# Quantum-Chemistry-Group-BNU/PyNQS

Measured on AMD Instinct MI355X. Metric: local energies/sec (whole node), higher is better.
Workload: dtype f64

## Files before the change

### include/pynqs_amd.h

```cpp
#ifndef PYNQS_AMD_H
#define PYNQS_AMD_H

#include <stdint.h>

#ifdef __cplusplus
extern "C" {
#endif

#define PYNQS_ABI_VERSION 1

#define PYNQS_OK 0
#define PYNQS_EINVAL (-1)
#define PYNQS_ELAUNCH (-2)
#define PYNQS_ELENGTH (-3)
#define PYNQS_EOVERFLOW (-4)

#define PYNQS_F32 0
#define PYNQS_F64 1

#define PYNQS_MAX_SORB_LEN 3
#define PYNQS_MAX_SORB 192
#define PYNQS_MAX_NELE 120
#define PYNQS_MAX_NVIR 120

int pynqs_abi_version(void);
const char *pynqs_last_error(void);

int64_t pynqs_num_sd(int sorb, int noA, int noB);

int pynqs_check_sorb(int sorb, int nele);

int pynqs_comb_hij_fused(const uint64_t *bra, int64_t nbatch, int sorb, int nele, int noA, int noB,
                         const void *h1e, const void *h2e, int dtype, uint64_t *comb, void *hmat,
                         void *stream);

int pynqs_comb(const uint64_t *bra, int64_t nbatch, int sorb, int noA, int noB, uint64_t *comb,
               double *comb_pm1, void *stream);

int pynqs_hij(const uint64_t *bra, int64_t n, const uint64_t *ket, int64_t m, int ket_is_3d,
              const void *h1e, const void *h2e, int dtype, int sorb, int nele, void *hmat, void *stream);

int pynqs_onv_to_pm1(const uint64_t *bra, int64_t n, int sorb, int dtype, void *out, void *stream);

int pynqs_pm01_to_onv(const uint8_t *occ, int64_t n, int sorb, uint64_t *out, void *stream);

int pynqs_wavefunction_lut(const uint64_t *keys, int64_t nkeys, const uint64_t *onv, int64_t n, int sorb,
                           int64_t *idx, uint8_t *mask, void *stream);

int pynqs_spin_flip_rand(const uint64_t *bra, int64_t n, int sorb, int noA, int noB, uint64_t seed,
                         uint64_t offset, uint64_t *out, void *stream);

int64_t pynqs_plan_bytes(int sorb, int dtype);
int pynqs_plan_build(const void *h1e, const void *h2e, int sorb, int dtype, void *plan, void *stream);

int pynqs_comb_hij_fused_plan(const uint64_t *bra, int64_t nbatch, int sorb, int nele, int noA, int noB,
                              const void *plan, int dtype, uint64_t *comb, void *hmat, void *stream);

int pynqs_eloc_sample_space(const uint64_t *bra, int64_t nbatch, int sorb, int nele, int noA, int noB,
                            const void *plan, const uint64_t *keys, int64_t nkeys, const double *wf,
                            int wf_is_complex, double *eloc, double *psi0, void *stream);

int64_t pynqs_hash_bytes(int64_t nkeys, int sorb);
int pynqs_hash_build(const uint64_t *keys, int64_t nkeys, int sorb, void *table, void *stream);
int pynqs_hash_lookup(const void *table, int64_t nkeys, const uint64_t *onv, int64_t n, int sorb, int64_t *idx,
                      uint8_t *mask, void *stream);
int pynqs_eloc_sample_space_hash(const uint64_t *bra, int64_t nbatch, int sorb, int nele, int noA, int noB,
                                 const void *plan, const void *table, int64_t nkeys, const double *wf,
                                 int wf_is_complex, double *eloc, double *psi0, void *stream);

int pynqs_eloc_sample_space_flip(const uint64_t *bra, int64_t nbatch, int sorb, int nele, int noA, int noB,
                                 const void *plan, const uint64_t *keys, int64_t nkeys, const double *wf,
                                 int wf_is_complex, const double *psi0, double *out, void *stream);
int pynqs_eloc_sample_space_hash_flip(const uint64_t *bra, int64_t nbatch, int sorb, int nele, int noA, int noB,
                                      const void *plan, const void *table, int64_t nkeys, const double *wf,
                                      int wf_is_complex, const double *psi0, double *out, void *stream);

int pynqs_eloc_sample_space_keys(const uint64_t *bra, int64_t nbatch, int sorb, int nele, int noA, int noB, const void *plan,
                                 const uint64_t *keys, int64_t nkeys, const double *wf, int wf_is_complex, int flip, double *eloc,
                                 double *psi0, void *stream);

int64_t pynqs_keys_index_bytes(int64_t nkeys, int sorb);
int64_t pynqs_keys_index_workspace(int64_t nkeys, int sorb);
int pynqs_keys_index_build(const uint64_t *keys, int64_t nkeys, int sorb, void *index, void *workspace, void *stream);
int pynqs_keys_index_density(const void *index, int64_t nkeys, int sorb, uint64_t *sum_sq, void *stream);
int pynqs_eloc_sample_space_indexed(const uint64_t *bra, int64_t nbatch, int sorb, int nele, int noA, int noB, const void *plan,
                                    const uint64_t *keys, int64_t nkeys, const void *index, const double *wf, int wf_is_complex,
                                    int flip, double *eloc, double *psi0, void *stream);

int pynqs_eloc_sample_space_form(int64_t nbatch, int sorb, int nele, int noA, int noB, int64_t nkeys, int hash, int64_t out[8]);
int pynqs_eloc_sample_space_keys_form(int64_t nbatch, int sorb, int64_t nkeys, int indexed, int64_t out[3]);

int64_t pynqs_unique_workspace(int64_t n);
int pynqs_unique_first(const uint64_t *onv, int64_t n, int sorb, void *workspace, int32_t *first, void *stream);

int pynqs_eloc_rbm_supported(int sorb, int nele, int noA, int noB, int nhidden);
int pynqs_eloc_rbm_form(int64_t nbatch, int sorb, int nele, int noA, int noB, int nhidden, int green);
int64_t pynqs_rbm_table_bytes(int sorb, int nhidden);
int pynqs_rbm_table_build(const double *weights, const double *hidden_bias, const double *visible_bias, int sorb,
                          int nhidden, void *table, void *stream);
int pynqs_eloc_rbm(const uint64_t *bra, int64_t nbatch, int sorb, int nele, int noA, int noB, const void *plan,
                   const void *rbm_table, int nhidden, double *eloc, double *psi, void *stream);
#define PYNQS_RBM_REAL 0
#define PYNQS_RBM_TANH 1
#define PYNQS_RBM_PHASE 2
int pynqs_eloc_rbm_flavour(const uint64_t *bra, int64_t nbatch, int sorb, int nele, int noA, int noB, const void *plan,
                           const void *rbm_table, int nhidden, int flavour, double *eloc, double *psi, void *stream);

int pynqs_eloc_crbm_supported(int sorb, int nele, int noA, int noB, int nhidden);
int pynqs_eloc_crbm_form(int64_t nbatch, int sorb, int nele, int noA, int noB, int nhidden);
int64_t pynqs_crbm_table_bytes(int sorb, int nhidden);
int pynqs_crbm_table_build(const double *weights, const double *hidden_bias, const double *visible_bias, int sorb, int nhidden,
                           void *table, void *stream);
int pynqs_eloc_crbm(const uint64_t *bra, int64_t nbatch, int sorb, int nele, int noA, int noB, const void *plan,
                    const void *crbm_table, int nhidden, double log_scale, double *eloc, double *psi, void *stream);

int64_t pynqs_jastrow_table_bytes(int sorb);
int pynqs_jastrow_table_build(const double *jastrow, int sorb, void *table, void *stream);
int pynqs_eloc_jrbm_supported(int sorb, int nele, int noA, int noB, int nhidden);
int pynqs_eloc_jrbm_form(int64_t nbatch, int sorb, int nele, int noA, int noB, int nhidden);
int pynqs_eloc_jrbm(const uint64_t *bra, int64_t nbatch, int sorb, int nele, int noA, int noB, const void *plan,
                    const void *rbm_table, const void *jastrow_table, int nhidden, double *eloc, double *psi, void *stream);
int pynqs_jrbm_forward(const uint64_t *onv, int64_t n, int sorb, const double *weights, const double *hidden_bias,
                       const double *visible_bias, const double *jastrow, int nhidden, double *psi, void *stream);
int64_t pynqs_jastrow_grad_workspace(int64_t n, int sorb);
int pynqs_jastrow_grad(const uint64_t *onv, int64_t n, int sorb, const double *jastrow, const double *prob, const double *eloc,
                       const double *e_total, const double *pow, double *grad_jastrow, double *loss, void *workspace, void *stream);

int pynqs_gfmc_sample(const double *green, int64_t n, int64_t ncomb, const double *rand_num, const uint64_t *comb,
                      int sorb, int64_t *index, double *beta, uint64_t *x_new, void *stream);

int pynqs_green_rbm(const uint64_t *bra, int64_t nbatch, int sorb, int nele, int noA, int noB, const void *plan,
                    const void *rbm_table, int nhidden, int flavour, double lambda, double *eloc, double *psi, double *green,
                    uint8_t *clamped, void *stream);
int pynqs_gfmc_sample_rank(const double *green, int64_t n, const double *rand_num, const uint64_t *bra, int sorb, int nele,
                           int noA, int noB, int64_t *index, double *beta, uint64_t *x_new, void *stream);

int64_t pynqs_moments_workspace(void);
int pynqs_stats_finish(const double *moments, double inv_world, double counts, double *out5, void *stream);
int pynqs_weighted_moments(const double *x, int is_complex, const double *prob, int64_t n, void *workspace, void *stream);

int64_t pynqs_reduce_tiles(int64_t nbatch, int sorb, int nele, int noA, int noB);
int pynqs_reduce_count(const uint64_t *bra, int64_t nbatch, int sorb, int nele, int noA, int noB,
                       const void *plan, int dtype, double eps, uint32_t *tile_counts, void *stream);
int pynqs_reduce_emit(const uint64_t *bra, int64_t nbatch, int sorb, int nele, int noA, int noB,
                      const void *plan, int dtype, double eps, const int64_t *tile_offsets, int32_t *kept_col,
                      uint64_t *kept_onv, void *kept_h, void *stream);

int pynqs_reduce_count_sums(const uint64_t *bra, int64_t nbatch, int sorb, int nele, int noA, int noB,
                            const void *plan, int dtype, double eps, uint32_t *tile_counts, double *tile_sums,
                            void *stream);
int pynqs_reduce_sample(const uint64_t *bra, int64_t nbatch, int sorb, int nele, int noA, int noB, const void *plan,
                        int dtype, double eps, const int32_t *tile_draws, const int64_t *sample_offsets,
                        const double *walker_scale, uint64_t seed, int32_t *s_col, uint64_t *s_onv, void *s_h,
                        void *stream);

typedef struct pynqs_reduce_io {
  int64_t cap_doubles;
  int64_t cap_unique;
  int64_t dedup_slots;
  int32_t *rec_col;
  void *rec_w;
  uint64_t *rec_onv;
  int32_t *rec_link;
  int32_t *seg_count;
  int32_t *srec_col;
  void *srec_w;
  uint64_t *srec_onv;
  int32_t *srec_link;
  double *row_sum;
  void *dedup_table;
  uint64_t *uniq_onv;
  void *uniq_pm1;
  int32_t pm1_dtype;
  int32_t lut_is_hash;
  const void *lut_table;
  int64_t lut_nkeys;
  int32_t *counters;
  const uint64_t *seed_dev;
  void *row_cache;
  int32_t *uniq_parent;
  void *tile_scratch;
  int64_t tile_scratch_bytes;
  float *row_f32;
} pynqs_reduce_io;
int pynqs_reduce_onepass_geometry(int64_t nbatch, int sorb, int nele, int noA, int noB, int eps_sample, int64_t *out4);
int64_t pynqs_reduce_onepass_tile_scratch_bytes(int64_t nbatch, int sorb, int nele, int noA, int noB, int eps_sample);
int pynqs_reduce_onepass_list_capacity(int64_t nbatch, int sorb, int nele, int noA, int noB, int dtype, int eps_sample,
                                       int with_row_cache, int without_table, int64_t *cap_doubles);
int pynqs_reduce_onepass_wants_row_f32(int64_t nbatch, int sorb, int nele, int noA, int noB, int dtype, int eps_sample, int64_t cap_doubles,
                                       int with_tile_scratch ,
                                       int without_table );
int64_t pynqs_reduce_onepass_row_f32_elements(int64_t nbatch, int sorb, int nele, int noA, int noB);
int pynqs_reduce_onepass(const uint64_t *bra, int64_t nbatch, int sorb, int nele, int noA, int noB, const void *plan,
                         int dtype, double eps, int eps_sample, uint64_t seed, const pynqs_reduce_io *io, void *stream);
int pynqs_reduce_contract(int64_t nbatch, int sorb, int nele, int noA, int noB, int dtype, int eps_sample,
                          const pynqs_reduce_io *io, const double *psi_unique, const double *psi_table, int psi_is_complex,
                          int divide, double *eloc, double *psi_x, void *stream);

#define PYNQS_RBM_COMPLEX 4
int pynqs_rbm_forward(const uint64_t *onv, int64_t n, int sorb, const double *weights, const double *hidden_bias,
                      const double *visible_bias, int nhidden, int flavour, double *psi, void *stream);

int64_t pynqs_rbm_children_table_bytes(int64_t nwalkers, int sorb, int nhidden, int flavour);
int pynqs_rbm_children_prepare(const uint64_t *walkers, int64_t nwalkers, int sorb, const double *weights, const double *hidden_bias,
                               const double *visible_bias, int nhidden, int flavour, void *table, void *stream);
int pynqs_rbm_forward_children(const uint64_t *onv, int64_t n, const int32_t *count_dev, const int32_t *parent,
                               const uint64_t *walkers, int64_t nwalkers, const void *table, int sorb, const double *weights,
                               const double *hidden_bias, const double *visible_bias, int nhidden, int flavour, double *psi,
                               void *stream);
int pynqs_rbm_forward_children_supported(int sorb, int nhidden, int flavour);

int64_t pynqs_rbm_grad_workspace(int64_t n, int sorb, int nhidden, int flavour);
int pynqs_rbm_grad(const uint64_t *onv, int64_t n, int sorb, const double *weights, const double *hidden_bias,
                   const double *visible_bias, int nhidden, int flavour, const double *prob, const double *eloc,
                   int eloc_is_complex, const double *e_total, const double *pow, double *grad_weights,
                   double *grad_hidden_bias, double *grad_visible_bias, double *loss, void *workspace, void *stream);

#define PYNQS_SR_RHO 0
#define PYNQS_SR_RHS2 1
#define PYNQS_SR_DONE 2
#define PYNQS_SR_ITER 3
#define PYNQS_SR_TRUE2 4
#define PYNQS_SR_PAP 5
#define PYNQS_SR_CONVERGED 6
#define PYNQS_SR_BREAKDOWN 7
#define PYNQS_SR_NSCALARS 8
#define PYNQS_SR_CG_INIT 0
#define PYNQS_SR_CG_STEP 1
#define PYNQS_SR_CG_RESIDUAL 2
int64_t pynqs_rbm_sr_workspace(int64_t n, int sorb, int nhidden, int flavour);
int pynqs_rbm_sr_prepare(const uint64_t *onv, int64_t n, int sorb, const double *weights, const double *hidden_bias, int nhidden,
                         int flavour, const double *prob, void *workspace, double *obar, void *stream);
int pynqs_rbm_sr_matvec(const uint64_t *onv, int64_t n, int sorb, int nhidden, int flavour, const double *prob, const void *workspace,
                        const double *obar, const double *v, double *y, void *stream);
int pynqs_rbm_sr_cg_step(int mode, int64_t np, double *y, const double *rhs, double *d, double *r, double *p, double *scalars,
                         double inv_world, double diag_shift, double tol, void *stream);

#define PYNQS_MCMC_ACCEPT_KEY 0x243F6A8885A308D3ull
int pynqs_mcmc_rbm_supported(int sorb, int nhidden, int flavour);
int pynqs_mcmc_rbm(uint64_t *states, int64_t nchains, int sorb, int noA, int noB, const void *table, int nhidden, int flavour,
                   uint64_t seed, uint64_t chain_base, uint64_t t0, int nsteps, int every, uint64_t *records, int64_t *n_accept,
                   double *lnpsi, void *stream);
int pynqs_mcmc_accept(uint64_t *states, double *psi, const uint64_t *proposals, const double *psi_proposals, int64_t nchains,
                      int sorb, int is_complex, uint64_t seed, uint64_t chain_base, uint64_t t, uint64_t *record_row,
                      int64_t *n_accept, void *stream);

int pynqs_rdm_scatter(const uint64_t *bra, int64_t nbatch, int sorb, int nele, int noA, int noB, const double *w, const double *ratio,
                      int is_complex, double *rdm1, double *rdm2, void *stream);
int pynqs_rdm_rbm_supported(int sorb, int nele, int noA, int noB, int nhidden);
int64_t pynqs_rdm_rbm_workspace(int64_t nbatch, int sorb, int nhidden);
int pynqs_rdm_rbm(const uint64_t *bra, int64_t nbatch, int sorb, int nele, int noA, int noB, const double *w, const void *rbm_table,
                  int nhidden, void *workspace, double *rdm1, double *rdm2, void *stream);

#ifdef __cplusplus
}
#endif
#endif
```

### pynqs_amd/C_extension.py

```python
from __future__ import annotations

import os
import warnings
import weakref
from typing import Tuple

import numpy as np
import torch
from torch import Tensor

from . import _native as N

MAX_SORB_LEN = 3
MAX_SORB = 64 * MAX_SORB_LEN
MAX_NELE = 120
USE_PLAN = True

__all__ = [
    "tensor_to_onv", "onv_to_tensor", "get_comb_tensor", "get_hij_torch", "get_comb_hij_fused",
    "wavefunction_lut", "hash_build", "hash_lookup", "HashTable", "RBMTable", "eloc_rbm", "JastrowTable", "eloc_jrbm", "jrbm_forward", "eloc_jrbm_supported", "merge_rank_sample", "spin_flip_rand", "check_sorb", "compress_h1e_h2e", "decompress_h1e_h2e", "get_Num_SinglesDoubles",
    "MAX_SORB", "MAX_SORB_LEN", "MAX_NELE",
]


def _bra_len(sorb: int) -> int:
    return (sorb - 1) // 64 + 1


def _gpu() -> torch.device:
    if not torch.cuda.is_available():
        raise RuntimeError("pynqs_amd: no HIP device available (this package has no CPU fallback)")
    return torch.device("cuda", torch.cuda.current_device())


def _stage(*ts: Tensor):
    all_cpu = all(t.device.type == "cpu" for t in ts)
    dev = next((t.device for t in ts if t.device.type == "cuda"), None) or _gpu()
    return dev, [t if t.device == dev else t.to(dev) for t in ts], all_cpu


def _ver(t: Tensor) -> int:
    try:
        return t._version
    except RuntimeError:
        return -1


def _stream(dev: torch.device) -> int:
    return torch.cuda.current_stream(dev).cuda_stream


def _contig(t: Tensor, name: str) -> None:
    if not t.is_contiguous():
        raise RuntimeError(f"{name} must be contiguous")


def _check_onv(t: Tensor, name: str, sorb: int, dims) -> None:
    _contig(t, name)
    if t.dtype != torch.uint8:
        raise RuntimeError(f"{name} must be torch.uint8")
    if t.dim() not in dims:
        raise RuntimeError(f"{name} must have dim in {dims}, got {t.dim()}")
    if t.size(-1) != 8 * _bra_len(sorb):
        raise RuntimeError(f"{name}: last dim {t.size(-1)} != 8 * bra_len = {8 * _bra_len(sorb)} for sorb = {sorb}")


def _fdtype(h1e: Tensor, h2e: Tensor) -> int:
    if h1e.dtype != h2e.dtype or h1e.dtype not in (torch.float32, torch.float64):
        raise RuntimeError("h1e/h2e must both be float32 or both float64")
    return N.PYNQS_F64 if h1e.dtype == torch.float64 else N.PYNQS_F32


def _check_integrals(h1e: Tensor, h2e: Tensor, sorb: int) -> None:
    _contig(h1e, "h1e_tensor"); _contig(h2e, "h2e_tensor")
    pair = sorb * (sorb - 1) // 2
    if h1e.numel() != sorb * sorb or h2e.numel() != pair * (pair + 1) // 2:
        raise RuntimeError(f"h1e/h2e sizes {h1e.numel()}/{h2e.numel()} do not match sorb = {sorb}")


class IntegralPlan:

    def __init__(self, h1e: Tensor, h2e: Tensor, sorb: int, device: "torch.device | None" = None):
        code = _fdtype(h1e, h2e)
        _check_integrals(h1e, h2e, sorb)
        nbytes = N.lib().pynqs_plan_bytes(sorb, code)
        if nbytes < 0:
            raise RuntimeError(f"integral plan needs an even sorb in [2, {MAX_SORB}], got {sorb}")
        dev, (a, b), _ = _stage(h1e, h2e)
        if device is not None and device.type == "cuda" and all(t.device.type == "cpu" for t in (h1e, h2e)):
            dev, a, b = device, h1e.to(device), h2e.to(device)
        self.sorb, self.code, self.dtype, self.device = sorb, code, h1e.dtype, dev
        self.buf = torch.empty(nbytes // h1e.element_size(), dtype=h1e.dtype, device=dev)
        N.check(N.lib().pynqs_plan_build(a.data_ptr(), b.data_ptr(), sorb, code, self.buf.data_ptr(), _stream(dev)), "plan_build")
        if a is not h1e or b is not h2e:
            torch.cuda.current_stream(dev).synchronize()

    def data_ptr(self) -> int:
        return self.buf.data_ptr()


_PLANS: "list[tuple]" = []
_MAX_PLANS = 4
_PLAN_BUILDS: "dict[tuple, int]" = {}
_PLAN_REBUILD_WARN = 16


_FINGERPRINT_CHUNK = 1 << 24


def _fingerprint(h1e: Tensor, h2e: Tensor):
    if any(t.is_cuda for t in (h1e, h2e)) and torch.cuda.is_current_stream_capturing():
        return None
    golden = -7046029254386353131
    out = []
    with torch.no_grad():
        for t in (h1e, h2e):
            c = t.detach().contiguous().reshape(-1)
            c = c.view(torch.int64) if c.element_size() == 8 else c.view(torch.int32)
            plain = torch.zeros((), dtype=torch.int64, device=c.device)
            mixed = torch.zeros((), dtype=torch.int64, device=c.device)
            for s in range(0, c.numel(), _FINGERPRINT_CHUNK):
                v = c[s:s + _FINGERPRINT_CHUNK].to(torch.int64)
                plain += v.sum()
                m = torch.arange(s, s + v.numel(), dtype=torch.int64, device=c.device).mul_(golden).add_(v)
                del v
                m.bitwise_xor_(m >> 30).mul_(-4658895280553007687)
                m.bitwise_xor_(m >> 27).mul_(-7723592293110705685)
                m.bitwise_xor_(m >> 31)
                mixed += m.sum()
                del m
            out.append((tuple(t.shape), str(t.dtype), str(t.device), int(plain.item()), int(mixed.item())))
    return tuple(out)


def plan_for(h1e: Tensor, h2e: Tensor, sorb: int, device: "torch.device | None" = None) -> "IntegralPlan | None":
    if sorb % 2 or sorb < 2:
        return None
    ver = (_ver(h1e), _ver(h2e), h1e.data_ptr(), h2e.data_ptr())
    trackable = ver[0] >= 0 and ver[1] >= 0
    def same(ref, t):
        o = ref()
        return o is t or (o is not None and o.data_ptr() == t.data_ptr() and o.shape == t.shape and o.stride() == t.stride() and o.dtype == t.dtype)

    dev_ok = lambda pl: device is None or device.type != "cuda" or pl.device == device or h1e.device.type == "cuda"
    for i, (r1, r2, v, s, pl, fp) in enumerate(_PLANS if trackable else ()):
        if same(r1, h1e) and same(r2, h2e) and v == ver and s == sorb and dev_ok(pl):
            if i:
                _PLANS.insert(0, _PLANS.pop(i))
            return pl
    fp = None
    if any(s == sorb and f is not None and f[1][0] == tuple(h2e.shape) for _, _, _, s, _, f in _PLANS):
        fp = _fingerprint(h1e, h2e)
        for i, (r1, r2, v, s, pl, f) in enumerate(_PLANS):
            if fp is not None and f == fp and s == sorb and dev_ok(pl):
# ... 292 lines not shown

    def _build(self, kind: str, given, params, nhidden: int, sorb: int) -> None:
        dev, ts, _ = _stage(*params)
        self.nhidden, self.sorb, self.device = nhidden, sorb, dev
        nbytes = getattr(N.lib(), f"pynqs_{kind}_table_bytes")(sorb, nhidden)
        if nbytes < 0:
            raise RuntimeError(f"bad RBM sizes: sorb = {sorb}, num_hidden = {nhidden}")
        self.buf = torch.empty(nbytes // 8, dtype=torch.float64, device=dev)
        N.check(getattr(N.lib(), f"pynqs_{kind}_table_build")(ts[0].data_ptr(), ts[1].data_ptr(), ts[2].data_ptr() if len(ts) > 2 else None,
                                                              sorb, nhidden, self.buf.data_ptr(), _stream(dev)), f"{kind}_table_build")
        if any(a.data_ptr() != b.data_ptr() for a, b in zip(given, ts)):
            torch.cuda.current_stream(dev).synchronize()

    def data_ptr(self) -> int:
        return self.buf.data_ptr()


class RBMTable(_RBMTableBase):

    def __init__(self, weights: Tensor, hidden_bias: Tensor, visible_bias: "Tensor | None" = None) -> None:
        if weights.dim() != 2 or hidden_bias.numel() != weights.size(0):
            raise RuntimeError("weights must be [num_hidden, sorb] and hidden_bias [num_hidden]")
        if visible_bias is not None and visible_bias.numel() != weights.size(1):
            raise RuntimeError("visible_bias must be [sorb]")
        ts = [weights, hidden_bias] + ([visible_bias] if visible_bias is not None else [])
        if any(t.dtype != torch.float64 for t in ts):
            raise RuntimeError("the fused RBM local energy is float64 only")
        self._build("rbm", ts, [t.detach().contiguous() for t in ts], int(weights.size(0)), int(weights.size(1)))


class JastrowTable:

    def __init__(self, jastrow: Tensor) -> None:
        if jastrow.dim() != 2 or jastrow.size(0) != jastrow.size(1):
            raise RuntimeError("jastrow must be [sorb, sorb]")
        if jastrow.dtype != torch.float64:
            raise RuntimeError("the fused Jastrow-RBM local energy is float64 only")
        given = jastrow.detach().contiguous()
        dev, (m,), _ = _stage(given)
        self.sorb, self.device = int(m.size(0)), dev
        nbytes = N.lib().pynqs_jastrow_table_bytes(self.sorb)
        if nbytes < 0:
            raise RuntimeError(f"bad Jastrow size: sorb = {self.sorb}")
        self.buf = torch.empty(nbytes // 8, dtype=torch.float64, device=dev)
        N.check(N.lib().pynqs_jastrow_table_build(m.data_ptr(), self.sorb, self.buf.data_ptr(), _stream(dev)), "jastrow_table_build")
        if m.data_ptr() != jastrow.data_ptr():
            torch.cuda.current_stream(dev).synchronize()

    def data_ptr(self) -> int:
        return self.buf.data_ptr()


RBM_TYPE_FLAVOUR = {"real": N.RBM_REAL, "tanh": N.RBM_TANH, "pRBM": N.RBM_PHASE, "complex": N.RBM_COMPLEX}
RBM_FLAVOURS = {k: v for k, v in RBM_TYPE_FLAVOUR.items() if v != N.RBM_COMPLEX}


def _rbm_dtype(rbm_type: str) -> torch.dtype:
    return torch.complex128 if rbm_type in ("pRBM", "complex") else torch.float64


def _eloc_fused(bra: Tensor, h1e: Tensor, h2e: Tensor, table, sorb: int, want_psi: bool, dtype: torch.dtype, call):
    if table.sorb != sorb:
        raise RuntimeError(f"RBM table was built for sorb = {table.sorb}, not {sorb}")
    if _fdtype(h1e, h2e) != N.PYNQS_F64:
        raise RuntimeError("the fused RBM local energy is float64 only")
    plan = plan_for(h1e, h2e, sorb, bra.device)
    if plan is None:
        raise RuntimeError("the fused RBM local energy needs an even sorb")
    dev, (x,), all_cpu = _stage(bra)
    if plan.device != dev or table.device != dev:
        raise RuntimeError("bra, integrals and RBM table must be on the same device")
    n = x.size(0)
    eloc = torch.empty(n, dtype=dtype, device=dev)
    psi = torch.empty(n, dtype=dtype, device=dev) if want_psi else None
    call(x, n, plan, eloc, psi.data_ptr() if want_psi else None, _stream(dev))
    if all_cpu and bra.device.type == "cpu":
        return eloc.cpu(), (psi.cpu() if want_psi else None)
    return eloc, psi


def eloc_rbm(bra: Tensor, h1e: Tensor, h2e: Tensor, table: RBMTable, sorb: int, nele: int, noA: int, noB: int,
             want_psi: bool = True, rbm_type: str = "real") -> Tuple[Tensor, "Tensor | None"]:
    _check_onv(bra, "bra", sorb, (2,))
    if rbm_type not in RBM_FLAVOURS:
        raise RuntimeError(f"rbm_type {rbm_type!r} has no fused local energy (fused: {sorted(RBM_FLAVOURS)})")
    return _eloc_fused(bra, h1e, h2e, table, sorb, want_psi, _rbm_dtype(rbm_type), lambda x, n, plan, eloc, psi, st: N.check(
        N.lib().pynqs_eloc_rbm_flavour(x.data_ptr(), n, sorb, nele, noA, noB, plan.data_ptr(), table.data_ptr(), table.nhidden,
                                       RBM_FLAVOURS[rbm_type], eloc.data_ptr(), psi, st), "pynqs_eloc_rbm"))


def eloc_jrbm_supported(sorb: int, nele: int, noA: int, noB: int, num_hidden: int) -> bool:
    return bool(N.lib().pynqs_eloc_jrbm_supported(sorb, nele, noA, noB, num_hidden))


def eloc_jrbm(bra: Tensor, h1e: Tensor, h2e: Tensor, rbm_table: RBMTable, jastrow_table: JastrowTable, sorb: int, nele: int, noA: int, noB: int,
              want_psi: bool = True) -> Tuple[Tensor, "Tensor | None"]:
    _check_onv(bra, "bra", sorb, (2,))
    if jastrow_table.sorb != sorb or jastrow_table.device != rbm_table.device:
        raise RuntimeError(f"Jastrow table: sorb = {jastrow_table.sorb} on {jastrow_table.device}, RBM table: sorb = {sorb} on {rbm_table.device}")
    return _eloc_fused(bra, h1e, h2e, rbm_table, sorb, want_psi, torch.float64, lambda x, n, plan, eloc, psi, st: N.check(
        N.lib().pynqs_eloc_jrbm(x.data_ptr(), n, sorb, nele, noA, noB, plan.data_ptr(), rbm_table.data_ptr(), jastrow_table.data_ptr(),
                                rbm_table.nhidden, eloc.data_ptr(), psi, st), "pynqs_eloc_jrbm"))


def jrbm_forward(onv: Tensor, weights: Tensor, hidden_bias: Tensor, visible_bias: "Tensor | None", jastrow: Tensor, sorb: int) -> Tensor:
    _check_onv(onv, "onv", sorb, (2,))
    _, W, hb, vb, H = _rbm_params(weights, hidden_bias, visible_bias, sorb, "real", on_gpu=False)
    M = jastrow.detach().double().contiguous()
    if M.shape != (sorb, sorb):
        raise RuntimeError("jastrow must be [sorb, sorb]")
    if not (onv.is_cuda and W.is_cuda and hb.is_cuda and (vb is None or vb.is_cuda) and M.is_cuda):
        raise RuntimeError("jrbm_forward: determinants and parameters must be on the GPU")
    n = onv.size(0)
    psi = torch.empty(n, dtype=torch.float64, device=onv.device)
    N.check(N.lib().pynqs_jrbm_forward(onv.data_ptr(), n, sorb, W.data_ptr(), hb.data_ptr(), vb.data_ptr() if vb is not None else None, M.data_ptr(),
                                       H, psi.data_ptr(), _stream(onv.device)), "pynqs_jrbm_forward")
    return psi


def rbm_forward(onv: Tensor, weights: Tensor, hidden_bias: Tensor, visible_bias: "Tensor | None", sorb: int, rbm_type: str = "real") -> Tensor:
    _check_onv(onv, "onv", sorb, (2,))
    flav, W, hb, vb, H = _rbm_params(weights, hidden_bias, visible_bias, sorb, rbm_type, on_gpu=False)
    if not (onv.is_cuda and W.is_cuda and hb.is_cuda and (vb is None or vb.is_cuda)):
        raise RuntimeError("rbm_forward: determinants and parameters must be on the GPU")
    n = onv.size(0)
    psi = torch.empty(n, dtype=_rbm_dtype(rbm_type), device=onv.device)
    N.check(N.lib().pynqs_rbm_forward(onv.data_ptr(), n, sorb, W.data_ptr(), hb.data_ptr(), vb.data_ptr() if vb is not None else None, H, flav,
                                      psi.data_ptr(), _stream(onv.device)), "pynqs_rbm_forward")
    return psi


def _rbm_params(weights, hidden_bias, visible_bias, sorb, rbm_type, on_gpu=True):
    flav = RBM_TYPE_FLAVOUR.get(rbm_type)
    if flav is None:
        raise RuntimeError(f"rbm_type {rbm_type!r} has no fused forward")
    cplx_par = rbm_type == "complex"
    W = weights.detach().double().contiguous()
    hb = hidden_bias.detach().double().contiguous()
    vb = visible_bias.detach().double().contiguous() if visible_bias is not None else None
    H = W.size(0)
    if W.shape[:2] != (H, sorb) or W.dim() != (3 if cplx_par else 2) or hb.numel() != H * (2 if cplx_par else 1) or \
            (vb is not None and vb.numel() != sorb * (2 if cplx_par else 1)):
        raise RuntimeError("RBM parameter shapes do not match sorb / num_hidden")
    if on_gpu and not (W.is_cuda and hb.is_cuda and (vb is None or vb.is_cuda)):
        raise RuntimeError("RBM parameters must be on the GPU")
    return flav, W, hb, vb, H


def rbm_forward_children_supported(sorb: int, num_hidden: int, rbm_type: str = "real") -> bool:
    flav = RBM_TYPE_FLAVOUR.get(rbm_type)
    return flav is not None and bool(N.lib().pynqs_rbm_forward_children_supported(sorb, num_hidden, flav))


def rbm_forward_children(onv: Tensor, parent: Tensor, walkers: Tensor, weights: Tensor, hidden_bias: Tensor, visible_bias: "Tensor | None",
                         sorb: int, rbm_type: str = "real", count: "Tensor | None" = None, out: "Tensor | None" = None) -> Tensor:
    _check_onv(onv, "onv", sorb, (2,))
    _check_onv(walkers, "walkers", sorb, (2,))
    flav, W, hb, vb, H = _rbm_params(weights, hidden_bias, visible_bias, sorb, rbm_type)
    dev = onv.device
    if not (onv.is_cuda and walkers.device == dev and parent.device == dev and parent.dtype == torch.int32 and parent.numel() >= onv.size(0)):
        raise RuntimeError("rbm_forward_children: onv, walkers and parent (int32) on one GPU")
    n, nw = onv.size(0), walkers.size(0)
    nbytes = N.lib().pynqs_rbm_children_table_bytes(nw, sorb, H, flav)
    table = torch.empty(max(nbytes // 8, 1), dtype=torch.float64, device=dev)
    st = _stream(dev)
    wk = walkers.contiguous()
    N.check(N.lib().pynqs_rbm_children_prepare(wk.data_ptr(), nw, sorb, W.data_ptr(), hb.data_ptr(), vb.data_ptr() if vb is not None else None,
                                               H, flav, table.data_ptr(), st), "pynqs_rbm_children_prepare")
    psi = out if out is not None else torch.empty(n, dtype=_rbm_dtype(rbm_type), device=dev)
    N.check(N.lib().pynqs_rbm_forward_children(onv.contiguous().data_ptr(), n, count.data_ptr() if count is not None else None, parent.data_ptr(),
                                               wk.data_ptr(), nw, table.data_ptr(), sorb, W.data_ptr(), hb.data_ptr(),
                                               vb.data_ptr() if vb is not None else None, H, flav, psi.data_ptr(), st), "pynqs_rbm_forward_children")
    return psi


class CRBMTable(_RBMTableBase):

    def __init__(self, weights: Tensor, hidden_bias: Tensor, visible_bias: "Tensor | None" = None) -> None:
        def as_pairs(t: Tensor) -> Tensor:
            t = t.detach()
            if t.is_complex():
                t = torch.view_as_real(t.to(torch.complex128))
            if t.dtype != torch.float64 or t.size(-1) != 2:
                raise RuntimeError("complex RBM parameters must be complex128 or float64 (re, im) pairs")
            return t.contiguous()

        w, hb = as_pairs(weights), as_pairs(hidden_bias).reshape(-1, 2)
        vb = as_pairs(visible_bias).reshape(-1, 2) if visible_bias is not None else None
        if w.dim() != 3 or hb.size(0) != w.size(0) or (vb is not None and vb.size(0) != w.size(1)):
            raise RuntimeError("weights must be [num_hidden, sorb], hidden_bias [num_hidden], visible_bias [sorb]")
        given = [weights, hidden_bias] + ([visible_bias] if visible_bias is not None else [])
        self._build("crbm", given, [w, hb] + ([vb] if vb is not None else []), int(w.size(0)), int(w.size(1)))


def eloc_crbm(bra: Tensor, h1e: Tensor, h2e: Tensor, table: CRBMTable, sorb: int, nele: int, noA: int, noB: int,
              want_psi: bool = True, log_scale: float = 0.0) -> Tuple[Tensor, "Tensor | None"]:
    _check_onv(bra, "bra", sorb, (2,))
    return _eloc_fused(bra, h1e, h2e, table, sorb, want_psi, torch.complex128, lambda x, n, plan, eloc, psi, st: N.check(
        N.lib().pynqs_eloc_crbm(x.data_ptr(), n, sorb, nele, noA, noB, plan.data_ptr(), table.data_ptr(), table.nhidden, float(log_scale),
                                eloc.data_ptr(), psi, st), "pynqs_eloc_crbm"))


_CHARTS = None


def constrain_make_charts(sym_idex: Tensor) -> Tensor:
    sym_index = sym_idex
    global _CHARTS
    if _CHARTS is None:
        t = torch.zeros((16, 4), dtype=torch.float64)
        for k, row in zip((10, 6, 14, 9, 5, 13, 11, 7, 15), ((1, 0, 0, 0), (0, 0, 1, 0), (1, 0, 1, 0), (0, 1, 0, 0), (0, 0, 0, 1), (0, 1, 0, 1),
                                                             (1, 1, 0, 0), (0, 0, 1, 1), (1, 1, 1, 1))):
            t[k] = torch.tensor(row, dtype=torch.float64)
        _CHARTS = t
    idx = sym_index.reshape(-1).long()
    inside = (idx >= 0) & (idx < 16)
    out = _CHARTS.to(idx.device)[idx.clamp(0, 15)]
    return torch.where(inside.unsqueeze(1), out, torch.zeros_like(out))


def permute_sgn(image2: Tensor, onstate: Tensor, sorb: int) -> Tensor:
    if image2.numel() != sorb and onstate.size(-1) != sorb:
        raise ValueError("Dim error")
    if onstate.size(0) == 0:
        return torch.zeros(0, dtype=torch.float64, device=onstate.device)
    order = image2.reshape(-1).long().to(onstate.device)
    occ = (onstate.reshape(onstate.size(0), -1)[:, order] != 0).to(torch.float64)
    pos = torch.arange(order.numel(), device=order.device)
    inverted = ((pos.unsqueeze(1) < pos.unsqueeze(0)) & (order.unsqueeze(1) > order.unsqueeze(0))).to(torch.float64)
    pairs = ((occ @ inverted) * occ).sum(1)
    return (1 - 2 * (pairs.long() & 1)).to(torch.float64)


def spin_flip_rand(bra: Tensor, sorb: int, nele: int, noA: int, noB: int, seed: int, in_place: bool = False) -> Tuple[Tensor, Tensor]:
    global _SPIN_FLIP_CALLS
    _check_onv(bra, "bra_tensor", sorb, (1, 2))
    x2 = bra.view(-1, bra.size(-1))
    n = x2.size(0)
    dev, (x,), cpu = _stage(x2)
    out = x if (in_place and not cpu) else torch.empty_like(x)
    if n:
        N.check(N.lib().pynqs_spin_flip_rand(x.data_ptr(), n, sorb, noA, noB, int(seed) & (2**64 - 1), _SPIN_FLIP_CALLS << 32,
                                             out.data_ptr(), _stream(dev)), "spin_flip_rand")
    _SPIN_FLIP_CALLS += 1
    if cpu:
        out = out.cpu()
        if in_place:
            x2.copy_(out)
            out = x2
    return onv_to_tensor(out, sorb), out


def merge_rank_sample(idx: Tensor, counts: Tensor, split_idx: Tensor, length: int) -> Tensor:
    _contig(idx, "idx"); _contig(counts, "counts")
    out = torch.zeros(int(length), dtype=torch.int64, device=idx.device)
    return out.index_add_(0, idx.to(torch.int64), counts.to(torch.int64))


def _pair_maps(sorb: int):
    i, j = np.meshgrid(np.arange(sorb), np.arange(sorb), indexing="ij")
    hi, lo = np.maximum(i, j), np.minimum(i, j)
    pair = hi * (hi - 1) // 2 + lo
    sgn = np.where(i > j, 1.0, -1.0)
    return pair, sgn, i != j


def compress_h1e_h2e(h1e: np.ndarray, h2e: np.ndarray, sorb: int):
    h1e = np.asarray(h1e, dtype=np.float64)
    h2e = np.asarray(h2e, dtype=np.float64)
    if h1e.shape != (sorb, sorb) or h2e.shape != (sorb,) * 4:
        raise ValueError(f"expected h1e {(sorb, sorb)} and h2e {(sorb,) * 4}, got {h1e.shape} and {h2e.shape}")
    npair = sorb * (sorb - 1) // 2
    pair, sgn, off = _pair_maps(sorb)
    out = np.zeros(npair * (npair + 1) // 2, dtype=np.float64)
    kl, skl, okl = pair[None, :, :], sgn[None, :, :], off[None, :, :]
    for i in range(sorb):
        ij = pair[i][:, None, None]
        valid = off[i][:, None, None] & okl
        P, Q = np.maximum(ij, kl), np.minimum(ij, kl)
        out[(P * (P + 1) // 2 + Q)[valid]] = (sgn[i][:, None, None] * skl * h2e[i])[valid]
    return h1e.reshape(-1).copy(), out


def decompress_h1e_h2e(h1e: np.ndarray, h2e: np.ndarray, sorb: int):
    h1e = np.asarray(h1e, dtype=np.float64).reshape(-1)
    h2e = np.asarray(h2e, dtype=np.float64).reshape(-1)
    npair = sorb * (sorb - 1) // 2
    if h1e.size != sorb * sorb:
        raise ValueError(f"h1e array size is incorrect: expected {sorb * sorb}, got {h1e.size}")
    if h2e.size != npair * (npair + 1) // 2:
        raise ValueError(f"h2e array size is incorrect: expected {npair * (npair + 1) // 2}, got {h2e.size}")
    pair, sgn, off = _pair_maps(sorb)
    full = np.zeros((sorb,) * 4, dtype=np.float64)
    kl, skl, okl = pair[None, :, :], sgn[None, :, :], off[None, :, :]
    for i in range(sorb):
        ij = pair[i][:, None, None]
        valid = off[i][:, None, None] & okl
        P, Q = np.maximum(ij, kl), np.minimum(ij, kl)
        slot = np.where(valid, P * (P + 1) // 2 + Q, 0)
        full[i] = np.where(valid, h2e[slot] * (sgn[i][:, None, None] * skl), 0.0)
    return h1e.reshape(sorb, sorb).copy(), full
```

### pynqs_amd/_native.py

```python
from __future__ import annotations

import ctypes as C
import os

_HERE = os.path.dirname(os.path.abspath(__file__))
LIB_PATH = os.environ.get("PYNQS_AMD_LIB") or os.path.join(_HERE, "csrc", "libpynqs_amd.so")

PYNQS_F32, PYNQS_F64 = 0, 1
RBM_REAL, RBM_TANH, RBM_PHASE, RBM_COMPLEX = 0, 1, 2, 4
OK, EINVAL, ELAUNCH, ELENGTH, EOVERFLOW = 0, -1, -2, -3, -4

_i64, _int, _vp, _dbl = C.c_int64, C.c_int, C.c_void_p, C.c_double

SIGNATURES = {
    "pynqs_abi_version": (_int, []),
    "pynqs_last_error": (C.c_char_p, []),
    "pynqs_num_sd": (_i64, [_int, _int, _int]),
    "pynqs_check_sorb": (_int, [_int, _int]),
    "pynqs_comb_hij_fused": (_int, [_vp, _i64, _int, _int, _int, _int, _vp, _vp, _int, _vp, _vp, _vp]),
    "pynqs_comb": (_int, [_vp, _i64, _int, _int, _int, _vp, _vp, _vp]),
    "pynqs_hij": (_int, [_vp, _i64, _vp, _i64, _int, _vp, _vp, _int, _int, _int, _vp, _vp]),
    "pynqs_onv_to_pm1": (_int, [_vp, _i64, _int, _int, _vp, _vp]),
    "pynqs_pm01_to_onv": (_int, [_vp, _i64, _int, _vp, _vp]),
    "pynqs_wavefunction_lut": (_int, [_vp, _i64, _vp, _i64, _int, _vp, _vp, _vp]),
    "pynqs_spin_flip_rand": (_int, [_vp, _i64, _int, _int, _int, C.c_uint64, C.c_uint64, _vp, _vp]),
    "pynqs_plan_bytes": (_i64, [_int, _int]),
    "pynqs_plan_build": (_int, [_vp, _vp, _int, _int, _vp, _vp]),
    "pynqs_comb_hij_fused_plan": (_int, [_vp, _i64, _int, _int, _int, _int, _vp, _int, _vp, _vp, _vp]),
    "pynqs_eloc_sample_space": (_int, [_vp, _i64, _int, _int, _int, _int, _vp, _vp, _i64, _vp, _int, _vp, _vp, _vp]),
    "pynqs_hash_bytes": (_i64, [_i64, _int]),
    "pynqs_hash_build": (_int, [_vp, _i64, _int, _vp, _vp]),
    "pynqs_hash_lookup": (_int, [_vp, _i64, _vp, _i64, _int, _vp, _vp, _vp]),
    "pynqs_unique_workspace": (_i64, [_i64]),
    "pynqs_unique_first": (_int, [_vp, _i64, _int, _vp, _vp, _vp]),
    "pynqs_eloc_sample_space_hash": (_int, [_vp, _i64, _int, _int, _int, _int, _vp, _vp, _i64, _vp, _int, _vp, _vp, _vp]),
    "pynqs_eloc_sample_space_flip": (_int, [_vp, _i64, _int, _int, _int, _int, _vp, _vp, _i64, _vp, _int, _vp, _vp, _vp]),
    "pynqs_eloc_sample_space_hash_flip": (_int, [_vp, _i64, _int, _int, _int, _int, _vp, _vp, _i64, _vp, _int, _vp, _vp, _vp]),
    "pynqs_eloc_sample_space_keys": (_int, [_vp, _i64, _int, _int, _int, _int, _vp, _vp, _i64, _vp, _int, _int, _vp, _vp, _vp]),
    "pynqs_keys_index_bytes": (_i64, [_i64, _int]),
    "pynqs_keys_index_workspace": (_i64, [_i64, _int]),
    "pynqs_keys_index_build": (_int, [_vp, _i64, _int, _vp, _vp, _vp]),
    "pynqs_keys_index_density": (_int, [_vp, _i64, _int, _vp, _vp]),
    "pynqs_eloc_sample_space_indexed": (_int, [_vp, _i64, _int, _int, _int, _int, _vp, _vp, _i64, _vp, _vp, _int, _int, _vp, _vp, _vp]),
    "pynqs_eloc_sample_space_form": (_int, [_i64, _int, _int, _int, _int, _i64, _int, C.POINTER(_i64)]),
    "pynqs_eloc_sample_space_keys_form": (_int, [_i64, _int, _i64, _int, C.POINTER(_i64)]),
    "pynqs_eloc_rbm_supported": (_int, [_int, _int, _int, _int, _int]),
    "pynqs_eloc_rbm_form": (_int, [_i64, _int, _int, _int, _int, _int, _int]),
    "pynqs_rbm_table_bytes": (_i64, [_int, _int]),
    "pynqs_rbm_table_build": (_int, [_vp, _vp, _vp, _int, _int, _vp, _vp]),
    "pynqs_eloc_rbm": (_int, [_vp, _i64, _int, _int, _int, _int, _vp, _vp, _int, _vp, _vp, _vp]),
    "pynqs_eloc_rbm_flavour": (_int, [_vp, _i64, _int, _int, _int, _int, _vp, _vp, _int, _int, _vp, _vp, _vp]),
    "pynqs_eloc_crbm_supported": (_int, [_int, _int, _int, _int, _int]),
    "pynqs_eloc_crbm_form": (_int, [_i64, _int, _int, _int, _int, _int]),
    "pynqs_crbm_table_bytes": (_i64, [_int, _int]),
    "pynqs_crbm_table_build": (_int, [_vp, _vp, _vp, _int, _int, _vp, _vp]),
    "pynqs_eloc_crbm": (_int, [_vp, _i64, _int, _int, _int, _int, _vp, _vp, _int, _dbl, _vp, _vp, _vp]),
    "pynqs_gfmc_sample": (_int, [_vp, _i64, _i64, _vp, _vp, _int, _vp, _vp, _vp, _vp]),
    "pynqs_green_rbm": (_int, [_vp, _i64, _int, _int, _int, _int, _vp, _vp, _int, _int, _dbl, _vp, _vp, _vp, _vp, _vp]),
    "pynqs_gfmc_sample_rank": (_int, [_vp, _i64, _vp, _vp, _int, _int, _int, _int, _vp, _vp, _vp, _vp]),
    "pynqs_moments_workspace": (_i64, []),
    "pynqs_stats_finish": (_int, [_vp, _dbl, _dbl, _vp, _vp]),
    "pynqs_weighted_moments": (_int, [_vp, _int, _vp, _i64, _vp, _vp]),
    "pynqs_reduce_tiles": (_i64, [_i64, _int, _int, _int, _int]),
    "pynqs_reduce_count": (_int, [_vp, _i64, _int, _int, _int, _int, _vp, _int, _dbl, _vp, _vp]),
    "pynqs_reduce_count_sums": (_int, [_vp, _i64, _int, _int, _int, _int, _vp, _int, _dbl, _vp, _vp, _vp]),
    "pynqs_reduce_sample": (_int, [_vp, _i64, _int, _int, _int, _int, _vp, _int, _dbl, _vp, _vp, _vp, C.c_uint64, _vp, _vp, _vp, _vp]),
    "pynqs_reduce_emit": (_int, [_vp, _i64, _int, _int, _int, _int, _vp, _int, _dbl, _vp, _vp, _vp, _vp, _vp]),
}



class ReduceIO(C.Structure):
    _fields_ = [("cap_doubles", _i64), ("cap_unique", _i64), ("dedup_slots", _i64),
                ("rec_col", _vp), ("rec_w", _vp), ("rec_onv", _vp), ("rec_link", _vp), ("seg_count", _vp),
                ("srec_col", _vp), ("srec_w", _vp), ("srec_onv", _vp), ("srec_link", _vp), ("row_sum", _vp),
                ("dedup_table", _vp), ("uniq_onv", _vp), ("uniq_pm1", _vp), ("pm1_dtype", C.c_int32), ("lut_is_hash", C.c_int32),
                ("lut_table", _vp), ("lut_nkeys", _i64), ("counters", _vp), ("seed_dev", _vp), ("row_cache", _vp), ("uniq_parent", _vp),
                ("tile_scratch", _vp), ("tile_scratch_bytes", _i64), ("row_f32", _vp)]


SIGNATURES.update({
    "pynqs_reduce_onepass_geometry": (_int, [_i64, _int, _int, _int, _int, _int, C.POINTER(_i64)]),
    "pynqs_reduce_onepass_tile_scratch_bytes": (_i64, [_i64, _int, _int, _int, _int, _int]),
    "pynqs_reduce_onepass_list_capacity": (_int, [_i64, _int, _int, _int, _int, _int, _int, _int, _int, C.POINTER(_i64)]),
    "pynqs_reduce_onepass_wants_row_f32": (_int, [_i64, _int, _int, _int, _int, _int, _int, _i64, _int, _int]),
    "pynqs_reduce_onepass_row_f32_elements": (_i64, [_i64, _int, _int, _int, _int]),
    "pynqs_reduce_onepass": (_int, [_vp, _i64, _int, _int, _int, _int, _vp, _int, _dbl, _int, C.c_uint64, C.POINTER(ReduceIO), _vp]),
    "pynqs_rbm_forward": (_int, [_vp, _i64, _int, _vp, _vp, _vp, _int, _int, _vp, _vp]),
    "pynqs_rbm_children_table_bytes": (_i64, [_i64, _int, _int, _int]),
    "pynqs_rbm_children_prepare": (_int, [_vp, _i64, _int, _vp, _vp, _vp, _int, _int, _vp, _vp]),
    "pynqs_rbm_forward_children": (_int, [_vp, _i64, _vp, _vp, _vp, _i64, _vp, _int, _vp, _vp, _vp, _int, _int, _vp, _vp]),
    "pynqs_rbm_forward_children_supported": (_int, [_int, _int, _int]),
    "pynqs_rbm_grad_workspace": (_i64, [_i64, _int, _int, _int]),
    "pynqs_rbm_grad": (_int, [_vp, _i64, _int, _vp, _vp, _vp, _int, _int, _vp, _vp, _int, _vp, _vp, _vp, _vp, _vp, _vp, _vp, _vp]),
    "pynqs_reduce_contract": (_int, [_i64, _int, _int, _int, _int, _int, _int, C.POINTER(ReduceIO), _vp, _vp, _int, _int, _vp, _vp, _vp]),    "pynqs_mcmc_rbm_supported": (_int, [_int, _int, _int]),
    "pynqs_mcmc_rbm": (_int, [_vp, _i64, _int, _int, _int, _vp, _int, _int, C.c_uint64, C.c_uint64, C.c_uint64, _int, _int, _vp, _vp, _vp, _vp]),
    "pynqs_rbm_sr_workspace": (_i64, [_i64, _int, _int, _int]),
    "pynqs_rbm_sr_prepare": (_int, [_vp, _i64, _int, _vp, _vp, _int, _int, _vp, _vp, _vp, _vp]),
    "pynqs_rbm_sr_matvec": (_int, [_vp, _i64, _int, _int, _int, _vp, _vp, _vp, _vp, _vp, _vp]),
    "pynqs_rbm_sr_cg_step": (_int, [_int, _i64, _vp, _vp, _vp, _vp, _vp, _vp, _dbl, _dbl, _dbl, _vp]),
    "pynqs_mcmc_accept": (_int, [_vp, _vp, _vp, _vp, _i64, _int, _int, C.c_uint64, C.c_uint64, C.c_uint64, _vp, _vp, _vp]),
    "pynqs_rdm_scatter": (_int, [_vp, _i64, _int, _int, _int, _int, _vp, _vp, _int, _vp, _vp, _vp]),
    "pynqs_rdm_rbm_supported": (_int, [_int, _int, _int, _int, _int]),
    "pynqs_rdm_rbm_workspace": (_i64, [_i64, _int, _int]),
    "pynqs_rdm_rbm": (_int, [_vp, _i64, _int, _int, _int, _int, _vp, _vp, _int, _vp, _vp, _vp, _vp]),
    "pynqs_jastrow_table_bytes": (_i64, [_int]),
    "pynqs_jastrow_table_build": (_int, [_vp, _int, _vp, _vp]),
    "pynqs_eloc_jrbm_supported": (_int, [_int, _int, _int, _int, _int]),
    "pynqs_eloc_jrbm_form": (_int, [_i64, _int, _int, _int, _int, _int]),
    "pynqs_eloc_jrbm": (_int, [_vp, _i64, _int, _int, _int, _int, _vp, _vp, _vp, _int, _vp, _vp, _vp]),
    "pynqs_jrbm_forward": (_int, [_vp, _i64, _int, _vp, _vp, _vp, _vp, _int, _vp, _vp]),
    "pynqs_jastrow_grad_workspace": (_i64, [_i64, _int]),
    "pynqs_jastrow_grad": (_int, [_vp, _i64, _int, _vp, _vp, _vp, _vp, _vp, _vp, _vp, _vp, _vp]),
})

_lib = None


class NativeLibraryError(RuntimeError):
    pass


def lib() -> C.CDLL:
    global _lib
    if _lib is None:
        if not os.path.exists(LIB_PATH):
            raise NativeLibraryError(
                f"{LIB_PATH} not found: build the HIP extension first (python -c 'import __graft_entry__ as g; g.build()'). "
                "pynqs_amd has no CPU fallback."
            )
        try:
            l = C.CDLL(LIB_PATH)
        except OSError as e:
            raise NativeLibraryError(f"cannot load {LIB_PATH}: {e}") from e
        for name, (res, args) in SIGNATURES.items():
            f = getattr(l, name)
            f.restype = res
            f.argtypes = args
        if l.pynqs_abi_version() != 1:
            raise NativeLibraryError("libpynqs_amd.so ABI version mismatch")
        _lib = l
    return _lib


def check(rc: int, what: str) -> None:
    if rc == OK:
        return
    msg = lib().pynqs_last_error().decode(errors="replace")
    if rc == ELENGTH:
        raise ValueError(msg)
    if rc == EOVERFLOW:
        raise OverflowError(msg)
    raise RuntimeError(f"{what}: {msg} (code {rc})")
```

### pynqs_amd/csrc/kernels_gfmc.hip

```cpp
#include "detcore.h"
#include "launch.h"

namespace pynqs {

constexpr int kGfmcMaxTiles = 1024;

__device__ __forceinline__ double wave_incl_scan(double v, int lane) {
#pragma unroll
  for (int d = 1; d < 64; d <<= 1) {
    const double o = __shfl_up(v, d);
    if (lane >= d) v += o;
  }
  return v;
}

template <int LEN, bool FROM_RANK>
__global__ __launch_bounds__(kBlock) void gfmc_sample_kernel(const double *__restrict__ gk, int64_t m, uint32_t tile, uint32_t ntiles,
                                                             const double *__restrict__ rnd, const uint64_t *__restrict__ comb, SDParams p,
                                                             int64_t *__restrict__ index, double *__restrict__ beta,
                                                             uint64_t *__restrict__ x_new) {
  __shared__ double tsum[kGfmcMaxTiles];
  __shared__ double s_target, s_before;
  __shared__ uint32_t s_tile;
  const int64_t walker = blockIdx.x;
  const int tid = threadIdx.x, lane = tid & 63, wave = tid >> 6;
  const double *__restrict__ row = gk + walker * m;
  for (uint32_t t = wave; t < ntiles; t += kBlock / 64) {
    const int64_t c0 = (int64_t)t * tile, c1 = min(c0 + (int64_t)tile, m);
    double acc = 0.0;
    for (int64_t c = c0 + lane; c < c1; c += 64) acc += row[c];
#pragma unroll
    for (int d = 32; d > 0; d >>= 1) acc += __shfl_xor(acc, d);
    if (lane == 0) tsum[t] = acc;
  }
  __syncthreads();
  if (wave == 0) {
    constexpr int kPer = kGfmcMaxTiles / 64;
    double loc[kPer], s = 0.0;
#pragma unroll
    for (int i = 0; i < kPer; ++i) {
      const uint32_t t = lane * kPer + i;
      loc[i] = t < ntiles ? tsum[t] : 0.0;
      s += loc[i];
    }
    const double incl = wave_incl_scan(s, lane);
    const double total = __shfl(incl, 63);
    const double target = rnd[walker] * total;
    double before = incl - s;
    uint32_t mine = 0xffffffffu;
    double mine_before = 0.0;
#pragma unroll
    for (int i = 0; i < kPer; ++i) {
      const uint32_t t = lane * kPer + i;
      if (mine == 0xffffffffu && t < ntiles && before + loc[i] >= target) { mine = t; mine_before = before; }
      before += loc[i];
    }
    const uint64_t have = __ballot(mine != 0xffffffffu);
    const int first = have ? __ffsll((long long)have) - 1 : -1;
    if (lane == (first < 0 ? 0 : first)) {
      s_tile = first < 0 ? ntiles - 1 : mine;
      s_before = first < 0 ? total - tsum[ntiles - 1] : mine_before;
      s_target = target;
    }
    if (lane == 0) beta[walker] = total;
  }
  __syncthreads();
  if (wave == 0) {
    const uint32_t t = s_tile;
    const double target = s_target;
    double run = s_before;
    const int64_t c0 = (int64_t)t * tile, c1 = min(c0 + (int64_t)tile, m);
    int64_t found = -1, last_pos = -1;
    for (int64_t c = c0; c < c1 && found < 0; c += 64) {
      const double v = c + lane < c1 ? row[c + lane] : 0.0;
      const double incl = wave_incl_scan(v, lane) + run;
      const uint64_t hit = __ballot(c + lane < c1 && incl >= target);
      if (hit) found = c + __ffsll((long long)hit) - 1;
      const uint64_t pos = __ballot(v > 0.0);
      if (pos) last_pos = c + 63 - __clzll((long long)pos);
      run = __shfl(incl, 63);
    }
    if (found < 0) found = last_pos >= 0 ? last_pos : c1 - 1;
    if (lane == 0) index[walker] = found;
    if constexpr (FROM_RANK) {
      if (lane == 0) {
        uint64_t x[LEN];
#pragma unroll
        for (int i = 0; i < LEN; ++i) x[i] = comb[walker * LEN + i];
        if (found > 0) excite_by_rank<LEN>(x, (uint32_t)(found - 1), p);
#pragma unroll
        for (int i = 0; i < LEN; ++i) x_new[walker * LEN + i] = x[i];
      }
    } else {
      if (lane < LEN) x_new[walker * LEN + lane] = comb[(walker * m + found) * LEN + lane];
    }
  }
}

}

using namespace pynqs;

template <bool FROM_RANK>
static int gfmc_sample_impl(const double *green, int64_t n, int64_t ncomb, const double *rand_num, const uint64_t *comb, int sorb,
                            const SDParams &p, int64_t *index, double *beta, uint64_t *x_new, void *stream) {
  pynqs::DeviceScope device_scope_(green);
  if (n < 0 || ncomb < 1 || sorb < 1 || sorb > kMaxSorb) return set_error(PYNQS_EINVAL, "bad n / ncomb / sorb");
  if (n == 0) return PYNQS_OK;
  if (!green || !rand_num || !comb || !index || !beta || !x_new) return set_error(PYNQS_EINVAL, "null pointer");
  if (n > 0x7fffffffll) return set_error(PYNQS_EINVAL, "n too large for one launch");
  uint32_t tile = 256;
  while ((ncomb + tile - 1) / tile > kGfmcMaxTiles) tile *= 2;
  const uint32_t ntiles = (uint32_t)((ncomb + tile - 1) / tile);
  const int len = (sorb - 1) / 64 + 1;
  hipStream_t st = (hipStream_t)stream;
  DISPATCH_LEN(len, hipLaunchKernelGGL((gfmc_sample_kernel<LEN, FROM_RANK>), dim3((uint32_t)n), dim3(kBlock), 0, st, green, ncomb, tile, ntiles,
                                       rand_num, comb, p, index, beta, x_new));
  return check_launch("gfmc_sample");
}

extern "C" int pynqs_gfmc_sample(const double *green, int64_t n, int64_t ncomb, const double *rand_num, const uint64_t *comb, int sorb,
                                 int64_t *index, double *beta, uint64_t *x_new, void *stream) {
  SDParams p = {};
  return gfmc_sample_impl<false>(green, n, ncomb, rand_num, comb, sorb, p, index, beta, x_new, stream);
}

extern "C" int pynqs_gfmc_sample_rank(const double *green, int64_t n, const double *rand_num, const uint64_t *bra, int sorb, int nele,
                                      int noA, int noB, int64_t *index, double *beta, uint64_t *x_new, void *stream) {
  SDParams p;
  if (!make_sd_params(sorb, nele, noA, noB, &p)) return set_error(PYNQS_EINVAL, "bad sorb/noA/noB");
  return gfmc_sample_impl<true>(green, n, (int64_t)p.nsd + 1, rand_num, bra, sorb, p, index, beta, x_new, stream);
}

namespace pynqs {

constexpr int kMomentBlocks = 128;

template <bool CPLX>
__global__ __launch_bounds__(kBlock) void moments_kernel(const double *__restrict__ x, const double *__restrict__ prob, int64_t n,
                                                         double *__restrict__ out, unsigned int *__restrict__ done) {
  __shared__ double red[4][kBlock / 64];
  __shared__ bool last;
  const int tid = threadIdx.x, lane = tid & 63, wave = tid >> 6;
  double s[4] = {0.0, 0.0, 0.0, 0.0};
  for (int64_t i = (int64_t)blockIdx.x * kBlock + tid; i < n; i += (int64_t)gridDim.x * kBlock) {
    const double p = prob[i];
    const double re = CPLX ? x[2 * i] : x[i], im = CPLX ? x[2 * i + 1] : 0.0;
    s[0] += p * re; s[1] += p * im; s[2] += p * (re * re + im * im); s[3] += p;
  }
#pragma unroll
  for (int k = 0; k < 4; ++k) {
#pragma unroll
    for (int d = 32; d > 0; d >>= 1) s[k] += __shfl_xor(s[k], d);
    if (lane == 0) red[k][wave] = s[k];
  }
  __syncthreads();
  if (tid < 4) {
    double t = 0.0;
    for (int w = 0; w < kBlock / 64; ++w) t += red[tid][w];
    out[4 * (1 + blockIdx.x) + tid] = t;
  }
  __threadfence();
  __syncthreads();
  if (tid == 0) last = atomicAdd(done, 1u) == gridDim.x - 1;
  __syncthreads();
  if (last) {
    __threadfence();
    if (tid < 4) {
      double t = 0.0;
      for (unsigned b = 0; b < gridDim.x; ++b) t += out[4 * (1 + b) + tid];
      out[tid] = t;
    }
    if (tid == 0) *done = 0;
  }
}

}

namespace pynqs {
__global__ void stats_finish_kernel(const double *__restrict__ m, double inv_world, double counts, double *__restrict__ out) {
  const double re = m[0] * inv_world, im = m[1] * inv_world, m2 = m[2] * inv_world, ps = m[3] * inv_world;
  double var = m2 - (re * re + im * im) * (2.0 - ps);
  var = var > 0.0 ? var : 0.0;
  const double sd = sqrt(var);
  out[0] = re; out[1] = im; out[2] = var; out[3] = sd; out[4] = sd / sqrt(counts);
}
}

extern "C" int pynqs_stats_finish(const double *moments, double inv_world, double counts, double *out5, void *stream) {
  pynqs::DeviceScope device_scope_(moments);
  if (!moments || !out5 || !(counts > 0.0)) return set_error(PYNQS_EINVAL, "bad arguments");
  hipLaunchKernelGGL(stats_finish_kernel, dim3(1), dim3(1), 0, (hipStream_t)stream, moments, inv_world, counts, out5);
  return check_launch("stats_finish");
}

extern "C" int64_t pynqs_moments_workspace(void) { return 8 * 4 * (pynqs::kMomentBlocks + 1) + 8; }

extern "C" int pynqs_weighted_moments(const double *x, int is_complex, const double *prob, int64_t n, void *workspace, void *stream) {
  pynqs::DeviceScope device_scope_(x);
  if (n < 0) return set_error(PYNQS_EINVAL, "bad n");
  if (!workspace || (n > 0 && (!x || !prob))) return set_error(PYNQS_EINVAL, "null pointer");
  double *out = (double *)workspace;
  unsigned int *done = (unsigned int *)(out + 4 * (kMomentBlocks + 1));
  int64_t blocks = (n + kBlock - 1) / kBlock;
  if (blocks > kMomentBlocks) blocks = kMomentBlocks;
  if (blocks < 1) blocks = 1;
  hipStream_t st = (hipStream_t)stream;
  if (is_complex) hipLaunchKernelGGL((moments_kernel<true>), dim3((uint32_t)blocks), dim3(kBlock), 0, st, x, prob, n, out, done);
  else hipLaunchKernelGGL((moments_kernel<false>), dim3((uint32_t)blocks), dim3(kBlock), 0, st, x, prob, n, out, done);
  return check_launch("weighted_moments");
}
```

### pynqs_amd/csrc/kernels_rbm_forward.hip

```cpp
#include "detcore.h"
#include "launch.h"
#include "rbm_math.h"

namespace pynqs {

constexpr int kHChunk = 8;

struct Prod {
  double re = 1.0, im = 0.0;
  double lin = 0.0, ang = 0.0;
  int e2 = 0;
  __device__ __forceinline__ void renorm() {
    int k;
    (void)frexp(fmax(fabs(re), fabs(im)), &k);
    re = ldexp(re, -k); im = ldexp(im, -k);
    e2 += k;
  }
  __device__ __forceinline__ bool finite() const { return fabs(re) < __builtin_inf() && fabs(im) < __builtin_inf(); }
  template <bool CPLX>
  __device__ __forceinline__ void times_2cosh(double x, double y) {
    const double ax = fabs(x);
    const double rho = exp(-2.0 * ax);
    lin += ax;
    if constexpr (CPLX) {
      const double sy = x < 0.0 ? -y : y;
      double sn, cs;
      sincos_mod(-2.0 * sy, sn, cs);
      const double u = fma(rho, cs, 1.0), v = rho * sn;
      const double nr = re * u - im * v;
      im = fma(re, v, im * u);
      re = nr;
      ang += sy;
    } else {
      re *= 1.0 + rho;
    }
  }
};

template <int FLAVOUR>
__device__ __forceinline__ void write_psi(double *__restrict__ psi, int64_t i, const Prod &P, double axr, double axi) {
  const double kLn2 = 0.693147180559945309417;
  if constexpr (FLAVOUR == PYNQS_RBM_REAL) {
    psi[i] = P.re * exp(axr + P.lin + kLn2 * (double)P.e2);
  } else if constexpr (FLAVOUR == PYNQS_RBM_TANH) {
    psi[i] = tanh(axr) * P.re * exp(P.lin + kLn2 * (double)P.e2);
  } else if constexpr (FLAVOUR == PYNQS_RBM_PHASE) {
    double sn, cs;
    sincos(axr + P.lin + log(P.re) + kLn2 * (double)P.e2, &sn, &cs);
    psi[2 * i] = cs; psi[2 * i + 1] = sn;
  } else {
    const double m = exp(axr + P.lin + kLn2 * (double)P.e2);
    double sn, cs;
    sincos(axi + P.ang, &sn, &cs);
    psi[2 * i] = m * (P.re * cs - P.im * sn);
    psi[2 * i + 1] = m * (P.re * sn + P.im * cs);
  }
}

template <int LEN, int FLAVOUR>
__device__ __forceinline__ void rbm_forward_row(const uint64_t (&ket)[LEN], int sorb, int H, const double *__restrict__ W,
                                                const double *__restrict__ hb, const double *__restrict__ vb, Prod &P, double &axr, double &axi) {
  constexpr bool CPLX = FLAVOUR == PYNQS_RBM_COMPLEX;
  for (int h0 = 0; h0 < H; h0 += kHChunk) {
    double tr[kHChunk], ti[kHChunk];
#pragma unroll
    for (int j = 0; j < kHChunk; ++j) {
      const int h = min(h0 + j, H - 1);
      tr[j] = CPLX ? hb[2 * h] : hb[h];
      ti[j] = CPLX ? hb[2 * h + 1] : 0.0;
    }
    for (int o = 0; o < sorb; ++o) {
      const double x = pm1_of<LEN>(ket, o);
#pragma unroll
      for (int j = 0; j < kHChunk; ++j) {
        const int h = min(h0 + j, H - 1);
        if constexpr (CPLX) {
          tr[j] = fma(x, W[((size_t)h * sorb + o) * 2], tr[j]);
          ti[j] = fma(x, W[((size_t)h * sorb + o) * 2 + 1], ti[j]);
        } else {
          tr[j] = fma(x, W[(size_t)h * sorb + o], tr[j]);
        }
      }
    }
#pragma unroll
    for (int j = 0; j < kHChunk; ++j)
      if (h0 + j < H) P.template times_2cosh<CPLX>(tr[j], ti[j]);
    P.renorm();
  }
  axr = 0.0; axi = 0.0;
  if (vb) {
    for (int o = 0; o < sorb; ++o) {
      const double x = pm1_of<LEN>(ket, o);
      if constexpr (CPLX) { axr = fma(x, vb[2 * o], axr); axi = fma(x, vb[2 * o + 1], axi); }
      else axr = fma(x, vb[o], axr);
    }
  }
}

template <int LEN, int FLAVOUR>
__global__ __launch_bounds__(kBlock) void rbm_forward_kernel(const uint64_t *__restrict__ onv, int64_t n, int sorb, int H,
                                                             const double *__restrict__ W, const double *__restrict__ hb,
                                                             const double *__restrict__ vb, double *__restrict__ psi) {
  const int64_t i = (int64_t)blockIdx.x * kBlock + threadIdx.x;
  const int64_t row = i < n ? i : n - 1;
  uint64_t ket[LEN];
#pragma unroll
  for (int w = 0; w < LEN; ++w) ket[w] = onv[row * LEN + w];
  Prod P;
  double axr, axi;
  rbm_forward_row<LEN, FLAVOUR>(ket, sorb, H, W, hb, vb, P, axr, axi);
  if (i >= n) return;
  write_psi<FLAVOUR>(psi, i, P, axr, axi);
}

template <int LEN>
__global__ __launch_bounds__(kBlock) void jrbm_forward_kernel(const uint64_t *__restrict__ onv, int64_t n, int sorb, int H,
                                                              const double *__restrict__ W, const double *__restrict__ hb,
                                                              const double *__restrict__ vb, const double *__restrict__ M,
                                                              double *__restrict__ psi) {
  const int64_t i = (int64_t)blockIdx.x * kBlock + threadIdx.x;
  const int64_t row = i < n ? i : n - 1;
  uint64_t ket[LEN];
#pragma unroll
  for (int w = 0; w < LEN; ++w) ket[w] = onv[row * LEN + w];
  Prod P;
  double axr, axi;
  rbm_forward_row<LEN, PYNQS_RBM_REAL>(ket, sorb, H, W, hb, vb, P, axr, axi);
  double xmx = 0.0;
  for (int a = 0; a < sorb; ++a) {
    double r = 0.0;
    for (int b = 0; b < sorb; ++b) r = fma(pm1_of<LEN>(ket, b), M[(size_t)a * sorb + b], r);
    xmx = fma(pm1_of<LEN>(ket, a), r, xmx);
  }
  if (i >= n) return;
  write_psi<PYNQS_RBM_REAL>(psi, i, P, axr + xmx, axi);
}

__host__ __device__ inline int children_hp(int H) { return (H + 2) | 1; }

template <bool CPLX>
__global__ __launch_bounds__(kBlock) void rbm_children_factors_kernel(int sorb, int H, const double *__restrict__ W, const double *__restrict__ vb,
                                                                      double *__restrict__ factors) {
  constexpr int C = CPLX ? 2 : 1;
  const int HP = children_hp(H);
  const int idx = blockIdx.x * kBlock + threadIdx.x;
  if (idx == 0) factors[(size_t)(2 * sorb + 1) * HP * C] = 0.0;
  if (idx >= (2 * sorb + 1) * HP) return;
  const int row = idx / HP, h = idx - row * HP, o = row >> 1;
  const double sign = (row & 1) ? -1.0 : 1.0;
  double re = 0.0, im = 0.0;
  if (row == 2 * sorb) {
    re = h < H ? 1.0 : 0.0;
  } else if (h < H) {
    const double wr = W[((size_t)h * sorb + o) * C], wi = CPLX ? W[((size_t)h * sorb + o) * C + 1] : 0.0;
    const double m = fabs(4.0 * wr) <= 80.0 ? exp(-4.0 * sign * wr) : __builtin_nan("");
    if constexpr (CPLX) {
      double sn, cs;
      sincos(-4.0 * sign * wi, &sn, &cs);
      re = m * cs; im = m * sn;
    } else {
      re = m;
    }
  } else if (h == H) {
#pragma unroll 16
    for (int k = 0; k < H; ++k) {
      re += W[((size_t)k * sorb + o) * C];
      if constexpr (CPLX) im += W[((size_t)k * sorb + o) * C + 1];
    }
    re *= 2.0 * sign; im *= 2.0 * sign;
  } else if (h == H + 1 && vb) {
    re = 2.0 * sign * vb[(size_t)o * C];
    if constexpr (CPLX) im = 2.0 * sign * vb[(size_t)o * C + 1];
  }
  factors[(size_t)idx * C] = re;
  if constexpr (CPLX) factors[(size_t)idx * C + 1] = im;
}

constexpr int kParentChunk = 4;

template <int LEN, bool CPLX>
__global__ __launch_bounds__(kBlock) void rbm_children_parents_kernel(const uint64_t *__restrict__ onv, int64_t n, int sorb, int H,
                                                                      const double *__restrict__ W, const double *__restrict__ hb,
                                                                      const double *__restrict__ vb, const double *__restrict__ factors,
                                                                      double *__restrict__ table) {
  constexpr int C = CPLX ? 2 : 1;
  const int64_t i = (int64_t)blockIdx.x * kBlock + threadIdx.x;
  const int64_t row = i < n ? i : n - 1;
  const int h0 = (int)blockIdx.y * kParentChunk;
  uint64_t ket[LEN];
#pragma unroll
  for (int w = 0; w < LEN; ++w) ket[w] = onv[row * LEN + w];
  double *__restrict__ out = table + (size_t)row * (size_t)(H + 2) * C;
  double tr[kParentChunk], ti[kParentChunk];
#pragma unroll
  for (int j = 0; j < kParentChunk; ++j) {
    const int h = min(h0 + j, H - 1);
    tr[j] = CPLX ? hb[2 * h] : hb[h];
    ti[j] = CPLX ? hb[2 * h + 1] : 0.0;
  }
  for (int o = 0; o < sorb; ++o) {
    const double x = pm1_of<LEN>(ket, o);
#pragma unroll
    for (int j = 0; j < kParentChunk; ++j) {
      const int h = min(h0 + j, H - 1);
      tr[j] = fma(x, W[((size_t)h * sorb + o) * C], tr[j]);
      if constexpr (CPLX) ti[j] = fma(x, W[((size_t)h * sorb + o) * C + 1], ti[j]);
    }
  }
#pragma unroll
  for (int j = 0; j < kParentChunk; ++j) {
    if (h0 + j < H && i < n) {
      if (!(tr[j] > -340.0)) const_cast<double *>(factors)[(size_t)(2 * sorb + 1) * children_hp(H) * C] = 1.0;
      const double m = exp(-2.0 * tr[j]);
      if constexpr (CPLX) {
        double sn, cs;
        sincos_mod(-2.0 * ti[j], sn, cs);
        out[(size_t)(h0 + j) * 2] = m * cs;
        out[(size_t)(h0 + j) * 2 + 1] = m * sn;
      } else {
        out[h0 + j] = m;
      }
    }
  }
  if (blockIdx.y != 0) return;
  const int HP = children_hp(H);
  double sr = 0.0, si = 0.0, axr = 0.0, axi = 0.0;
  for (int h = 0; h < H; ++h) {
    sr += hb[(size_t)h * C];
    if constexpr (CPLX) si += hb[(size_t)h * C + 1];
  }
  for (int o = 0; o < sorb; ++o) {
    const double x = pm1_of<LEN>(ket, o);
    const double *__restrict__ f = factors + ((size_t)(2 * o) * HP + H) * C;
    sr = fma(0.5 * x, f[0], sr);
    axr = fma(0.5 * x, f[C], axr);
    if constexpr (CPLX) { si = fma(0.5 * x, f[1], si); axi = fma(0.5 * x, f[C + 1], axi); }
  }
  if (i >= n) return;
  out[(size_t)H * C] = sr;
  out[(size_t)(H + 1) * C] = axr;
  if constexpr (CPLX) { out[(size_t)H * C + 1] = si; out[(size_t)(H + 1) * C + 1] = axi; }
}

#ifndef PYNQS_CHILD_BLOCK
#define PYNQS_CHILD_BLOCK 1024
#endif
constexpr int kChildBlock = PYNQS_CHILD_BLOCK;

template <int LEN, int FLAVOUR>
__global__ __launch_bounds__(kChildBlock) void rbm_forward_children_kernel(const uint64_t *__restrict__ onv, int64_t n, const int32_t *__restrict__ count_dev,
                                                                      const int32_t *__restrict__ parent, const uint64_t *__restrict__ walkers,
                                                                      int64_t nwalkers, const double *__restrict__ table,
                                                                      const double *__restrict__ factors, int sorb, int H,
                                                                      const double *__restrict__ W, const double *__restrict__ hb,
                                                                      const double *__restrict__ vb, double *__restrict__ psi) {
  constexpr bool CPLX = FLAVOUR == PYNQS_RBM_COMPLEX;
  constexpr int C = CPLX ? 2 : 1;
  extern __shared__ __attribute__((aligned(16))) double wl[];
  const int HP = children_hp(H);
  int64_t cnt = n;
  if (count_dev) cnt = min((int64_t)max(*count_dev, 0), n);
  if (factors[(size_t)(2 * sorb + 1) * HP * C] != 0.0) {
    const int64_t rounds = (cnt + (int64_t)gridDim.x * kChildBlock - 1) / ((int64_t)gridDim.x * kChildBlock);
    for (int64_t r = 0; r < rounds; ++r) {
      const int64_t i = ((int64_t)r * gridDim.x + blockIdx.x) * kChildBlock + threadIdx.x;
      const int64_t row = i < cnt ? i : cnt - 1;
      uint64_t ket[LEN];
#pragma unroll
      for (int w = 0; w < LEN; ++w) ket[w] = onv[row * LEN + w];
      Prod P;
      double axr, axi;
      rbm_forward_row<LEN, FLAVOUR>(ket, sorb, H, W, hb, vb, P, axr, axi);
      if (i < cnt) write_psi<FLAVOUR>(psi, i, P, axr, axi);
    }
    return;
  }
  for (int idx = threadIdx.x; idx < (2 * sorb + 1) * HP * C; idx += kChildBlock) wl[idx] = factors[idx];
  __syncthreads();
  for (int64_t i = (int64_t)blockIdx.x * kChildBlock + threadIdx.x; i < cnt; i += (int64_t)gridDim.x * kChildBlock) {
    int64_t p = parent[i];
    bool stranger = p < 0 || p >= nwalkers;
    p = stranger ? 0 : p;
    int at[4];
#pragma unroll
    for (int q = 0; q < 4; ++q) at[q] = 2 * sorb * HP;
    int k = 0, nflip = 0;
#pragma unroll
    for (int w = 0; w < LEN; ++w) {
      const uint64_t xc = onv[i * LEN + w];
      uint64_t d = xc ^ walkers[p * LEN + w];
      nflip += __popcll(d);
#pragma unroll
      for (int t = 0; t < 4; ++t) {
        if (d && k < 4) {
          const int b = __builtin_ctzll(d);
          d &= d - 1;
          const int r = (2 * (64 * w + b) + (((xc >> b) & 1ull) ? 0 : 1)) * HP;
#pragma unroll
          for (int q = 0; q < 4; ++q)
            if (q == k) at[q] = r;
          ++k;
        }
      }
    }
    const double *__restrict__ tp = table + (size_t)p * (size_t)(H + 2) * C;
    Prod P;
    for (int h0 = 0; h0 < H; h0 += kHChunk) {
#pragma unroll
      for (int j = 0; j < kHChunk; ++j) {
        const int h = h0 + j;
        if (h < H) {
          double qr = tp[(size_t)h * C], qi = CPLX ? tp[(size_t)h * C + 1] : 0.0;
#pragma unroll
          for (int q = 0; q < 4; ++q) {
            const double fr = wl[(size_t)(at[q] + h) * C];
            if constexpr (CPLX) {
              const double fi = wl[(size_t)(at[q] + h) * C + 1];
              const double nr = qr * fr - qi * fi;
              qi = fma(qr, fi, qi * fr);
              qr = nr;
            } else {
              qr *= fr;
            }
          }
          if constexpr (CPLX) {
            const double u = 1.0 + qr;
            const double nr = P.re * u - P.im * qi;
            P.im = fma(P.re, qi, P.im * u);
            P.re = nr;
          } else {
            P.re *= 1.0 + qr;
          }
        }
      }
      P.renorm();
    }
    double axr = tp[(size_t)(H + 1) * C], axi = CPLX ? tp[(size_t)(H + 1) * C + 1] : 0.0;
    P.lin = tp[(size_t)H * C];
    P.ang = CPLX ? tp[(size_t)H * C + 1] : 0.0;
#pragma unroll
    for (int q = 0; q < 4; ++q) {
      P.lin += wl[(size_t)(at[q] + H) * C];
      axr += wl[(size_t)(at[q] + H + 1) * C];
      if constexpr (CPLX) {
        P.ang += wl[(size_t)(at[q] + H) * C + 1];
        axi += wl[(size_t)(at[q] + H + 1) * C + 1];
      }
    }
    stranger = stranger || nflip > 4 || !P.finite();
    if (__ballot(stranger)) {
      uint64_t ket[LEN];
#pragma unroll
      for (int w = 0; w < LEN; ++w) ket[w] = onv[i * LEN + w];
      Prod P2;
      double a2r, a2i;
      rbm_forward_row<LEN, FLAVOUR>(ket, sorb, H, W, hb, vb, P2, a2r, a2i);
      if (stranger) { P = P2; axr = a2r; axi = a2i; }
    }
    write_psi<FLAVOUR>(psi, i, P, axr, axi);
  }
}

template <int LEN, int FLAVOUR>
__global__ __launch_bounds__(kBlock) void rbm_forward_children_wave_kernel(const uint64_t *__restrict__ onv, int64_t n, const int32_t *__restrict__ count_dev,
                                                                           const int32_t *__restrict__ parent, const uint64_t *__restrict__ walkers,
                                                                           int64_t nwalkers, const double *__restrict__ table,
                                                                           const double *__restrict__ factors, int sorb, int H,
                                                                           const double *__restrict__ W, const double *__restrict__ hb,
                                                                           const double *__restrict__ vb, double *__restrict__ psi) {
  constexpr bool CPLX = FLAVOUR == PYNQS_RBM_COMPLEX;
  constexpr int C = CPLX ? 2 : 1;
  const int HP = children_hp(H);
  int64_t cnt = n;
  if (count_dev) cnt = min((int64_t)max(*count_dev, 0), n);
  if (factors[(size_t)(2 * sorb + 1) * HP * C] != 0.0) {
    const int64_t rounds = (cnt + (int64_t)gridDim.x * kBlock - 1) / ((int64_t)gridDim.x * kBlock);
    for (int64_t r = 0; r < rounds; ++r) {
      const int64_t i = ((int64_t)r * gridDim.x + blockIdx.x) * kBlock + threadIdx.x;
      const int64_t row = i < cnt ? i : cnt - 1;
      uint64_t ket[LEN];
#pragma unroll
      for (int w = 0; w < LEN; ++w) ket[w] = onv[row * LEN + w];
      Prod P;
      double axr, axi;
      rbm_forward_row<LEN, FLAVOUR>(ket, sorb, H, W, hb, vb, P, axr, axi);
      if (i < cnt) write_psi<FLAVOUR>(psi, i, P, axr, axi);
    }
    return;
  }
  const int lane = threadIdx.x & 63;
  const int wave = __builtin_amdgcn_readfirstlane((int)(threadIdx.x >> 6));
  const int64_t nwaves = (int64_t)gridDim.x * (kBlock / 64);
  constexpr int kWaveRows = 16;
  for (int64_t i0 = ((int64_t)blockIdx.x * (kBlock / 64) + wave) * kWaveRows; i0 < cnt; i0 += nwaves * kWaveRows)
  for (int64_t i = i0; i < min(i0 + kWaveRows, cnt); ++i) {
    int64_t p = parent[i];
    bool stranger = p < 0 || p >= nwalkers;
    p = stranger ? 0 : p;
    int at[4];
#pragma unroll
    for (int q = 0; q < 4; ++q) at[q] = 2 * sorb * HP;
    int k = 0, nflip = 0;
#pragma unroll
    for (int w = 0; w < LEN; ++w) {
      const uint64_t xc = onv[i * LEN + w];
      uint64_t d = xc ^ walkers[p * LEN + w];
      nflip += __popcll(d);
#pragma unroll
      for (int t = 0; t < 4; ++t) {
        if (d && k < 4) {
          const int b = __builtin_ctzll(d);
          d &= d - 1;
          const int r = (2 * (64 * w + b) + (((xc >> b) & 1ull) ? 0 : 1)) * HP;
#pragma unroll
          for (int q = 0; q < 4; ++q)
            if (q == k) at[q] = r;
          ++k;
        }
      }
    }
    const auto from_scratch = [&]() {
      uint64_t ket[LEN];
#pragma unroll
      for (int w = 0; w < LEN; ++w) ket[w] = onv[i * LEN + w];
      Prod P2;
      double a2r, a2i;
      rbm_forward_row<LEN, FLAVOUR>(ket, sorb, H, W, hb, vb, P2, a2r, a2i);
      if (lane == 0) write_psi<FLAVOUR>(psi, i, P2, a2r, a2i);
    };
    if (stranger || nflip > 4) {
      from_scratch();
      continue;
    }
    const double *__restrict__ tp = table + (size_t)p * (size_t)(H + 2) * C;
    Prod P;
    for (int h = lane; h < H; h += 64) {
      double qr = tp[(size_t)h * C], qi = CPLX ? tp[(size_t)h * C + 1] : 0.0;
#pragma unroll
      for (int q = 0; q < 4; ++q) {
        const double fr = factors[(size_t)(at[q] + h) * C];
        if constexpr (CPLX) {
          const double fi = factors[(size_t)(at[q] + h) * C + 1];
          const double nr = qr * fr - qi * fi;
          qi = fma(qr, fi, qi * fr);
          qr = nr;
        } else {
          qr *= fr;
        }
      }
      if constexpr (CPLX) {
        const double u = 1.0 + qr;
        const double nr = P.re * u - P.im * qi;
        P.im = fma(P.re, qi, P.im * u);
        P.re = nr;
      } else {
        P.re *= 1.0 + qr;
      }
      P.renorm();
    }
#pragma unroll
    for (int d = 32; d > 0; d >>= 1) {
      const double orr = __shfl_xor(P.re, d), oi = CPLX ? __shfl_xor(P.im, d) : 0.0;
      const int oe = __shfl_xor(P.e2, d);
      if constexpr (CPLX) {
        const double nr = P.re * orr - P.im * oi;
        P.im = fma(P.re, oi, P.im * orr);
        P.re = nr;
      } else {
        P.re *= orr;
      }
      P.e2 += oe;
    }
    P.renorm();
    if (__ballot(!P.finite())) {
      from_scratch();
      continue;
    }
    if (lane == 0) {
      double axr = tp[(size_t)(H + 1) * C], axi = CPLX ? tp[(size_t)(H + 1) * C + 1] : 0.0;
      P.lin = tp[(size_t)H * C];
      P.ang = CPLX ? tp[(size_t)H * C + 1] : 0.0;
#pragma unroll
      for (int q = 0; q < 4; ++q) {
        P.lin += factors[(size_t)(at[q] + H) * C];
        axr += factors[(size_t)(at[q] + H + 1) * C];
        if constexpr (CPLX) {
          P.ang += factors[(size_t)(at[q] + H) * C + 1];
          axi += factors[(size_t)(at[q] + H + 1) * C + 1];
        }
      }
      write_psi<FLAVOUR>(psi, i, P, axr, axi);
    }
  }
}

}

using namespace pynqs;

extern "C" int pynqs_rbm_forward(const uint64_t *onv, int64_t n, int sorb, const double *weights, const double *hidden_bias,
                                 const double *visible_bias, int nhidden, int flavour, double *psi, void *stream) {
  pynqs::DeviceScope device_scope_(onv);
  if (n < 0 || n > 0x7fffffffll * kBlock || sorb < 1 || sorb > kMaxSorb || nhidden < 1) return set_error(PYNQS_EINVAL, "bad n/sorb/nhidden");
  if (flavour != PYNQS_RBM_REAL && flavour != PYNQS_RBM_TANH && flavour != PYNQS_RBM_PHASE && flavour != PYNQS_RBM_COMPLEX)
    return set_error(PYNQS_EINVAL, "bad flavour");
  if (n == 0) return PYNQS_OK;
  if (!onv || !weights || !hidden_bias || !psi) return set_error(PYNQS_EINVAL, "null pointer");
  const int len = (sorb - 1) / 64 + 1;
  const uint32_t grid = (uint32_t)((n + kBlock - 1) / kBlock);
  hipStream_t st = (hipStream_t)stream;
#define PYNQS_RF(F) hipLaunchKernelGGL((rbm_forward_kernel<LEN, F>), dim3(grid), dim3(kBlock), 0, st, onv, n, sorb, nhidden, weights, hidden_bias, visible_bias, psi)
  DISPATCH_LEN(len, {
    switch (flavour) {
      case PYNQS_RBM_REAL: PYNQS_RF(PYNQS_RBM_REAL); break;
      case PYNQS_RBM_TANH: PYNQS_RF(PYNQS_RBM_TANH); break;
      case PYNQS_RBM_PHASE: PYNQS_RF(PYNQS_RBM_PHASE); break;
      default: PYNQS_RF(PYNQS_RBM_COMPLEX); break;
    }
  });
#undef PYNQS_RF
  return check_launch("rbm_forward");
}

extern "C" int pynqs_jrbm_forward(const uint64_t *onv, int64_t n, int sorb, const double *weights, const double *hidden_bias,
                                  const double *visible_bias, const double *jastrow, int nhidden, double *psi, void *stream) {
  pynqs::DeviceScope device_scope_(onv);
  if (n < 0 || n > 0x7fffffffll * kBlock || sorb < 1 || sorb > kMaxSorb || nhidden < 1) return set_error(PYNQS_EINVAL, "bad n/sorb/nhidden");
  if (n == 0) return PYNQS_OK;
  if (!onv || !weights || !hidden_bias || !jastrow || !psi) return set_error(PYNQS_EINVAL, "null pointer");
  const int len = (sorb - 1) / 64 + 1;
  const uint32_t grid = (uint32_t)((n + kBlock - 1) / kBlock);
  DISPATCH_LEN(len, {
    hipLaunchKernelGGL((jrbm_forward_kernel<LEN>), dim3(grid), dim3(kBlock), 0, (hipStream_t)stream, onv, n, sorb, nhidden, weights, hidden_bias,
                       visible_bias, jastrow, psi);
  });
  return check_launch("jrbm_forward");
}

static size_t children_lds_bytes(int sorb, int nhidden, int flavour) {
  return (size_t)(2 * sorb + 1) * (size_t)children_hp(nhidden) * (flavour == PYNQS_RBM_COMPLEX ? 16 : 8);
}

static bool children_flavour_ok(int flavour) {
  return flavour == PYNQS_RBM_REAL || flavour == PYNQS_RBM_TANH || flavour == PYNQS_RBM_PHASE || flavour == PYNQS_RBM_COMPLEX;
}

extern "C" int pynqs_rbm_forward_children_supported(int sorb, int nhidden, int flavour) {
  if (sorb < 1 || sorb > kMaxSorb || nhidden < 1 || !children_flavour_ok(flavour)) return 0;
  return 1;
}
static bool children_table_in_lds(int sorb, int nhidden, int flavour) {
  static const int force = getenv("PYNQS_RBM_CHILDREN_WAVE") ? atoi(getenv("PYNQS_RBM_CHILDREN_WAVE")) : -1;
  return force != 1 && children_lds_bytes(sorb, nhidden, flavour) <= 64 * 1024;
}

extern "C" int64_t pynqs_rbm_children_table_bytes(int64_t nwalkers, int sorb, int nhidden, int flavour) {
  if (nwalkers < 0 || sorb < 1 || sorb > kMaxSorb || nhidden < 1 || !children_flavour_ok(flavour)) return -1;
  const int64_t c = flavour == PYNQS_RBM_COMPLEX ? 16 : 8;
  return nwalkers * (nhidden + 2) * c + (int64_t)children_lds_bytes(sorb, nhidden, flavour) + 8;
}

extern "C" int pynqs_rbm_children_prepare(const uint64_t *walkers, int64_t nwalkers, int sorb, const double *weights, const double *hidden_bias,
                                          const double *visible_bias, int nhidden, int flavour, void *table, void *stream) {
  pynqs::DeviceScope device_scope_(table);
  if (nwalkers < 0 || nwalkers > 0x7fffffffll * kBlock || sorb < 1 || sorb > kMaxSorb || nhidden < 1 || !children_flavour_ok(flavour))
    return set_error(PYNQS_EINVAL, "bad nwalkers/sorb/nhidden/flavour");
  if (!weights || !hidden_bias || !table || (nwalkers > 0 && !walkers)) return set_error(PYNQS_EINVAL, "null pointer");
  const bool cplx = flavour == PYNQS_RBM_COMPLEX;
  const int len = (sorb - 1) / 64 + 1;
  hipStream_t st = (hipStream_t)stream;
  double *parents = (double *)table;
  double *factors = parents + (size_t)nwalkers * (size_t)(nhidden + 2) * (cplx ? 2 : 1);
  const uint32_t gf = (uint32_t)(((2 * sorb + 1) * children_hp(nhidden) + kBlock - 1) / kBlock);
  if (cplx) hipLaunchKernelGGL((rbm_children_factors_kernel<true>), dim3(gf), dim3(kBlock), 0, st, sorb, nhidden, weights, visible_bias, factors);
  else hipLaunchKernelGGL((rbm_children_factors_kernel<false>), dim3(gf), dim3(kBlock), 0, st, sorb, nhidden, weights, visible_bias, factors);
  if (nwalkers > 0) {
    const dim3 grid((uint32_t)((nwalkers + kBlock - 1) / kBlock), (uint32_t)((nhidden + kParentChunk - 1) / kParentChunk));
    if (grid.y > 65535u) return set_error(PYNQS_EINVAL, "too many hidden units");
    DISPATCH_LEN(len, {
      if (cplx)
        hipLaunchKernelGGL((rbm_children_parents_kernel<LEN, true>), grid, dim3(kBlock), 0, st, walkers, nwalkers, sorb, nhidden, weights,
                           hidden_bias, visible_bias, factors, parents);
      else
        hipLaunchKernelGGL((rbm_children_parents_kernel<LEN, false>), grid, dim3(kBlock), 0, st, walkers, nwalkers, sorb, nhidden, weights,
                           hidden_bias, visible_bias, factors, parents);
    });
  }
  return check_launch("rbm_children_prepare");
}

extern "C" int pynqs_rbm_forward_children(const uint64_t *onv, int64_t n, const int32_t *count_dev, const int32_t *parent,
                                          const uint64_t *walkers, int64_t nwalkers, const void *table, int sorb, const double *weights,
                                          const double *hidden_bias, const double *visible_bias, int nhidden, int flavour, double *psi,
                                          void *stream) {
  pynqs::DeviceScope device_scope_(onv);
  if (n < 0 || n > 0x7fffffffll * kBlock || nwalkers < 0 || sorb < 1 || sorb > kMaxSorb || nhidden < 1) return set_error(PYNQS_EINVAL, "bad n/sorb/nhidden");
  if (!pynqs_rbm_forward_children_supported(sorb, nhidden, flavour))
    return set_error(PYNQS_EINVAL, "rbm_forward_children: bad flavour");
  if (n == 0) return PYNQS_OK;
  if (!onv || !parent || !walkers || !table || !psi || !weights || !hidden_bias || nwalkers == 0) return set_error(PYNQS_EINVAL, "null pointer");
  const int len = (sorb - 1) / 64 + 1;
  int64_t blocks = (n + kChildBlock - 1) / kChildBlock;
  if (blocks > 1024) blocks = 1024;
  const uint32_t grid = (uint32_t)blocks;
  const size_t lds = children_lds_bytes(sorb, nhidden, flavour);
  const double *parents = (const double *)table;
  const double *factors = parents + (size_t)nwalkers * (size_t)(nhidden + 2) * (flavour == PYNQS_RBM_COMPLEX ? 2 : 1);
  hipStream_t st = (hipStream_t)stream;
  const bool in_lds = children_table_in_lds(sorb, nhidden, flavour);
  int64_t wblocks = (n + (kBlock / 64) * 16 - 1) / ((kBlock / 64) * 16);
  if (wblocks > 256 * 32) wblocks = 256 * 32;
#define PYNQS_RC(F)                                                                                                                          \
  do {                                                                                                                                       \
    if (in_lds)                                                                                                                              \
      hipLaunchKernelGGL((rbm_forward_children_kernel<LEN, F>), dim3(grid), dim3(kChildBlock), lds, st, onv, n, count_dev, parent, walkers,  \
                         nwalkers, parents, factors, sorb, nhidden, weights, hidden_bias, visible_bias, psi);                                \
    else                                                                                                                                     \
      hipLaunchKernelGGL((rbm_forward_children_wave_kernel<LEN, F>), dim3((uint32_t)wblocks), dim3(kBlock), 0, st, onv, n, count_dev,        \
                         parent, walkers, nwalkers, parents, factors, sorb, nhidden, weights, hidden_bias, visible_bias, psi);               \
  } while (0)
  DISPATCH_LEN(len, {
    switch (flavour) {
      case PYNQS_RBM_REAL: PYNQS_RC(PYNQS_RBM_REAL); break;
      case PYNQS_RBM_TANH: PYNQS_RC(PYNQS_RBM_TANH); break;
      case PYNQS_RBM_PHASE: PYNQS_RC(PYNQS_RBM_PHASE); break;
      default: PYNQS_RC(PYNQS_RBM_COMPLEX); break;
    }
  });
#undef PYNQS_RC
  return check_launch("rbm_forward_children");
}
```

### pynqs_amd/csrc/kernels_rbm_grad.hip

```cpp
#include "detcore.h"
#include "launch.h"
#include "rbm_math.h"

namespace pynqs {

constexpr int kGradWalkers = 32;
constexpr int kGradHidden = 32;

template <int LEN, bool CPLX>
__global__ __launch_bounds__(kBlock) void rbm_grad_partial_kernel(const uint64_t *__restrict__ onv, int64_t n, int sorb, int H,
                                                                  const double *__restrict__ W, const double *__restrict__ hb,
                                                                  const double *__restrict__ vb, const double *__restrict__ prob,
                                                                  const double *__restrict__ eloc, bool eloc_cplx,
                                                                  const double *__restrict__ e_total, const double *__restrict__ pw,
                                                                  double *__restrict__ partial, int64_t stride) {
  constexpr int C = CPLX ? 2 : 1;
  __shared__ uint64_t xs[kGradWalkers][LEN];
  __shared__ double tc[kGradWalkers][kGradHidden + 1][C];
  __shared__ double cf[kGradWalkers][C];
  constexpr int NQ = kBlock / kGradWalkers;
  const int tid = threadIdx.x, w = tid % kGradWalkers, q = tid / kGradWalkers;
  const int64_t i = (int64_t)blockIdx.x * kGradWalkers + w;
  const bool valid = i < n;
  const int64_t row = valid ? i : n - 1;
  uint64_t ket[LEN];
#pragma unroll
  for (int k = 0; k < LEN; ++k) ket[k] = onv[row * LEN + k];
  double fr = 0.0, fi = 0.0;
  if (valid) {
    const double pr = prob[i], c = pw ? pw[i] : 1.0;
    const double er = eloc_cplx ? eloc[2 * i] : eloc[i], ei = eloc_cplx ? eloc[2 * i + 1] : 0.0;
    const double tr = e_total[0], ti = eloc_cplx ? e_total[1] : 0.0;
    fr = pr * (er - tr * c);
    fi = pr * (ei - ti * c);
  }
  if (q == 0) {
#pragma unroll
    for (int k = 0; k < LEN; ++k) xs[w][k] = ket[k];
    cf[w][0] = fr;
    if constexpr (CPLX) cf[w][1] = -fi;
  }
  double *__restrict__ out = partial + (int64_t)blockIdx.x * stride;
  double lre = 0.0, lim = 0.0;
  const int SP = sorb + 1;
  for (int h0 = 0; h0 < H; h0 += kGradHidden) {
    constexpr int HC = kGradHidden / NQ;
    double tr[HC], ti[HC];
#pragma unroll
    for (int j = 0; j < HC; ++j) {
      const int h = min(h0 + HC * q + j, H - 1);
      tr[j] = CPLX ? hb[2 * h] : hb[h];
      ti[j] = CPLX ? hb[2 * h + 1] : 0.0;
    }
    for (int o = 0; o < sorb; ++o) {
      const double x = pm1_of<LEN>(ket, o);
#pragma unroll
      for (int j = 0; j < HC; ++j) {
        const int h = min(h0 + HC * q + j, H - 1);
        if constexpr (CPLX) {
          tr[j] = fma(x, W[((size_t)h * sorb + o) * 2], tr[j]);
          ti[j] = fma(x, W[((size_t)h * sorb + o) * 2 + 1], ti[j]);
        } else {
          tr[j] = fma(x, W[(size_t)h * sorb + o], tr[j]);
        }
      }
    }
    if (h0) __syncthreads();
#pragma unroll
    for (int j = 0; j < HC; ++j) {
      const int hh = HC * q + j;
      const bool live = h0 + hh < H;
      const double ax = fabs(tr[j]), e = exp(-2.0 * ax), s = tr[j] < 0.0 ? -1.0 : 1.0;
      double yr, yi = 0.0;
      if constexpr (CPLX) {
        double sn, cs;
        sincos_mod(2.0 * ti[j], sn, cs);
        const double den = fma(2.0 * e, cs, fma(e, e, 1.0));
        yr = s * (1.0 - e * e) / den;
        yi = 2.0 * e * sn / den;
        if (live) {
          const double u = fma(e, cs, 1.0), v = -s * e * sn;
          lre += ax + 0.5 * log(u * u + v * v);
          lim += s * ti[j] + atan2(v, u);
        }
        tc[w][hh][0] = live ? yr * fr + yi * fi : 0.0;
        tc[w][hh][1] = live ? yi * fr - yr * fi : 0.0;
      } else {
        yr = s * (1.0 - e) / (1.0 + e);
        if (live) lre += ax + log1p(e);
        tc[w][hh][0] = live ? yr * fr : 0.0;
      }
    }
    __syncthreads();
    const int nout = min(kGradHidden, H - h0) * SP;
    for (int k = tid; k < nout; k += kBlock) {
      const int hh = k / SP, o = k - hh * SP;
      double ar = 0.0, ai = 0.0;
      if (o < sorb) {
        const int word = o >> 6, bit = o & 63;
#pragma unroll 8
        for (int v = 0; v < kGradWalkers; ++v) {
          const bool up = (xs[v][word] >> bit) & 1ull;
          const double a = tc[v][hh][0];
          ar += up ? a : -a;
          if constexpr (CPLX) { const double b = tc[v][hh][1]; ai += up ? b : -b; }
        }
      } else {
#pragma unroll 8
        for (int v = 0; v < kGradWalkers; ++v) {
          ar += tc[v][hh][0];
          if constexpr (CPLX) ai += tc[v][hh][1];
        }
      }
      const int64_t at = (int64_t)(h0 + hh) * SP + o;
      out[C * at] = ar;
      if constexpr (CPLX) out[C * at + 1] = ai;
    }
  }
  const int64_t off_vb = (int64_t)H * SP;
  for (int o = tid; o < sorb; o += kBlock) {
    const int word = o >> 6, bit = o & 63;
    double ar = 0.0, ai = 0.0;
    for (int v = 0; v < kGradWalkers; ++v) {
      const bool up = (xs[v][word] >> bit) & 1ull;
      ar += up ? cf[v][0] : -cf[v][0];
      if constexpr (CPLX) ai += up ? cf[v][1] : -cf[v][1];
    }
    out[C * (off_vb + o)] = ar;
    if constexpr (CPLX) out[C * (off_vb + o) + 1] = ai;
  }
  if (vb && q == 0) {
    for (int o = 0; o < sorb; ++o) {
      const double x = pm1_of<LEN>(ket, o);
      lre = fma(x, CPLX ? vb[2 * o] : vb[o], lre);
      if constexpr (CPLX) lim = fma(x, vb[2 * o + 1], lim);
    }
  }
  __syncthreads();
  double *lr = &tc[0][0][0];
  lr[(q * kGradWalkers + w) * 2] = lre;
  lr[(q * kGradWalkers + w) * 2 + 1] = lim;
  __syncthreads();
  if (tid < 64) {
    double l = 0.0;
    if (q == 0) {
      double re = 0.0, im = 0.0;
#pragma unroll
      for (int k = 0; k < NQ; ++k) { re += lr[(k * kGradWalkers + w) * 2]; im += lr[(k * kGradWalkers + w) * 2 + 1]; }
      im -= 6.283185307179586476925 * rint(im * 0.15915494309189533577);
      l = valid ? 2.0 * (re * fr + im * fi) : 0.0;
    }
#pragma unroll
    for (int d = 32; d > 0; d >>= 1) l += __shfl_xor(l, d);
    if (tid == 0) out[C * (off_vb + sorb)] = l;
  }
}

template <bool CPLX>
__global__ __launch_bounds__(kBlock) void rbm_grad_reduce_kernel(const double *__restrict__ partial, int64_t stride, int ngroups, int sorb, int H,
                                                                 double *__restrict__ gw, double *__restrict__ ghb, double *__restrict__ gvb,
                                                                 double *__restrict__ loss) {
  constexpr int C = CPLX ? 2 : 1;
  constexpr int NS = kBlock / 64;
  __shared__ double part[NS][64][2];
  const int SP = sorb + 1;
  const int64_t nout = (int64_t)H * SP + sorb + 1;
  const int lane = threadIdx.x & 63, slice = threadIdx.x >> 6;
  const int64_t k = (int64_t)blockIdx.x * 64 + lane;
  const int per = (ngroups + NS - 1) / NS, g_lo = min(slice * per, ngroups), g_hi = min(g_lo + per, ngroups);
  double re = 0.0, im = 0.0;
  if (k < nout) {
    constexpr int RU = 16;
    for (int g0 = g_lo; g0 < g_hi; g0 += RU) {
      double vr[RU], vi[RU];
#pragma unroll
      for (int u = 0; u < RU; ++u) {
        const bool in = g0 + u < g_hi;
        vr[u] = in ? partial[(int64_t)(g0 + u) * stride + C * k] : 0.0;
        vi[u] = CPLX && in ? partial[(int64_t)(g0 + u) * stride + C * k + 1] : 0.0;
      }
#pragma unroll
      for (int u = 0; u < RU; ++u) { re += vr[u]; im += vi[u]; }
    }
  }
  part[slice][lane][0] = re;
  part[slice][lane][1] = im;
  __syncthreads();
  if (slice != 0 || k >= nout) return;
  re = 0.0; im = 0.0;
#pragma unroll
  for (int sl = 0; sl < NS; ++sl) { re += part[sl][lane][0]; im += part[sl][lane][1]; }
  if (k == nout - 1) {
    if (loss) loss[0] = re;
    return;
  }
  double *dst;
  int64_t at;
  if (k < (int64_t)H * SP) {
    const int64_t h = k / SP;
    const int o = (int)(k - h * SP);
    if (o < sorb) { dst = gw; at = h * sorb + o; }
    else { dst = ghb; at = h; }
  } else {
    dst = gvb; at = k - (int64_t)H * SP;
  }
  if (!dst) return;
  dst[C * at] = 2.0 * re;
  if constexpr (CPLX) dst[C * at + 1] = -2.0 * im;
}

static inline int64_t grad_stride(int sorb, int H, bool cplx) {
  return ((int64_t)H * (sorb + 1) + sorb + 1) * (cplx ? 2 : 1);
}

}

using namespace pynqs;

extern "C" int64_t pynqs_rbm_grad_workspace(int64_t n, int sorb, int nhidden, int flavour) {
  if (n < 0 || sorb < 1 || sorb > kMaxSorb || nhidden < 1 || (flavour != PYNQS_RBM_REAL && flavour != PYNQS_RBM_COMPLEX)) return -1;
  const int64_t groups = (n + kGradWalkers - 1) / kGradWalkers;
  return groups * grad_stride(sorb, nhidden, flavour == PYNQS_RBM_COMPLEX) * 8;
}

extern "C" int pynqs_rbm_grad(const uint64_t *onv, int64_t n, int sorb, const double *weights, const double *hidden_bias,
                              const double *visible_bias, int nhidden, int flavour, const double *prob, const double *eloc,
                              int eloc_is_complex, const double *e_total, const double *pow, double *grad_weights, double *grad_hidden_bias,
                              double *grad_visible_bias, double *loss, void *workspace, void *stream) {
  pynqs::DeviceScope device_scope_(onv);
  if (n < 0 || n > 0x7fffffffll * kGradWalkers || sorb < 1 || sorb > kMaxSorb || nhidden < 1) return set_error(PYNQS_EINVAL, "bad n/sorb/nhidden");
  if (flavour != PYNQS_RBM_REAL && flavour != PYNQS_RBM_COMPLEX) return set_error(PYNQS_EINVAL, "rbm_grad: flavour must be PYNQS_RBM_REAL or PYNQS_RBM_COMPLEX");
  if (!weights || !hidden_bias || !grad_weights || !grad_hidden_bias || (n > 0 && (!onv || !prob || !eloc || !e_total || !workspace)))
    return set_error(PYNQS_EINVAL, "null pointer");
  const bool cplx = flavour == PYNQS_RBM_COMPLEX;
  const int len = (sorb - 1) / 64 + 1;
  const int64_t groups = (n + kGradWalkers - 1) / kGradWalkers, stride = grad_stride(sorb, nhidden, cplx);
  hipStream_t st = (hipStream_t)stream;
  double *partial = (double *)workspace;
  if (groups > 0) {
#define PYNQS_RG(C)                                                                                                                          \
  hipLaunchKernelGGL((rbm_grad_partial_kernel<LEN, C>), dim3((uint32_t)groups), dim3(kBlock), 0, st, onv, n, sorb, nhidden, weights, hidden_bias, \
                     visible_bias, prob, eloc, eloc_is_complex != 0, e_total, pow, partial, stride)
    DISPATCH_LEN(len, {
      if (cplx) PYNQS_RG(true);
      else PYNQS_RG(false);
    });
#undef PYNQS_RG
  }
  const int64_t nout = (int64_t)nhidden * (sorb + 1) + sorb + 1;
  const uint32_t g2 = (uint32_t)((nout + 63) / 64);
  if (cplx)
    hipLaunchKernelGGL((rbm_grad_reduce_kernel<true>), dim3(g2), dim3(kBlock), 0, st, partial, stride, (int)groups, sorb, nhidden, grad_weights,
                       grad_hidden_bias, grad_visible_bias, loss);
  else
    hipLaunchKernelGGL((rbm_grad_reduce_kernel<false>), dim3(g2), dim3(kBlock), 0, st, partial, stride, (int)groups, sorb, nhidden, grad_weights,
                       grad_hidden_bias, grad_visible_bias, loss);
  return check_launch("rbm_grad");
}
```

### pynqs_amd/csrc/kernels_reduce_onepass.hip

```cpp
#include "detcore.h"
#include "launch.h"
#include "plan.h"
#include "plan_dev.h"
#include "plan_tiles.h"
#include "reduce_common.h"
#include "reduce_list.h"

namespace pynqs {




template <int LEN, typename T, bool SAMPLED>
struct KeepSink {
  T eps;
  uint32_t chunk, nchunks, tS;
  int64_t seg_base;
  volatile uint32_t *run;
  WinnerList wl;
  uint32_t *bufc;
  T *bufh;
  volatile uint32_t *dstat;
  double *tsum;
  uint32_t *kept_total;
// ... 373 lines not shown
    double before = 0.0, total = 0.0;
    for (int w = 0; w < kBlock / 64; ++w) {
      if (w < wave) before += s_part[w];
      total += s_part[w];
    }
    double run = before + incl - local;
    for (uint32_t i = b0; i < b1; ++i) { run += tsum[i]; tsum[i] = run; }
    __syncthreads();
    const double Srow = total;
    if (tid == 0 && o.row_sum) o.row_sum[walker] = Srow;
    const uint64_t key = op_mix64((o.seed_dev ? seed + *o.seed_dev : seed) ^ op_mix64(slot));
    if (Srow > 0.0) {
      for (uint32_t k = tid; k < nsample; k += kBlock) {
        const uint64_t r = op_mix64(key ^ op_mix64(0xffffffff00000000ull | k));
        const double target = (double)(r >> 11) * 0x1.0p-53 * Srow;
        uint32_t lo = 0, hi = max_tiles;
        while (lo < hi) {
          const uint32_t mid = (lo + hi) >> 1;
          if (tsum[mid] > target) hi = mid; else lo = mid + 1;
        }
        if (lo >= max_tiles) lo = max_tiles - 1;
        while (lo > 0 && !(tsum[lo] > tsum[lo - 1])) --lo;
        atomicAdd(&dinfo[lo], 1u);
      }
    }
    __syncthreads();
    uint32_t lsum = 0;
    for (uint32_t i = b0; i < b1; ++i) lsum += dinfo[i];
    uint32_t iscan = lsum;
#pragma unroll
    for (int d = 1; d < 64; d <<= 1) {
      const uint32_t ov = __shfl_up(iscan, d);
      if (lane >= d) iscan += ov;
    }
    if (lane == 63) s_parti[wave] = iscan;
    __syncthreads();
    uint32_t ibefore = 0;
    for (int w = 0; w < wave; ++w) ibefore += s_parti[w];
    uint32_t off = ibefore + iscan - lsum;
    for (uint32_t i = b0; i < b1; ++i) {
      const uint32_t c = dinfo[i];
      dinfo[i] = (off << 16) | c;
      off += c;
    }
    if (tid == 0) next_tile = 0;
    __syncthreads();
    unsigned char *mine = reinterpret_cast<unsigned char *>(dinfo) + (((size_t)max_tiles * 4 + 15) & ~(size_t)15) + (size_t)wave * kDrawLdsPerWave;
    DrawLds S;
    S.prefix = reinterpret_cast<double *>(mine);
    S.run = reinterpret_cast<volatile double *>(mine + (size_t)kOneTileCols * 8);
    S.cs = reinterpret_cast<uint32_t *>(mine + (size_t)kOneTileCols * 8 + 8);
    S.hits = S.cs + kOneTileCols;
    S.ncols = reinterpret_cast<volatile uint32_t *>(S.hits + kOneTileCols);
    DrawSink<LEN, T> sink{eps, S, &p, &L, &wk, dinfo, Srow / (double)nsample, key, (int64_t)walker * nsample, o, wl, 0xffffffffu};
    visit_tiles<LEN, T>(p, pl, L, nocc, plan, wk, nchunks, chunk, chunk_len, 0u, &next_tile, sink);
    sink.flush();
    flush_winner_list<LEN, T>(o, wl, &wl_base, p, L, wk);
  }
}


template <int LEN, typename T, bool SAMPLED, bool CACHED = false>
__global__ __launch_bounds__(kBlock) __attribute__((amdgpu_waves_per_eu(8, 8)))
void reduce_onepass_list_kernel(const uint64_t *__restrict__ bra, SDParams p, PlanLayout pl, uint32_t nchunks, uint32_t chunk_len, uint32_t max_tiles,
                                const T *__restrict__ plan, T eps, uint32_t nsample, uint64_t seed, uint32_t P, OnepassOut<T> o) {
  static_assert(CACHED || !SAMPLED, "the re-enumerating form has its own kernel");
  reduce_onepass_list_body<LEN, T, SAMPLED, CACHED>(bra, p, pl, nchunks, chunk_len, max_tiles, plan, eps, nsample, seed, P, o);
}

template <int LEN, typename T, bool SAMPLED = false, bool GTILE = false>
__global__ __launch_bounds__(kBlock) void reduce_onepass_list_flush_kernel(const uint64_t *__restrict__ bra, SDParams p, PlanLayout pl, uint32_t nchunks,
                                                                           uint32_t chunk_len, uint32_t max_tiles, const T *__restrict__ plan, T eps,
                                                                           uint32_t nsample, uint64_t seed, uint32_t P, OnepassOut<T> o) {
  reduce_onepass_list_body<LEN, T, SAMPLED, false, true, GTILE>(bra, p, pl, nchunks, chunk_len, max_tiles, plan, eps, nsample, seed, P, o);
}

template <int LEN, typename T, bool GTILE = false>
__global__ __launch_bounds__(kBlock) void reduce_onepass_list_redraw_kernel(const uint64_t *__restrict__ bra, SDParams p, PlanLayout pl, uint32_t nchunks,
                                                                            uint32_t chunk_len, uint32_t max_tiles, const T *__restrict__ plan, T eps,
                                                                            uint32_t nsample, uint64_t seed, uint32_t P, OnepassOut<T> o) {
  reduce_onepass_list_body<LEN, T, true, false, false, GTILE>(bra, p, pl, nchunks, chunk_len, max_tiles, plan, eps, nsample, seed, P, o);
}

template <typename T, bool CPLX>
__global__ __launch_bounds__(kBlock) void reduce_contract_kernel(int64_t nbatch, uint32_t nchunks, uint32_t fixed, uint32_t cap_d,
                                                                 uint32_t nsample, const int32_t *__restrict__ rec_col,
                                                                 const T *__restrict__ rec_w, const int32_t *__restrict__ rec_link,
                                                                 const int32_t *__restrict__ seg_count, const int32_t *__restrict__ srec_col,
                                                                 const T *__restrict__ srec_w, const int32_t *__restrict__ srec_link,
                                                                 const int32_t *__restrict__ dedup_i32, int slot_i32, int row_off, uint32_t ucap,
                                                                 const double *__restrict__ psi_u, const double *__restrict__ psi_t, int divide,
                                                                 double *__restrict__ eloc, double *__restrict__ psi_x) {
  const int lane = threadIdx.x & 63;
  const int64_t walker = (int64_t)blockIdx.x * (kBlock / 64) + (threadIdx.x >> 6);
  if (walker >= nbatch) return;
  double ar = 0.0, ai = 0.0, xr = 0.0, xi = 0.0;
  bool bad = false;
  auto amp = [&](int32_t link, double &re, double &im) {
    const double *src;
    int64_t at;
    if (link >= kDirectLink) {
      src = psi_u; at = link - kDirectLink;
      if ((uint32_t)at >= ucap) { bad = true; re = im = 0.0; return; }
    } else if (link >= 0) {
      if (!dedup_i32) { bad = true; re = im = 0.0; return; }
      const int32_t row = dedup_i32[(int64_t)link * slot_i32 + row_off];
      if (row < 0 || (uint32_t)row >= ucap) { bad = true; re = im = 0.0; return; }
      src = psi_u; at = row;
    } else if (link <= -2) {
      src = psi_t; at = -2 - (int64_t)link;
    } else { bad = true; re = im = 0.0; return; }
    if constexpr (CPLX) { re = src[2 * at]; im = src[2 * at + 1]; }
    else { re = src[at]; im = 0.0; }
  };
  auto visit = [&](int32_t col, double w, int32_t link) {
    if (col < 0) return;
    double re, im;
    amp(link, re, im);
    ar += w * re; ai += w * im;
    if (col == 0) { xr = re; xi = im; }
  };
  const int64_t stride = (int64_t)fixed + cap_d;
  for (uint32_t c = 0; c < nchunks; ++c) {
    const int64_t seg = walker * nchunks + c, base = seg * stride;
    const uint32_t kept = (uint32_t)seg_count[seg];
    if (kept > cap_d) bad = true;
    const uint32_t nslots = fixed + min(kept, cap_d);
    for (uint32_t i = lane; i < nslots; i += 64) visit(rec_col[base + i], (double)rec_w[base + i], rec_link[base + i]);
  }
  for (uint32_t i = lane; i < nsample; i += 64) {
    const int64_t at = walker * nsample + i;
    visit(srec_col[at], (double)srec_w[at], srec_link[at]);
  }
#pragma unroll
  for (int d = 32; d > 0; d >>= 1) {
    ar += __shfl_xor(ar, d); ai += __shfl_xor(ai, d);
    xr += __shfl_xor(xr, d); xi += __shfl_xor(xi, d);
  }
  const bool anybad = __ballot(bad) != 0;
  if (lane == 0) {
    if (anybad) { ar = ai = __builtin_nan(""); }
    if constexpr (CPLX) {
      if (divide) scaled_cdiv(ar, ai, xr, xi, ar, ai);
      eloc[2 * walker] = ar;
      eloc[2 * walker + 1] = ai;
      psi_x[2 * walker] = xr; psi_x[2 * walker + 1] = xi;
    } else {
      eloc[walker] = divide ? ar / xr : ar;
      psi_x[walker] = xr;
    }
  }
}

}

using namespace pynqs;

static int onepass_geometry(int64_t nbatch, const SDParams &p, bool sampled, uint32_t *nchunks, uint32_t *chunk_len, uint32_t *max_tiles,
                            uint32_t *fixed) {
  const uint32_t ncomb = p.nsd + 1;
  if (sampled) {
    *nchunks = 1;
    *chunk_len = (ncomb + 255u) & ~255u;
  } else {
    plan_chunks(nbatch, ncomb, nchunks, chunk_len);
  }
  *max_tiles = max_tiles_per_chunk(p, *nchunks, *chunk_len);
  const uint32_t tS_all = (p.d1 + kSinglesPerTile - 1) / kSinglesPerTile;
  *fixed = kFixedHead + ((tS_all + *nchunks - 1) / *nchunks) * kSinglesPerTile;
  return 0;
}

static size_t onepass_static_lds(int) { return 16 + (kBlock / 64) * 4 + (kBlock / 64 + 1) * 12 + 64; }

extern "C" int pynqs_reduce_onepass_geometry(int64_t nbatch, int sorb, int nele, int noA, int noB, int eps_sample, int64_t *out4) {
  SDParams p;
  PlanLayout pl;
  if (!out4) return set_error(PYNQS_EINVAL, "null pointer");
  if (!make_sd_params(sorb, nele, noA, noB, &p) || !make_plan_layout(sorb, &pl)) return set_error(PYNQS_EINVAL, "bad sorb/noA/noB (even sorb in [2, 192])");
  if (nbatch < 0 || nbatch > 0x7fffffffll || eps_sample < 0 || eps_sample > 65535) return set_error(PYNQS_EINVAL, "bad nbatch / eps_sample (at most 65535 draws)");
  uint32_t nchunks, chunk_len, max_tiles, fixed;
  onepass_geometry(nbatch, p, eps_sample > 0, &nchunks, &chunk_len, &max_tiles, &fixed);
  const int len = (sorb - 1) / 64 + 1;
  const int64_t slots = out4[2];
  out4[0] = nbatch * (int64_t)nchunks;
  out4[1] = fixed;
  out4[2] = slots > 0 ? slots * dedup_slot_words(len) * 8 : 0;
  const bool lookback = onepass_lds(p, 8, max_tiles, eps_sample > 0, winner_list_cap(eps_sample)) + onepass_static_lds(len) <= 160 * 1024;
  const bool flushing = eps_sample > 0 && p.nsd + 1 > 65536 &&
                        onepass_list_lds(p, 8, max_tiles, true, 2048, (uint32_t)eps_sample, false, true) + 256 + onepass_static_lds(len) <= 160 * 1024;
  out4[3] = lookback || flushing ? 1 : 0;
  return PYNQS_OK;
}

constexpr uint32_t kLongRow = 65536;
struct OnepassForm {
  uint32_t P;
  bool use_list, use_cache, use_flush, use_gtile;
  size_t lds;
  bool use_split = false;
  bool use_row32 = false;
};
static OnepassForm onepass_form(const SDParams &p, size_t esz, uint32_t max_tiles, uint32_t fixed, uint64_t cap_doubles, int eps_sample,
                                bool have_cache, uint32_t chunk_len, bool no_table, bool have_tile_scratch = false, bool have_row_f32 = false) {
  static const int list_env = getenv("PYNQS_OP_LIST") ? atoi(getenv("PYNQS_OP_LIST")) : -1;
  static const int cache_env = getenv("PYNQS_OP_CACHE") ? atoi(getenv("PYNQS_OP_CACHE")) : -1;
  static const int flush_env = getenv("PYNQS_OP_FLUSH") ? atoi(getenv("PYNQS_OP_FLUSH")) : -1;
  const bool sampled = eps_sample > 0;
  const uint64_t seg_cap = (uint64_t)fixed + cap_doubles;
  OnepassForm f;
  f.P = 64;
  while (f.P < seg_cap && f.P < (1u << 20)) f.P <<= 1;
  const bool want_cache = sampled && have_cache && cache_env != 0;
  const bool gtile = sampled && !want_cache && have_tile_scratch;
  const size_t lds_list = onepass_list_lds(p, esz, max_tiles, sampled, f.P, (uint32_t)eps_sample, want_cache, gtile);
  const bool list_fits = seg_cap <= 2048 && lds_list + 256 <= 160 * 1024;
  f.use_list = list_env == 0 ? false : (list_fits && (list_env == 1 || seg_cap <= 1024 || p.nsd + 1 > kLongRow));
  f.use_cache = want_cache && f.use_list;
  f.use_gtile = gtile && f.use_list;
  f.lds = f.use_list ? lds_list : onepass_lds(p, esz, max_tiles, sampled, winner_list_cap(eps_sample));
  static const int split_env = getenv("PYNQS_OP_SPLIT") ? atoi(getenv("PYNQS_OP_SPLIT")) : -1;
  if (sampled && have_row_f32 && split_env != 0 && list_env != 0 && seg_cap <= 1024 && reduce_draw_supported(p, eps_sample)) {
    const uint32_t slots = ((uint32_t)seg_cap + 1u) & ~1u;
    const size_t lds_a = onepass_list_lds(p, esz, max_tiles, true, slots, (uint32_t)eps_sample, false, false, true);
    if (lds_a + 256 <= 160 * 1024) {
      f.P = slots;
      f.use_list = true; f.use_split = true; f.use_cache = f.use_gtile = f.use_flush = false; f.lds = lds_a;
      return f;
    }
  }
  const bool gtile_f = sampled && have_tile_scratch;
  const uint32_t flush_P = flush_list_slots((p.sorb - 1) / 64 + 1, sampled);
  const size_t lds_flush = onepass_list_lds(p, esz, max_tiles, sampled, flush_P, (uint32_t)eps_sample, false, gtile_f);
  const bool long_row = p.nsd + 1 > kLongRow;
  f.use_flush = !f.use_list && flush_env != 0 && lds_flush + 256 <= 160 * 1024 &&
                (long_row || flush_env == 1 || no_table || cap_doubles * 10 <= (uint64_t)chunk_len);
  if (f.use_flush) { f.use_gtile = gtile_f; f.use_cache = false; }
  if (f.use_flush) { f.P = flush_P; f.lds = lds_flush; }
  static const int row32_env = getenv("PYNQS_OP_ROW32") ? atoi(getenv("PYNQS_OP_ROW32")) : -1;
  const bool from_list = f.use_list && !f.use_cache && flush_env != 0;
  if ((f.use_flush || from_list) && sampled && have_row_f32 && row32_env != 0 && row32_fits(esz, flush_P, (uint32_t)eps_sample, gtile_f)) {
    const size_t lds_r = onepass_list_lds(p, esz, max_tiles, true, flush_P, (uint32_t)eps_sample, false, gtile_f, false, true);
    const size_t wg_old = (size_t)160 * 1024 / ((f.use_flush ? lds_flush : f.lds) + 512), wg_new = (size_t)160 * 1024 / (lds_r + 512);
    if (lds_r + 256 <= 160 * 1024 && (row32_env == 1 || wg_new > wg_old || (uint64_t)eps_sample * 8 >= max_tiles)) {
      f.use_row32 = true; f.use_flush = true; f.use_list = false; f.use_cache = false; f.use_gtile = gtile_f; f.P = flush_P; f.lds = lds_r;
    }
  }
  return f;
}

extern "C" int64_t pynqs_reduce_onepass_tile_scratch_bytes(int64_t nbatch, int sorb, int nele, int noA, int noB, int eps_sample) {
  SDParams p;
  PlanLayout pl;
  if (!make_sd_params(sorb, nele, noA, noB, &p) || !make_plan_layout(sorb, &pl) || nbatch < 0 || nbatch > 0x7fffffffll || eps_sample < 0 || eps_sample > 65535) {
    set_error(PYNQS_EINVAL, "bad arguments");
    return -1;
  }
  if (eps_sample == 0) return 0;
  uint32_t nchunks, chunk_len, max_tiles, fixed;
  onepass_geometry(nbatch, p, true, &nchunks, &chunk_len, &max_tiles, &fixed);
  return (int64_t)((size_t)nbatch * tile_scratch_stride(max_tiles));
}

extern "C" int pynqs_reduce_onepass_list_capacity(int64_t nbatch, int sorb, int nele, int noA, int noB, int dtype, int eps_sample,
                                                  int with_row_cache, int without_table, int64_t *cap_doubles) {
  SDParams p;
  PlanLayout pl;
  if (!cap_doubles) return set_error(PYNQS_EINVAL, "null pointer");
  if (!make_sd_params(sorb, nele, noA, noB, &p) || !make_plan_layout(sorb, &pl)) return set_error(PYNQS_EINVAL, "bad sorb/noA/noB (even sorb in [2, 192])");
  if (nbatch < 0 || nbatch > 0x7fffffffll || eps_sample < 0 || eps_sample > 65535 || (dtype != PYNQS_F32 && dtype != PYNQS_F64))
    return set_error(PYNQS_EINVAL, "bad nbatch / eps_sample / dtype");
  uint32_t nchunks, chunk_len, max_tiles, fixed;
  onepass_geometry(nbatch, p, eps_sample > 0, &nchunks, &chunk_len, &max_tiles, &fixed);
  const size_t esz = dtype == PYNQS_F64 ? 8 : 4;
  auto listed = [&](uint64_t cap) {
    const OnepassForm f = onepass_form(p, esz, max_tiles, fixed, cap, eps_sample, with_row_cache != 0, chunk_len, without_table != 0,
                                       eps_sample > 0 && with_row_cache == 0);
    return (f.use_list || f.use_flush) && f.lds + onepass_static_lds(0) <= 160 * 1024;
  };
  *cap_doubles = -1;
  if (listed((uint64_t)1 << 29)) { *cap_doubles = ((int64_t)1 << 30) - 1; return PYNQS_OK; }
  for (uint32_t seg = 2048; seg >= 128; seg >>= 1) {
    if (seg < fixed) break;
    if (listed(seg - fixed)) { *cap_doubles = (int64_t)(seg - fixed); break; }
  }
  if ((int64_t)(chunk_len / 10) > *cap_doubles && listed(chunk_len / 10)) *cap_doubles = chunk_len / 10;
  return PYNQS_OK;
}

extern "C" int pynqs_reduce_onepass_wants_row_f32(int64_t nbatch, int sorb, int nele, int noA, int noB, int dtype, int eps_sample, int64_t cap_doubles,
                                                  int with_tile_scratch, int without_table) {
  SDParams p;
  PlanLayout pl;
  if (!make_sd_params(sorb, nele, noA, noB, &p) || !make_plan_layout(sorb, &pl) || nbatch < 0 || nbatch > 0x7fffffffll || eps_sample < 0 ||
      eps_sample > 65535 || cap_doubles < 0 || (dtype != PYNQS_F32 && dtype != PYNQS_F64)) {
    set_error(PYNQS_EINVAL, "bad arguments");
    return -1;
  }
  if (eps_sample == 0) return 0;
  uint32_t nchunks, chunk_len, max_tiles, fixed;
  onepass_geometry(nbatch, p, true, &nchunks, &chunk_len, &max_tiles, &fixed);
  const size_t esz = dtype == PYNQS_F64 ? 8 : 4;
  const OnepassForm f = onepass_form(p, esz, max_tiles, fixed, (uint64_t)cap_doubles, eps_sample, false, chunk_len, without_table != 0, false, true);
  if (f.use_split) return 1;
  const OnepassForm g = with_tile_scratch ? onepass_form(p, esz, max_tiles, fixed, (uint64_t)cap_doubles, eps_sample, false, chunk_len, without_table != 0, true, true) : f;
  return g.use_row32 ? 2 : 0;
}

extern "C" int64_t pynqs_reduce_onepass_row_f32_elements(int64_t nbatch, int sorb, int nele, int noA, int noB) {
  SDParams p;
  if (!make_sd_params(sorb, nele, noA, noB, &p) || nbatch < 0 || nbatch > 0x7fffffffll) {
    set_error(PYNQS_EINVAL, "bad arguments");
    return -1;
  }
  return (int64_t)((size_t)nbatch * draw_row_stride(p.nsd + 1));
}

extern "C" int pynqs_reduce_onepass(const uint64_t *bra, int64_t nbatch, int sorb, int nele, int noA, int noB, const void *plan, int dtype,
                                    double eps, int eps_sample, uint64_t seed, const pynqs_reduce_io *io, void *stream) {
  pynqs::DeviceScope device_scope_(bra);
  SDParams p;
  PlanLayout pl;
  if (!make_sd_params(sorb, nele, noA, noB, &p) || !make_plan_layout(sorb, &pl)) return set_error(PYNQS_EINVAL, "bad sorb/noA/noB (even sorb in [2, 192])");
  if (nbatch < 0 || nbatch > 0x7fffffffll || (dtype != PYNQS_F32 && dtype != PYNQS_F64)) return set_error(PYNQS_EINVAL, "bad nbatch/dtype");
  if (eps_sample < 0 || eps_sample > 65535) return set_error(PYNQS_EINVAL, "eps_sample must be in [0, 65535]");
  if (!io) return set_error(PYNQS_EINVAL, "null pointer");
  const bool sampled = eps_sample > 0;
  if (!io->counters || !io->uniq_onv || !io->rec_col || !io->rec_w || !io->rec_link || !io->seg_count ||
      (sampled && (!io->srec_col || !io->srec_w || !io->srec_link)))
    return set_error(PYNQS_EINVAL, "null pointer");
  if (io->cap_unique < 1 || io->cap_unique >= (1ll << 30) || io->cap_doubles < 0 || io->cap_doubles >= (1ll << 30) ||
      (io->dedup_table && (io->dedup_slots < 64 || (io->dedup_slots & (io->dedup_slots - 1)) || io->dedup_slots > (1ll << 30) ||
                           2 * io->cap_unique > io->dedup_slots)))
    return set_error(PYNQS_EINVAL, "bad capacities (dedup_slots: power of two >= 2 * cap_unique)");
  if (io->pm1_dtype != PYNQS_F32 && io->pm1_dtype != PYNQS_F64) return set_error(PYNQS_EINVAL, "bad pm1_dtype");
  if (io->lut_table && io->lut_nkeys < 0) return set_error(PYNQS_EINVAL, "bad lut_nkeys");
  hipStream_t st = (hipStream_t)stream;
  const int len = (sorb - 1) / 64 + 1;
  if (hipMemsetAsync(io->counters, 0, 16, st) != hipSuccess) return check_launch("memset");
  if (io->dedup_table &&
      hipMemsetAsync(io->dedup_table, 0xFF, (size_t)io->dedup_slots * dedup_slot_words(len) * 8, st) != hipSuccess) return check_launch("memset");
  if (nbatch == 0) return PYNQS_OK;
  if (!bra || !plan) return set_error(PYNQS_EINVAL, "null pointer");
  uint32_t nchunks, chunk_len, max_tiles, fixed;
  onepass_geometry(nbatch, p, sampled, &nchunks, &chunk_len, &max_tiles, &fixed);
  const uint64_t grid = (uint64_t)nbatch * nchunks;
  if (grid > 0x7fffffffull) return set_error(PYNQS_EINVAL, "grid too large");
  if (grid * ((uint64_t)fixed + (uint64_t)io->cap_doubles) > 0x7fffffffull * 16ull) return set_error(PYNQS_EINVAL, "record arrays too large");
  const size_t esz = dtype == PYNQS_F64 ? 8 : 4;
  const bool have_tiles = io->tile_scratch != nullptr && io->tile_scratch_bytes >= (int64_t)((size_t)nbatch * tile_scratch_stride(max_tiles));
  const OnepassForm form = onepass_form(p, esz, max_tiles, fixed, (uint64_t)io->cap_doubles, eps_sample, io->row_cache != nullptr, chunk_len,
                                        io->dedup_table == nullptr, have_tiles, io->row_f32 != nullptr);
  const uint32_t P = form.P;
  const bool use_list = form.use_list || form.use_flush, use_cache = form.use_cache, use_flush = form.use_flush, use_gtile = form.use_gtile;
  const bool use_split = form.use_split, use_row32 = form.use_row32;
  const size_t lds = form.lds;
  if (lds + onepass_static_lds(len) > 160 * 1024) return set_error(PYNQS_EINVAL, "row too long for the fused form (LDS): use the multi-pass entry points");
  if (!io->dedup_table && !use_list)
    return set_error(PYNQS_EINVAL, "no de-duplication table: only the LIST forms run without one (cap_doubles <= pynqs_reduce_onepass_list_capacity)");
  static const bool verbose = getenv("PYNQS_OP_VERBOSE") != nullptr;
  if (verbose)
    fprintf(stderr, "pynqs_reduce_onepass: %s form%s, LDS %zu bytes per workgroup (walker tables %zu, max_tiles %u, list P %u), %u chunk(s) per walker\n",
            use_split ? "LIST + float32 row copy + sorted draws" : use_row32 ? (use_gtile ? "flushing LIST + float32 row copy (tile sums in global memory)" : "flushing LIST + float32 row copy") : use_flush ? "flushing LIST" : use_list ? (use_gtile ? "LIST (tile sums in global memory)" : "LIST") : "look-back", use_cache ? " with row cache" : "", lds, (size_t)lds_fixed_bytes(p), max_tiles, P, nchunks);
  const double eps_eff = (sampled && !(eps > 0.0)) ? __builtin_inf() : eps;
  if (use_split) return launch_reduce_rowout(bra, nbatch, p, pl, chunk_len, max_tiles, plan, dtype, eps_eff, eps_sample, seed, P, lds, io, fixed, st);
  if (use_row32) return launch_reduce_flush_row32(bra, nbatch, p, pl, chunk_len, max_tiles, plan, dtype, eps_eff, eps_sample, seed, P, lds, io, fixed, use_gtile, st);
#define PYNQS_OP_LAUNCH(TT, SM)                                                                                                      \
  do {                                                                                                                               \
    auto kfn = use_flush ? (use_gtile ? reduce_onepass_list_flush_kernel<LEN, TT, SM, SM> : reduce_onepass_list_flush_kernel<LEN, TT, SM, false>) \
             : use_list ? (use_cache ? reduce_onepass_list_kernel<LEN, TT, SM, SM>                                                   \
                                     : (SM ? (use_gtile ? reduce_onepass_list_redraw_kernel<LEN, TT, true> : reduce_onepass_list_redraw_kernel<LEN, TT, false>) \
                                           : reduce_onepass_list_kernel<LEN, TT, false, false>)) \
                        : reduce_onepass_kernel<LEN, TT, SM>;                                                                        \
    if (lds > 64 * 1024 && hipFuncSetAttribute(reinterpret_cast<const void *>(kfn), hipFuncAttributeMaxDynamicSharedMemorySize,      \
                                               (int)lds) != hipSuccess)                                                              \
      return check_launch("hipFuncSetAttribute");                                                                                   \
    hipLaunchKernelGGL(kfn, dim3((uint32_t)grid), dim3(kBlock), lds, st, bra, p, pl, nchunks, chunk_len, max_tiles, (const TT *)plan, \
                       (TT)eps_eff, (uint32_t)eps_sample, seed, use_list ? P : winner_list_cap(eps_sample), make_out<TT>(io, len, fixed, use_gtile ? max_tiles : 0u));                \
  } while (0)
  DISPATCH_LEN(len, {
    if (dtype == PYNQS_F64) { if (sampled) PYNQS_OP_LAUNCH(double, true); else PYNQS_OP_LAUNCH(double, false); }
    else { if (sampled) PYNQS_OP_LAUNCH(float, true); else PYNQS_OP_LAUNCH(float, false); }
  });
#undef PYNQS_OP_LAUNCH
  return check_launch("reduce_onepass");
}

extern "C" int pynqs_reduce_contract(int64_t nbatch, int sorb, int nele, int noA, int noB, int dtype, int eps_sample,
                                     const pynqs_reduce_io *io, const double *psi_unique, const double *psi_table, int psi_is_complex,
                                     int divide, double *eloc, double *psi_x, void *stream) {
  pynqs::DeviceScope device_scope_(eloc);
  SDParams p;
  if (!make_sd_params(sorb, nele, noA, noB, &p)) return set_error(PYNQS_EINVAL, "bad sorb/noA/noB");
  if (nbatch < 0 || nbatch > 0x7fffffffll || (dtype != PYNQS_F32 && dtype != PYNQS_F64) || eps_sample < 0 || eps_sample > 65535)
    return set_error(PYNQS_EINVAL, "bad nbatch/dtype/eps_sample");
  if (nbatch == 0) return PYNQS_OK;
  if (!io || !io->rec_col || !io->rec_w || !io->rec_link || !io->seg_count || !psi_unique || !eloc || !psi_x ||
      (eps_sample > 0 && (!io->srec_col || !io->srec_w || !io->srec_link)) || (io->lut_table && !psi_table))
    return set_error(PYNQS_EINVAL, "null pointer");
  uint32_t nchunks, chunk_len, max_tiles, fixed;
  onepass_geometry(nbatch, p, eps_sample > 0, &nchunks, &chunk_len, &max_tiles, &fixed);
  const int len = (sorb - 1) / 64 + 1;
  hipStream_t st = (hipStream_t)stream;
  const uint32_t grid = (uint32_t)((nbatch + kBlock / 64 - 1) / (kBlock / 64));
#define PYNQS_CT_LAUNCH(TT, CX)                                                                                                          \
  hipLaunchKernelGGL((reduce_contract_kernel<TT, CX>), dim3(grid), dim3(kBlock), 0, st, nbatch, nchunks, fixed, (uint32_t)io->cap_doubles, \
                     (uint32_t)eps_sample, io->rec_col, (const TT *)io->rec_w, io->rec_link, io->seg_count, io->srec_col,                \
                     (const TT *)io->srec_w, io->srec_link, (const int32_t *)io->dedup_table, dedup_slot_words(len) * 2,                 \
                     dedup_row_offset(len), (uint32_t)io->cap_unique, psi_unique, psi_table, divide, eloc, psi_x)
  if (dtype == PYNQS_F64) { if (psi_is_complex) PYNQS_CT_LAUNCH(double, true); else PYNQS_CT_LAUNCH(double, false); }
  else { if (psi_is_complex) PYNQS_CT_LAUNCH(float, true); else PYNQS_CT_LAUNCH(float, false); }
#undef PYNQS_CT_LAUNCH
  return check_launch("reduce_contract");
}

#ifdef PYNQS_OP_STAMPS
extern "C" int pynqs_debug_stamps(unsigned long long *out) {
  return (int)hipMemcpyFromSymbol(out, HIP_SYMBOL(pynqs::g_stamps), sizeof(unsigned long long) * 8192 * 16);
}
#endif
```

### pynqs_amd/grad.py

```python
from __future__ import annotations

import contextlib
from typing import Union

import torch
from torch import Tensor, nn

from .distributed import all_reduce_packed, get_world_size
from .public_function import split_batch_idx


def grad(nqs: nn.Module, states: Tensor, state_prob: Tensor, eloc: Tensor, e_total: Union[complex, float, Tensor],
         extra_psi_pow: Union[Tensor, float] = 1.0, dtype=torch.double, AD_MAX_DIM: int = -1, empty_shard_state: "Tensor | None" = None) -> Tensor:
    device = states.device
    dim = states.size(0)
    loss_sum = torch.zeros(1, device=device, dtype=torch.double)
    batch = dim if (AD_MAX_DIM == -1 or AD_MAX_DIM > dim) else AD_MAX_DIM
    ends = split_batch_idx(dim, batch) if dim > 0 else []

    def batch_loss_backward(begin: int, end: int) -> None:
        nonlocal loss_sum
        state = states[begin:end]
        if state.is_floating_point():
            state = state.requires_grad_()
# ... 15 lines not shown
            begin = end
    if ends:
        batch_loss_backward(begin, ends[-1])
    elif get_world_size() > 1 and hasattr(nqs, "no_sync"):
        dummy = empty_shard_state if empty_shard_state is not None else states.new_zeros((1,) + tuple(states.shape[1:]))
        out = nqs(dummy.reshape((1,) + tuple(states.shape[1:])).to(states.dtype)).to(dtype).sum()
        if not bool(torch.isfinite(torch.view_as_real(out) if out.is_complex() else out).all()):
            raise ValueError("empty shard: the ansatz is not finite on the dummy configuration; pass empty_shard_state=<a valid state>")
        (out.real * 0.0).backward()
    return all_reduce_packed([loss_sum], get_world_size())[0]


class GraphedGrad:

    def __init__(self, nqs: nn.Module, n: int, sorb: int, dtype=torch.double, device=None, use_pow: bool = False, warmup: int = 3,
                 check_nan: "bool | None" = None) -> None:
        m = getattr(nqs, "module", nqs)
        self.module, self.dtype = m, dtype
        self.check_nan = (not dtype.is_complex) if check_nan is None else check_nan
        self.params = [p for p in m.parameters() if p.requires_grad]
        self.ptrs = [p.data_ptr() for p in self.params]
        dev = device if device is not None else self.params[0].device
        rdt = dtype.to_real() if dtype.is_complex else dtype
        self.states = torch.zeros((n, sorb), dtype=rdt, device=dev)
        self.prob = torch.zeros(n, dtype=rdt, device=dev)
        self.eloc = torch.zeros(n, dtype=dtype, device=dev)
        self.e_total = torch.zeros((), dtype=dtype, device=dev)
        self.pow = torch.ones(n, dtype=dtype, device=dev) if use_pow else None
        self.flat = torch.zeros(sum(p.numel() for p in self.params), dtype=self.params[0].dtype, device=dev)
        assert all(p.dtype == self.flat.dtype for p in self.params), "one parameter dtype per module"
        views, o = [], 0
        for p in self.params:
            views.append(self.flat[o:o + p.numel()].view_as(p))
            o += p.numel()
        self.views = views
        self.loss = torch.zeros(1, dtype=torch.double, device=dev)
        self.events = None
        self.graph = torch.cuda.CUDAGraph()
        side = torch.cuda.Stream(device=dev)
        side.wait_stream(torch.cuda.current_stream(dev))
        with torch.cuda.stream(side):
            for _ in range(warmup):
                self._body()
        torch.cuda.current_stream(dev).wait_stream(side)
        with torch.cuda.graph(self.graph, capture_error_mode="thread_local"):
            self._body()

    def _body(self) -> None:
        log_psi = self.module(self.states).to(self.dtype).log()
        c = 1.0 if self.pow is None else self.pow
        loss = 2 * (log_psi.conj() * (self.eloc - self.e_total * c) * self.prob).sum().real
        grads = torch.autograd.grad(loss, self.params)
        for v, g in zip(self.views, grads):
            v.copy_(g)
        self.loss.copy_(loss.detach().reshape(1))

    def _check_params(self) -> None:
        cur = [p for p in self.module.parameters() if p.requires_grad]
        if len(cur) != len(self.params) or any(a is not b or a.data_ptr() != ptr for a, b, ptr in zip(cur, self.params, self.ptrs)):
            raise RuntimeError("GraphedGrad: the module's parameters were replaced or re-allocated since the graph was captured (the replay "
                               "would read the old storage and fill the old tensors' .grad); build a new GraphedGrad")

    def __call__(self, states: Tensor, state_prob: Tensor, eloc: Tensor, e_total, extra_psi_pow=1.0) -> Tensor:
        self._check_params()
        self.states.copy_(states)
        self.prob.copy_(state_prob.real if state_prob.is_complex() else state_prob)
        self.eloc.copy_(eloc)
        self.e_total.copy_((e_total if isinstance(e_total, Tensor) else torch.as_tensor(e_total)).reshape(()))
        if self.pow is not None:
            self.pow.copy_(extra_psi_pow)
        self.graph.replay()
        if self.check_nan and bool(torch.isnan(self.loss).any()):
            for p in self.params:
                p.grad = None
            raise ValueError("There are negative numbers in the log-psi, please use complex128")
        ws = get_world_size()
        ev = None
        if self.events is not None:
            ev = [torch.cuda.Event(enable_timing=True) for _ in range(2)]
            ev[0].record()
        if ws > 1:
            import torch.distributed as dist

            dist.all_reduce(self.flat, dist.ReduceOp.SUM)
            self.flat.div_(ws)
        if ev is not None:
            ev[1].record()
            self.events.append(ev)
        for p, v in zip(self.params, self.views):
            p.grad = v
        return all_reduce_packed([self.loss], ws)[0]


class FusedRbmGrad:

    def __init__(self, nqs: nn.Module, sorb: int) -> None:
        from . import _native as N
        from .rbm import ComplexRBM, RealRBM

        m = getattr(nqs, "module", nqs)
        if isinstance(m, ComplexRBM):
            self.flavour, self.names = N.RBM_COMPLEX, ("params_weights", "params_hidden_bias", "params_visible_bias")
        elif isinstance(m, RealRBM) and getattr(m, "rbm_type", "real") == "real":
            self.flavour, self.names = N.RBM_REAL, ("weights", "hidden_bias", "visible_bias")
        else:
            raise ValueError("FusedRbmGrad: the module is not a real (rbm_type 'real') or complex-parameter RBM")
        self.N, self.module, self.sorb = N, m, sorb
        params = [getattr(m, nm) for nm in self.names]
        if any(p.dtype != torch.float64 or not p.is_cuda for p in params):
            raise ValueError("FusedRbmGrad: float64 parameters on the GPU")
        dev = params[0].device
        self.H = params[0].size(0)
        self.shapes = [p.shape for p in params]
        self.flat = torch.zeros(sum(p.numel() for p in params) + 1, dtype=torch.float64, device=dev)
        self.views, o = [], 0
        for p in params:
            self.views.append(self.flat[o:o + p.numel()].view_as(p))
            o += p.numel()
        self.loss = self.flat[o:o + 1]
        self.work = None
        self.events = None

    @property
    def params(self):
        ps = [getattr(self.module, nm) for nm in self.names]
        if any(p.dtype != torch.float64 or p.device != self.flat.device for p in ps):
            raise ValueError("FusedRbmGrad: float64 parameters on the GPU")
        if [p.shape for p in ps] != self.shapes:
            raise ValueError(f"FusedRbmGrad: parameter shapes changed since construction ({self.shapes} -> {[p.shape for p in ps]})")
        return ps

    def __call__(self, onv: Tensor, state_prob: Tensor, eloc: Tensor, e_total, extra_psi_pow=1.0) -> Tensor:
        N, dev = self.N, self.flat.device
        n = onv.size(0)
        if onv.dtype != torch.uint8 or onv.dim() != 2 or onv.size(1) != 8 * ((self.sorb - 1) // 64 + 1) or onv.device != dev:
            raise ValueError("FusedRbmGrad: walkers as packed onv uint8[n, 8 len] on the parameters' device")
        cplx = eloc.is_complex()
        prob = (state_prob.real if state_prob.is_complex() else state_prob).to(torch.float64).contiguous()
        el = eloc.to(torch.complex128 if cplx else torch.float64).contiguous()
        et = (e_total if isinstance(e_total, Tensor) else torch.as_tensor(e_total)).to(device=dev, dtype=el.dtype).reshape(1).contiguous()
        pw = None
        if isinstance(extra_psi_pow, Tensor):
            if extra_psi_pow.is_complex():
                raise ValueError("FusedRbmGrad: extra_psi_pow must be real")
            pw = extra_psi_pow.to(torch.float64).contiguous()
        elif float(extra_psi_pow) != 1.0:
            pw = torch.full((n,), float(extra_psi_pow), dtype=torch.float64, device=dev)
        need = N.lib().pynqs_rbm_grad_workspace(n, self.sorb, self.H, self.flavour)
        if self.work is None or self.work.numel() * 8 < need:
            self.work = torch.empty(max(need // 8, 1), dtype=torch.float64, device=dev)
        params = self.params
        W, hb, vb = (p.detach().contiguous() for p in params)
        gw, ghb, gvb = self.views
        N.check(N.lib().pynqs_rbm_grad(onv.contiguous().data_ptr(), n, self.sorb, W.data_ptr(), hb.data_ptr(), vb.data_ptr(), self.H, self.flavour,
                                       prob.data_ptr(), el.data_ptr(), int(cplx), et.data_ptr(), pw.data_ptr() if pw is not None else None,
                                       gw.data_ptr(), ghb.data_ptr(), gvb.data_ptr(), self.loss.data_ptr(), self.work.data_ptr(),
                                       torch.cuda.current_stream(dev).cuda_stream), "pynqs_rbm_grad")
        ws = get_world_size()
        ev = None
        if self.events is not None:
            ev = [torch.cuda.Event(enable_timing=True) for _ in range(2)]
            ev[0].record()
        if ws > 1:
            import torch.distributed as dist

            dist.all_reduce(self.flat, dist.ReduceOp.SUM)
            self.flat.div_(ws)
        if ev is not None:
            ev[1].record()
            self.events.append(ev)
        for p, v in zip(params, self.views):
            p.grad = v
        return self.loss * ws if ws > 1 else self.loss.clone()


class FusedJastrowRbmGrad:

    names = ("weights", "hidden_bias", "visible_bias", "jastrow")

    def __init__(self, nqs: nn.Module, sorb: int) -> None:
        from . import _native as N
        from .rbm import JastrowRBM

        m = getattr(nqs, "module", nqs)
        if not isinstance(m, JastrowRBM):
            raise ValueError("FusedJastrowRbmGrad: the module is not a pynqs_amd.rbm.JastrowRBM")
        self.N, self.module, self.sorb = N, m, sorb
        params = [getattr(m, nm) for nm in self.names]
        if any(p.dtype != torch.float64 or not p.is_cuda for p in params):
            raise ValueError("FusedJastrowRbmGrad: float64 parameters on the GPU")
        if params[0].size(1) != sorb:
            raise ValueError(f"FusedJastrowRbmGrad: the module has {params[0].size(1)} orbitals, not {sorb}")
        dev = params[0].device
        self.H = params[0].size(0)
        self.shapes = [p.shape for p in params]
        self.flat = torch.zeros(sum(p.numel() for p in params) + 1, dtype=torch.float64, device=dev)
        self.views, o = [], 0
        for p in params:
            self.views.append(self.flat[o:o + p.numel()].view_as(p))
            o += p.numel()
        self.loss = self.flat[o:o + 1]
        self.loss_jastrow = torch.zeros(1, dtype=torch.float64, device=dev)
        self.work = None
        self.events = None

    @property
    def params(self):
        ps = [getattr(self.module, nm) for nm in self.names]
        if any(p.dtype != torch.float64 or p.device != self.flat.device for p in ps):
            raise ValueError("FusedJastrowRbmGrad: float64 parameters on the GPU")
        if [p.shape for p in ps] != self.shapes:
            raise ValueError(f"FusedJastrowRbmGrad: parameter shapes changed since construction ({self.shapes} -> {[p.shape for p in ps]})")
        return ps

    def __call__(self, onv: Tensor, state_prob: Tensor, eloc: Tensor, e_total, extra_psi_pow=1.0) -> Tensor:
        N, dev = self.N, self.flat.device
        n = onv.size(0)
        if onv.dtype != torch.uint8 or onv.dim() != 2 or onv.size(1) != 8 * ((self.sorb - 1) // 64 + 1) or onv.device != dev:
            raise ValueError("FusedJastrowRbmGrad: walkers as packed onv uint8[n, 8 len] on the parameters' device")
        if eloc.is_complex():
            raise ValueError("FusedJastrowRbmGrad: the amplitude is real: a real local energy")
        prob = (state_prob.real if state_prob.is_complex() else state_prob).to(torch.float64).contiguous()
        el = eloc.to(torch.float64).contiguous()
        et = (e_total if isinstance(e_total, Tensor) else torch.as_tensor(e_total)).to(device=dev, dtype=torch.float64).reshape(1).contiguous()
        pw = None
        if isinstance(extra_psi_pow, Tensor):
            if extra_psi_pow.is_complex():
                raise ValueError("FusedJastrowRbmGrad: extra_psi_pow must be real")
            pw = extra_psi_pow.to(torch.float64).contiguous()
        elif float(extra_psi_pow) != 1.0:
            pw = torch.full((n,), float(extra_psi_pow), dtype=torch.float64, device=dev)
        lib = N.lib()
        need = max(lib.pynqs_rbm_grad_workspace(n, self.sorb, self.H, N.RBM_REAL), lib.pynqs_jastrow_grad_workspace(n, self.sorb))
        if self.work is None or self.work.numel() * 8 < need:
            self.work = torch.empty(max(need // 8, 1), dtype=torch.float64, device=dev)
        params = self.params
        W, hb, vb, M = (p.detach().contiguous() for p in params)
        gw, ghb, gvb, gm = self.views
        x = onv.contiguous()
        st = torch.cuda.current_stream(dev).cuda_stream
        pwp = pw.data_ptr() if pw is not None else None
        N.check(lib.pynqs_rbm_grad(x.data_ptr(), n, self.sorb, W.data_ptr(), hb.data_ptr(), vb.data_ptr(), self.H, N.RBM_REAL, prob.data_ptr(),
                                   el.data_ptr(), 0, et.data_ptr(), pwp, gw.data_ptr(), ghb.data_ptr(), gvb.data_ptr(), self.loss.data_ptr(),
                                   self.work.data_ptr(), st), "pynqs_rbm_grad")
        N.check(lib.pynqs_jastrow_grad(x.data_ptr(), n, self.sorb, M.data_ptr(), prob.data_ptr(), el.data_ptr(), et.data_ptr(), pwp, gm.data_ptr(),
                                       self.loss_jastrow.data_ptr(), self.work.data_ptr(), st), "pynqs_jastrow_grad")
        self.loss += self.loss_jastrow
        ws = get_world_size()
        ev = None
        if self.events is not None:
            ev = [torch.cuda.Event(enable_timing=True) for _ in range(2)]
            ev[0].record()
        if ws > 1:
            import torch.distributed as dist

            dist.all_reduce(self.flat, dist.ReduceOp.SUM)
            self.flat.div_(ws)
        if ev is not None:
            ev[1].record()
            self.events.append(ev)
        for p, v in zip(params, self.views):
            p.grad = v
        return self.loss * ws if ws > 1 else self.loss.clone()
```

### pynqs_amd/stats.py

```python
from __future__ import annotations

from typing import Optional, Tuple

import torch
from torch import Tensor

from .distributed import all_reduce_packed, get_world_size


def _wdot(x: Tensor, p: Tensor) -> Tensor:
    if torch.is_complex(x):
        return torch.complex(torch.dot(x.real, p), torch.dot(x.imag, p))
    return torch.dot(x, p)


def dist_mean(x: Tensor, prob: Tensor, world_size: int = 1) -> Tensor:
    assert x.dim() == 1 and prob.dim() == 1
    return all_reduce_packed([_wdot(x, prob)], world_size)[0]


def dist_var(x: Tensor, prob: Tensor, world_size: int = 1) -> Tuple[Tensor, Tensor]:
    mean = dist_mean(x, prob, world_size)
    corr = mean - x
    var = all_reduce_packed([(corr * corr.conj() * prob).sum()], world_size)[0]
    return mean, var


def dist_stats(x: Tensor, prob: Tensor, counts: Optional[int] = None, world_size: int = 1):
    mean, var = dist_var(x, prob, world_size)
    sd = torch.sqrt(var)
    if counts is None:
        n = torch.tensor([float(x.size(0))], dtype=torch.float64, device=x.device)
        counts = all_reduce_packed([n], 1)[0].item()
    se = sd / counts**0.5
    return mean, var, sd, se


_WS: dict = {}


def _moments(x: Tensor, prob: Tensor) -> Tensor:
    if x.is_cuda and prob.is_cuda and prob.dtype == torch.float64 and x.dtype in (torch.float64, torch.complex128) and x.dim() == 1:
        from . import _native as N

        dev = x.device
        ws = _WS.get(dev)
        if ws is None:
            ws = _WS[dev] = torch.zeros(N.lib().pynqs_moments_workspace() // 8, dtype=torch.float64, device=dev)
        xc, pc = x.contiguous(), prob.contiguous()
        N.check(N.lib().pynqs_weighted_moments(xc.data_ptr(), int(x.is_complex()), pc.data_ptr(), x.numel(), ws.data_ptr(),
                                               torch.cuda.current_stream(dev).cuda_stream), "pynqs_weighted_moments")
        return ws[:4]
    w = _wdot(x, prob)
    z = torch.zeros((), dtype=prob.dtype, device=x.device)
    return torch.stack([w.real if torch.is_complex(w) else w, w.imag if torch.is_complex(w) else z,
                        torch.dot((x * x.conj()).real, prob), prob.sum()]).to(torch.float64)


def dist_stats_moments(x: Tensor, prob: Tensor, counts: Optional[int] = None, world_size: int = 1):
    m = _moments(x, prob)
    if counts is None:
        counts = x.size(0) * get_world_size()
    if m.is_cuda:
        import torch.distributed as dist

        from . import _native as N

        if get_world_size() > 1:
            dist.all_reduce(m, dist.ReduceOp.SUM)
        out = torch.empty(6, dtype=torch.float64, device=m.device)
        N.check(N.lib().pynqs_stats_finish(m.data_ptr(), 1.0 / world_size, float(counts), out.data_ptr(),
                                           torch.cuda.current_stream(m.device).cuda_stream), "pynqs_stats_finish")
        mean = torch.view_as_complex(out[0:2]).reshape(()) if torch.is_complex(x) else out[0]
        return mean, out[2], out[3], out[4]
    m = all_reduce_packed([m], world_size)[0]
    mean = torch.complex(m[0], m[1]) if torch.is_complex(x) else m[0]
    var = (m[2] - (m[0] * m[0] + m[1] * m[1]) * (2.0 - m[3])).clamp_min(0)
    if counts is None:
        counts = x.size(0) * get_world_size()
    sd = torch.sqrt(var)
    return mean, var, sd, sd / counts**0.5


def dist_stats_onepass(x: Tensor, prob: Tensor, counts: Optional[int] = None, world_size: int = 1):
    one = torch.ones((), dtype=prob.dtype, device=x.device)
    vals = [_wdot(x, prob), torch.dot((x * x.conj()).real, prob), prob.sum() * one]
    if counts is None:
        vals.append(torch.tensor(float(x.size(0)), dtype=prob.dtype, device=x.device) * get_world_size())
    red = all_reduce_packed([v.to(torch.complex128) if torch.is_complex(vals[0]) else v for v in vals], world_size)
    mean, m2, psum = red[0], red[1].real if torch.is_complex(red[1]) else red[1], red[2]
    var = (m2 - (mean * mean.conj()).real * (2.0 - (psum.real if torch.is_complex(psum) else psum))).to(vals[1].dtype)
    if counts is None:
        counts = float((red[3].real if torch.is_complex(red[3]) else red[3]).item())
    sd = torch.sqrt(var.clamp_min(0))
    return mean, var, sd, sd / counts**0.5


class operator_statistics:

    def __init__(self, x: Tensor, prob: Tensor, counts: Optional[int] = None, operator: Optional[str] = None) -> None:
        self.world_size = get_world_size()
        self.operator = operator if operator is not None else "O"
        mean, var, sd, se = dist_stats(x, prob, counts, self.world_size)
        self.stats_dict = {"mean": mean, "var": var, "sd": sd, "se": se}

    def __getitem__(self, key: str) -> Tensor:
        return self.stats_dict[key]

    def to_dict(self):
        return self.stats_dict

    def __repr__(self) -> str:
        m, se, var = self["mean"], self["se"], self["var"]
        return f"<{self.operator}> = {m.real:.9E} ± {se.real:.3E} [σ² = {var.real:.3E}]"
```

Before: 9.529 million.

## Fuse stats finish, grad loss copy, children prep stamping and dedup clear kernel

Several independent launch-reduction changes. The weighted-moments kernel can now compute the final statistics in its last block, and the RBM gradient reduce writes a copy of the loss directly instead of needing a separate clone. The dedup-table memsets are replaced with a single clear kernel that also zeroes the counters, and the children-table prepare/forward path gains a stamp argument that appears to restructure the factor table build. Each change aims to cut small kernel launches and host round trips per step, at the cost of more code paths and env-controlled fallbacks.

```diff
diff --git a/include/pynqs_amd.h b/include/pynqs_amd.h
--- a/include/pynqs_amd.h
+++ b/include/pynqs_amd.h
@@ -138,6 +138,8 @@
 int64_t pynqs_moments_workspace(void);
 int pynqs_stats_finish(const double *moments, double inv_world, double counts, double *out5, void *stream);
 int pynqs_weighted_moments(const double *x, int is_complex, const double *prob, int64_t n, void *workspace, void *stream);
+int pynqs_weighted_moments_finish(const double *x, int is_complex, const double *prob, int64_t n, void *workspace, double inv_world,
+                                  double counts, double *out5, void *stream);
 
 int64_t pynqs_reduce_tiles(int64_t nbatch, int sorb, int nele, int noA, int noB);
 int pynqs_reduce_count(const uint64_t *bra, int64_t nbatch, int sorb, int nele, int noA, int noB,
@@ -209,12 +211,24 @@
                                const double *hidden_bias, const double *visible_bias, int nhidden, int flavour, double *psi,
                                void *stream);
 int pynqs_rbm_forward_children_supported(int sorb, int nhidden, int flavour);
+int pynqs_rbm_children_prepare_stamped(const uint64_t *walkers, int64_t nwalkers, int sorb, const double *weights,
+                                       const double *hidden_bias, const double *visible_bias, int nhidden, int flavour, uint64_t stamp,
+                                       void *table, void *stream);
+int pynqs_rbm_forward_children_stamped(const uint64_t *onv, int64_t n, const int32_t *count_dev, const int32_t *parent,
+                                       const uint64_t *walkers, int64_t nwalkers, const void *table, int sorb, const double *weights,
+                                       const double *hidden_bias, const double *visible_bias, int nhidden, int flavour, uint64_t stamp,
+                                       double *psi, void *stream);
 
 int64_t pynqs_rbm_grad_workspace(int64_t n, int sorb, int nhidden, int flavour);
 int pynqs_rbm_grad(const uint64_t *onv, int64_t n, int sorb, const double *weights, const double *hidden_bias,
                    const double *visible_bias, int nhidden, int flavour, const double *prob, const double *eloc,
                    int eloc_is_complex, const double *e_total, const double *pow, double *grad_weights,
                    double *grad_hidden_bias, double *grad_visible_bias, double *loss, void *workspace, void *stream);
+int pynqs_rbm_grad_loss(const uint64_t *onv, int64_t n, int sorb, const double *weights, const double *hidden_bias,
+                        const double *visible_bias, int nhidden, int flavour, const double *prob, const double *eloc,
+                        int eloc_is_complex, const double *e_total, const double *pow, double *grad_weights,
+                        double *grad_hidden_bias, double *grad_visible_bias, double *loss, double *loss_copy, void *workspace,
+                        void *stream);
 
 #define PYNQS_SR_RHO 0
 #define PYNQS_SR_RHS2 1
diff --git a/pynqs_amd/C_extension.py b/pynqs_amd/C_extension.py
--- a/pynqs_amd/C_extension.py
+++ b/pynqs_amd/C_extension.py
@@ -1,5 +1,6 @@
 from __future__ import annotations
 
+import itertools
 import os
 import warnings
 import weakref
@@ -598,6 +599,9 @@
     return flav is not None and bool(N.lib().pynqs_rbm_forward_children_supported(sorb, num_hidden, flav))
 
 
+_CHILDREN_STAMP = itertools.count(1)
+
+
 def rbm_forward_children(onv: Tensor, parent: Tensor, walkers: Tensor, weights: Tensor, hidden_bias: Tensor, visible_bias: "Tensor | None",
                          sorb: int, rbm_type: str = "real", count: "Tensor | None" = None, out: "Tensor | None" = None) -> Tensor:
     _check_onv(onv, "onv", sorb, (2,))
@@ -611,12 +615,14 @@
     table = torch.empty(max(nbytes // 8, 1), dtype=torch.float64, device=dev)
     st = _stream(dev)
     wk = walkers.contiguous()
-    N.check(N.lib().pynqs_rbm_children_prepare(wk.data_ptr(), nw, sorb, W.data_ptr(), hb.data_ptr(), vb.data_ptr() if vb is not None else None,
-                                               H, flav, table.data_ptr(), st), "pynqs_rbm_children_prepare")
+    stamp = next(_CHILDREN_STAMP)
+    N.check(N.lib().pynqs_rbm_children_prepare_stamped(wk.data_ptr(), nw, sorb, W.data_ptr(), hb.data_ptr(), vb.data_ptr() if vb is not None else None,
+                                                       H, flav, stamp, table.data_ptr(), st), "pynqs_rbm_children_prepare_stamped")
     psi = out if out is not None else torch.empty(n, dtype=_rbm_dtype(rbm_type), device=dev)
-    N.check(N.lib().pynqs_rbm_forward_children(onv.contiguous().data_ptr(), n, count.data_ptr() if count is not None else None, parent.data_ptr(),
-                                               wk.data_ptr(), nw, table.data_ptr(), sorb, W.data_ptr(), hb.data_ptr(),
-                                               vb.data_ptr() if vb is not None else None, H, flav, psi.data_ptr(), st), "pynqs_rbm_forward_children")
+    N.check(N.lib().pynqs_rbm_forward_children_stamped(onv.contiguous().data_ptr(), n, count.data_ptr() if count is not None else None,
+                                                       parent.data_ptr(), wk.data_ptr(), nw, table.data_ptr(), sorb, W.data_ptr(), hb.data_ptr(),
+                                                       vb.data_ptr() if vb is not None else None, H, flav, stamp, psi.data_ptr(), st),
+            "pynqs_rbm_forward_children_stamped")
     return psi
 
 
diff --git a/pynqs_amd/_native.py b/pynqs_amd/_native.py
--- a/pynqs_amd/_native.py
+++ b/pynqs_amd/_native.py
@@ -61,6 +61,7 @@
     "pynqs_moments_workspace": (_i64, []),
     "pynqs_stats_finish": (_int, [_vp, _dbl, _dbl, _vp, _vp]),
     "pynqs_weighted_moments": (_int, [_vp, _int, _vp, _i64, _vp, _vp]),
+    "pynqs_weighted_moments_finish": (_int, [_vp, _int, _vp, _i64, _vp, _dbl, _dbl, _vp, _vp]),
     "pynqs_reduce_tiles": (_i64, [_i64, _int, _int, _int, _int]),
     "pynqs_reduce_count": (_int, [_vp, _i64, _int, _int, _int, _int, _vp, _int, _dbl, _vp, _vp]),
     "pynqs_reduce_count_sums": (_int, [_vp, _i64, _int, _int, _int, _int, _vp, _int, _dbl, _vp, _vp, _vp]),
@@ -91,8 +92,11 @@
     "pynqs_rbm_children_prepare": (_int, [_vp, _i64, _int, _vp, _vp, _vp, _int, _int, _vp, _vp]),
     "pynqs_rbm_forward_children": (_int, [_vp, _i64, _vp, _vp, _vp, _i64, _vp, _int, _vp, _vp, _vp, _int, _int, _vp, _vp]),
     "pynqs_rbm_forward_children_supported": (_int, [_int, _int, _int]),
+    "pynqs_rbm_children_prepare_stamped": (_int, [_vp, _i64, _int, _vp, _vp, _vp, _int, _int, C.c_uint64, _vp, _vp]),
+    "pynqs_rbm_forward_children_stamped": (_int, [_vp, _i64, _vp, _vp, _vp, _i64, _vp, _int, _vp, _vp, _vp, _int, _int, C.c_uint64, _vp, _vp]),
     "pynqs_rbm_grad_workspace": (_i64, [_i64, _int, _int, _int]),
     "pynqs_rbm_grad": (_int, [_vp, _i64, _int, _vp, _vp, _vp, _int, _int, _vp, _vp, _int, _vp, _vp, _vp, _vp, _vp, _vp, _vp, _vp]),
+    "pynqs_rbm_grad_loss": (_int, [_vp, _i64, _int, _vp, _vp, _vp, _int, _int, _vp, _vp, _int, _vp, _vp, _vp, _vp, _vp, _vp, _vp, _vp, _vp]),
     "pynqs_reduce_contract": (_int, [_i64, _int, _int, _int, _int, _int, _int, C.POINTER(ReduceIO), _vp, _vp, _int, _int, _vp, _vp, _vp]),    "pynqs_mcmc_rbm_supported": (_int, [_int, _int, _int]),
     "pynqs_mcmc_rbm": (_int, [_vp, _i64, _int, _int, _int, _vp, _int, _int, C.c_uint64, C.c_uint64, C.c_uint64, _int, _int, _vp, _vp, _vp, _vp]),
     "pynqs_rbm_sr_workspace": (_i64, [_i64, _int, _int, _int]),
diff --git a/pynqs_amd/csrc/kernels_gfmc.hip b/pynqs_amd/csrc/kernels_gfmc.hip
--- a/pynqs_amd/csrc/kernels_gfmc.hip
+++ b/pynqs_amd/csrc/kernels_gfmc.hip
@@ -136,9 +136,18 @@
 
 constexpr int kMomentBlocks = 128;
 
-template <bool CPLX>
+__device__ __forceinline__ void stats_finish(const double *m, double inv_world, double counts, double *__restrict__ out) {
+  const double re = m[0] * inv_world, im = m[1] * inv_world, m2 = m[2] * inv_world, ps = m[3] * inv_world;
+  double var = m2 - (re * re + im * im) * (2.0 - ps);
+  var = var > 0.0 ? var : 0.0;
+  const double sd = sqrt(var);
+  out[0] = re; out[1] = im; out[2] = var; out[3] = sd; out[4] = sd / sqrt(counts);
+}
+
+template <bool CPLX, bool FINISH>
 __global__ __launch_bounds__(kBlock) void moments_kernel(const double *__restrict__ x, const double *__restrict__ prob, int64_t n,
-                                                         double *__restrict__ out, unsigned int *__restrict__ done) {
+                                                         double *__restrict__ out, unsigned int *__restrict__ done, double inv_world,
+                                                         double counts, double *__restrict__ out5) {
   __shared__ double red[4][kBlock / 64];
   __shared__ bool last;
   const int tid = threadIdx.x, lane = tid & 63, wave = tid >> 6;
@@ -170,21 +179,20 @@
       double t = 0.0;
       for (unsigned b = 0; b < gridDim.x; ++b) t += out[4 * (1 + b) + tid];
       out[tid] = t;
+      if constexpr (FINISH) red[0][tid] = t;
     }
     if (tid == 0) *done = 0;
-  }
-}
-
-}
-
-namespace pynqs {
+    if constexpr (FINISH) {
+      __syncthreads();
+      if (tid == 0) stats_finish(&red[0][0], inv_world, counts, out5);
+    }
+  }
+}
+
 __global__ void stats_finish_kernel(const double *__restrict__ m, double inv_world, double counts, double *__restrict__ out) {
-  const double re = m[0] * inv_world, im = m[1] * inv_world, m2 = m[2] * inv_world, ps = m[3] * inv_world;
-  double var = m2 - (re * re + im * im) * (2.0 - ps);
-  var = var > 0.0 ? var : 0.0;
-  const double sd = sqrt(var);
-  out[0] = re; out[1] = im; out[2] = var; out[3] = sd; out[4] = sd / sqrt(counts);
-}
+  stats_finish(m, inv_world, counts, out);
+}
+
 }
 
 extern "C" int pynqs_stats_finish(const double *moments, double inv_world, double counts, double *out5, void *stream) {
@@ -196,17 +204,31 @@
 
 extern "C" int64_t pynqs_moments_workspace(void) { return 8 * 4 * (pynqs::kMomentBlocks + 1) + 8; }
 
-extern "C" int pynqs_weighted_moments(const double *x, int is_complex, const double *prob, int64_t n, void *workspace, void *stream) {
+static int weighted_moments_launch(const double *x, int is_complex, const double *prob, int64_t n, void *workspace, bool finish, double inv_world,
+                                   double counts, double *out5, void *stream) {
   pynqs::DeviceScope device_scope_(x);
   if (n < 0) return set_error(PYNQS_EINVAL, "bad n");
   if (!workspace || (n > 0 && (!x || !prob))) return set_error(PYNQS_EINVAL, "null pointer");
+  if (finish && (!out5 || !(counts > 0.0))) return set_error(PYNQS_EINVAL, "bad arguments");
   double *out = (double *)workspace;
   unsigned int *done = (unsigned int *)(out + 4 * (kMomentBlocks + 1));
   int64_t blocks = (n + kBlock - 1) / kBlock;
   if (blocks > kMomentBlocks) blocks = kMomentBlocks;
   if (blocks < 1) blocks = 1;
   hipStream_t st = (hipStream_t)stream;
-  if (is_complex) hipLaunchKernelGGL((moments_kernel<true>), dim3((uint32_t)blocks), dim3(kBlock), 0, st, x, prob, n, out, done);
-  else hipLaunchKernelGGL((moments_kernel<false>), dim3((uint32_t)blocks), dim3(kBlock), 0, st, x, prob, n, out, done);
+#define PYNQS_MK(C, F) \
+  hipLaunchKernelGGL((moments_kernel<C, F>), dim3((uint32_t)blocks), dim3(kBlock), 0, st, x, prob, n, out, done, inv_world, counts, out5)
+  if (finish) { if (is_complex) PYNQS_MK(true, true); else PYNQS_MK(false, true); }
+  else { if (is_complex) PYNQS_MK(true, false); else PYNQS_MK(false, false); }
+#undef PYNQS_MK
   return check_launch("weighted_moments");
 }
+
+extern "C" int pynqs_weighted_moments(const double *x, int is_complex, const double *prob, int64_t n, void *workspace, void *stream) {
+  return weighted_moments_launch(x, is_complex, prob, n, workspace, false, 1.0, 1.0, nullptr, stream);
+}
+
+extern "C" int pynqs_weighted_moments_finish(const double *x, int is_complex, const double *prob, int64_t n, void *workspace, double inv_world,
+                                             double counts, double *out5, void *stream) {
+  return weighted_moments_launch(x, is_complex, prob, n, workspace, true, inv_world, counts, out5, stream);
+}
diff --git a/pynqs_amd/csrc/kernels_rbm_forward.hip b/pynqs_amd/csrc/kernels_rbm_forward.hip
--- a/pynqs_amd/csrc/kernels_rbm_forward.hip
+++ b/pynqs_amd/csrc/kernels_rbm_forward.hip
@@ -139,12 +139,21 @@
 __host__ __device__ inline int children_hp(int H) { return (H + 2) | 1; }
 
 template <bool CPLX>
-__global__ __launch_bounds__(kBlock) void rbm_children_factors_kernel(int sorb, int H, const double *__restrict__ W, const double *__restrict__ vb,
-                                                                      double *__restrict__ factors) {
+__device__ __forceinline__ void sum_w_column(const double *__restrict__ W, int sorb, int H, int o, double &re, double &im) {
+  constexpr int C = CPLX ? 2 : 1;
+  re = 0.0; im = 0.0;
+#pragma unroll 16
+  for (int k = 0; k < H; ++k) {
+    re += W[((size_t)k * sorb + o) * C];
+    if constexpr (CPLX) im += W[((size_t)k * sorb + o) * C + 1];
+  }
+}
+
+template <bool CPLX>
+__device__ __forceinline__ void children_factor_entry(int idx, int sorb, int H, const double *__restrict__ W, const double *__restrict__ vb,
+                                                      double *__restrict__ factors) {
   constexpr int C = CPLX ? 2 : 1;
   const int HP = children_hp(H);
-  const int idx = blockIdx.x * kBlock + threadIdx.x;
-  if (idx == 0) factors[(size_t)(2 * sorb + 1) * HP * C] = 0.0;
   if (idx >= (2 * sorb + 1) * HP) return;
   const int row = idx / HP, h = idx - row * HP, o = row >> 1;
   const double sign = (row & 1) ? -1.0 : 1.0;
@@ -162,11 +171,7 @@
       re = m;
     }
   } else if (h == H) {
-#pragma unroll 16
-    for (int k = 0; k < H; ++k) {
-      re += W[((size_t)k * sorb + o) * C];
-      if constexpr (CPLX) im += W[((size_t)k * sorb + o) * C + 1];
-    }
+    sum_w_column<CPLX>(W, sorb, H, o, re, im);
     re *= 2.0 * sign; im *= 2.0 * sign;
   } else if (h == H + 1 && vb) {
     re = 2.0 * sign * vb[(size_t)o * C];
@@ -176,21 +181,22 @@
   if constexpr (CPLX) factors[(size_t)idx * C + 1] = im;
 }
 
+template <bool CPLX>
+__global__ __launch_bounds__(kBlock) void rbm_children_factors_kernel(int sorb, int H, const double *__restrict__ W, const double *__restrict__ vb,
+                                                                      double *__restrict__ factors) {
+  constexpr int C = CPLX ? 2 : 1;
+  const int idx = blockIdx.x * kBlock + threadIdx.x;
+  if (idx == 0) factors[(size_t)(2 * sorb + 1) * children_hp(H) * C] = 0.0;
+  children_factor_entry<CPLX>(idx, sorb, H, W, vb, factors);
+}
+
 constexpr int kParentChunk = 4;
 
 template <int LEN, bool CPLX>
-__global__ __launch_bounds__(kBlock) void rbm_children_parents_kernel(const uint64_t *__restrict__ onv, int64_t n, int sorb, int H,
-                                                                      const double *__restrict__ W, const double *__restrict__ hb,
-                                                                      const double *__restrict__ vb, const double *__restrict__ factors,
-                                                                      double *__restrict__ table) {
-  constexpr int C = CPLX ? 2 : 1;
-  const int64_t i = (int64_t)blockIdx.x * kBlock + threadIdx.x;
-  const int64_t row = i < n ? i : n - 1;
-  const int h0 = (int)blockIdx.y * kParentChunk;
-  uint64_t ket[LEN];
-#pragma unroll
-  for (int w = 0; w < LEN; ++w) ket[w] = onv[row * LEN + w];
-  double *__restrict__ out = table + (size_t)row * (size_t)(H + 2) * C;
+__device__ __forceinline__ void children_parent_chunk(const uint64_t (&ket)[LEN], bool live, int h0, int sorb, int H, const double *__restrict__ W,
+                                                      const double *__restrict__ hb, double *__restrict__ flag, double raised,
+                                                      double *__restrict__ out) {
+  constexpr int C = CPLX ? 2 : 1;
   double tr[kParentChunk], ti[kParentChunk];
 #pragma unroll
   for (int j = 0; j < kParentChunk; ++j) {
@@ -209,8 +215,8 @@
   }
 #pragma unroll
   for (int j = 0; j < kParentChunk; ++j) {
-    if (h0 + j < H && i < n) {
-      if (!(tr[j] > -340.0)) const_cast<double *>(factors)[(size_t)(2 * sorb + 1) * children_hp(H) * C] = 1.0;
+    if (h0 + j < H && live) {
+      if (!(tr[j] > -340.0)) *flag = raised;
       const double m = exp(-2.0 * tr[j]);
       if constexpr (CPLX) {
         double sn, cs;
@@ -222,8 +228,12 @@
       }
     }
   }
-  if (blockIdx.y != 0) return;
-  const int HP = children_hp(H);
+}
+
+template <int LEN, bool CPLX>
+__device__ __forceinline__ void children_parent_sums(const uint64_t (&ket)[LEN], bool live, int sorb, int H, const double *__restrict__ hb,
+                                                     const double *__restrict__ f, size_t fstride, double *__restrict__ out) {
+  constexpr int C = CPLX ? 2 : 1;
   double sr = 0.0, si = 0.0, axr = 0.0, axi = 0.0;
   for (int h = 0; h < H; ++h) {
     sr += hb[(size_t)h * C];
@@ -231,16 +241,75 @@
   }
   for (int o = 0; o < sorb; ++o) {
     const double x = pm1_of<LEN>(ket, o);
-    const double *__restrict__ f = factors + ((size_t)(2 * o) * HP + H) * C;
-    sr = fma(0.5 * x, f[0], sr);
-    axr = fma(0.5 * x, f[C], axr);
-    if constexpr (CPLX) { si = fma(0.5 * x, f[1], si); axi = fma(0.5 * x, f[C + 1], axi); }
-  }
-  if (i >= n) return;
+    const double *__restrict__ fo = f + (size_t)o * fstride;
+    sr = fma(0.5 * x, fo[0], sr);
+    axr = fma(0.5 * x, fo[C], axr);
+    if constexpr (CPLX) { si = fma(0.5 * x, fo[1], si); axi = fma(0.5 * x, fo[C + 1], axi); }
+  }
+  if (!live) return;
   out[(size_t)H * C] = sr;
   out[(size_t)(H + 1) * C] = axr;
   if constexpr (CPLX) { out[(size_t)H * C + 1] = si; out[(size_t)(H + 1) * C + 1] = axi; }
 }
+
+template <int LEN, bool CPLX>
+__global__ __launch_bounds__(kBlock) void rbm_children_parents_kernel(const uint64_t *__restrict__ onv, int64_t n, int sorb, int H,
+                                                                      const double *__restrict__ W, const double *__restrict__ hb,
+                                                                      const double *__restrict__ vb, const double *__restrict__ factors,
+                                                                      double *__restrict__ table) {
+  constexpr int C = CPLX ? 2 : 1;
+  const int64_t i = (int64_t)blockIdx.x * kBlock + threadIdx.x;
+  const int64_t row = i < n ? i : n - 1;
+  uint64_t ket[LEN];
+#pragma unroll
+  for (int w = 0; w < LEN; ++w) ket[w] = onv[row * LEN + w];
+  double *__restrict__ out = table + (size_t)row * (size_t)(H + 2) * C;
+  const int HP = children_hp(H);
+  children_parent_chunk<LEN, CPLX>(ket, i < n, (int)blockIdx.y * kParentChunk, sorb, H, W, hb,
+                                   const_cast<double *>(factors) + (size_t)(2 * sorb + 1) * HP * C, 1.0, out);
+  if (blockIdx.y != 0) return;
+  children_parent_sums<LEN, CPLX>(ket, i < n, sorb, H, hb, factors + (size_t)H * C, (size_t)2 * HP * C, out);
+}
+
+template <int LEN, bool CPLX>
+__global__ __launch_bounds__(kBlock) void rbm_children_prepare_kernel(const uint64_t *__restrict__ onv, int64_t n, int sorb, int H,
+                                                                      const double *__restrict__ W, const double *__restrict__ hb,
+                                                                      const double *__restrict__ vb, double *__restrict__ factors,
+                                                                      double *__restrict__ table, int nchunks, double stamp) {
+  constexpr int C = CPLX ? 2 : 1;
+  __shared__ double fs[kMaxSorb][2][C];
+  if ((int)blockIdx.y == nchunks + 1) {
+    const int64_t idx = (int64_t)blockIdx.x * kBlock + threadIdx.x;
+    if (idx < (int64_t)(2 * sorb + 1) * children_hp(H)) children_factor_entry<CPLX>((int)idx, sorb, H, W, vb, factors);
+    return;
+  }
+  const int64_t i = (int64_t)blockIdx.x * kBlock + threadIdx.x;
+  if ((int64_t)blockIdx.x * kBlock >= n) return;
+  const int64_t row = i < n ? i : n - 1;
+  uint64_t ket[LEN];
+#pragma unroll
+  for (int w = 0; w < LEN; ++w) ket[w] = onv[row * LEN + w];
+  double *__restrict__ out = table + (size_t)row * (size_t)(H + 2) * C;
+  if ((int)blockIdx.y < nchunks) {
+    children_parent_chunk<LEN, CPLX>(ket, i < n, (int)blockIdx.y * kParentChunk, sorb, H, W, hb,
+                                     factors + (size_t)(2 * sorb + 1) * children_hp(H) * C, stamp, out);
+    return;
+  }
+  for (int o = threadIdx.x; o < sorb; o += kBlock) {
+    double re, im;
+    sum_w_column<CPLX>(W, sorb, H, o, re, im);
+    fs[o][0][0] = re * 2.0;
+    fs[o][1][0] = vb ? 2.0 * vb[(size_t)o * C] : 0.0;
+    if constexpr (CPLX) {
+      fs[o][0][1] = im * 2.0;
+      fs[o][1][1] = vb ? 2.0 * vb[(size_t)o * C + 1] : 0.0;
+    }
+  }
+  __syncthreads();
+  children_parent_sums<LEN, CPLX>(ket, i < n, sorb, H, hb, &fs[0][0][0], (size_t)2 * C, out);
+}
+
+__device__ __forceinline__ bool children_flag_raised(double word, double stamp) { return stamp != 0.0 ? word == stamp : word != 0.0; }
 
 #ifndef PYNQS_CHILD_BLOCK
 #define PYNQS_CHILD_BLOCK 1024
@@ -253,14 +322,14 @@
                                                                       int64_t nwalkers, const double *__restrict__ table,
                                                                       const double *__restrict__ factors, int sorb, int H,
                                                                       const double *__restrict__ W, const double *__restrict__ hb,
-                                                                      const double *__restrict__ vb, double *__restrict__ psi) {
+                                                                      const double *__restrict__ vb, double *__restrict__ psi, double stamp) {
   constexpr bool CPLX = FLAVOUR == PYNQS_RBM_COMPLEX;
   constexpr int C = CPLX ? 2 : 1;
   extern __shared__ __attribute__((aligned(16))) double wl[];
   const int HP = children_hp(H);
   int64_t cnt = n;
   if (count_dev) cnt = min((int64_t)max(*count_dev, 0), n);
-  if (factors[(size_t)(2 * sorb + 1) * HP * C] != 0.0) {
+  if (children_flag_raised(factors[(size_t)(2 * sorb + 1) * HP * C], stamp)) {
     const int64_t rounds = (cnt + (int64_t)gridDim.x * kChildBlock - 1) / ((int64_t)gridDim.x * kChildBlock);
     for (int64_t r = 0; r < rounds; ++r) {
       const int64_t i = ((int64_t)r * gridDim.x + blockIdx.x) * kChildBlock + threadIdx.x;
@@ -367,13 +436,13 @@
                                                                            int64_t nwalkers, const double *__restrict__ table,
                                                                            const double *__restrict__ factors, int sorb, int H,
                                                                            const double *__restrict__ W, const double *__restrict__ hb,
-                                                                           const double *__restrict__ vb, double *__restrict__ psi) {
+                                                                           const double *__restrict__ vb, double *__restrict__ psi, double stamp) {
   constexpr bool CPLX = FLAVOUR == PYNQS_RBM_COMPLEX;
   constexpr int C = CPLX ? 2 : 1;
   const int HP = children_hp(H);
   int64_t cnt = n;
   if (count_dev) cnt = min((int64_t)max(*count_dev, 0), n);
-  if (factors[(size_t)(2 * sorb + 1) * HP * C] != 0.0) {
+  if (children_flag_raised(factors[(size_t)(2 * sorb + 1) * HP * C], stamp)) {
     const int64_t rounds = (cnt + (int64_t)gridDim.x * kBlock - 1) / ((int64_t)gridDim.x * kBlock);
     for (int64_t r = 0; r < rounds; ++r) {
       const int64_t i = ((int64_t)r * gridDim.x + blockIdx.x) * kBlock + threadIdx.x;
@@ -560,12 +629,18 @@
   return nwalkers * (nhidden + 2) * c + (int64_t)children_lds_bytes(sorb, nhidden, flavour) + 8;
 }
 
+static int children_prepare_check(const uint64_t *walkers, int64_t nwalkers, int sorb, const double *weights, const double *hidden_bias,
+                                  int nhidden, int flavour, void *table) {
+  if (nwalkers < 0 || nwalkers > 0x7fffffffll * kBlock || sorb < 1 || sorb > kMaxSorb || nhidden < 1 || !children_flavour_ok(flavour))
+    return set_error(PYNQS_EINVAL, "bad nwalkers/sorb/nhidden/flavour");
+  if (!weights || !hidden_bias || !table || (nwalkers > 0 && !walkers)) return set_error(PYNQS_EINVAL, "null pointer");
+  return PYNQS_OK;
+}
+
 extern "C" int pynqs_rbm_children_prepare(const uint64_t *walkers, int64_t nwalkers, int sorb, const double *weights, const double *hidden_bias,
                                           const double *visible_bias, int nhidden, int flavour, void *table, void *stream) {
   pynqs::DeviceScope device_scope_(table);
-  if (nwalkers < 0 || nwalkers > 0x7fffffffll * kBlock || sorb < 1 || sorb > kMaxSorb || nhidden < 1 || !children_flavour_ok(flavour))
-    return set_error(PYNQS_EINVAL, "bad nwalkers/sorb/nhidden/flavour");
-  if (!weights || !hidden_bias || !table || (nwalkers > 0 && !walkers)) return set_error(PYNQS_EINVAL, "null pointer");
+  if (const int rc = children_prepare_check(walkers, nwalkers, sorb, weights, hidden_bias, nhidden, flavour, table)) return rc;
   const bool cplx = flavour == PYNQS_RBM_COMPLEX;
   const int len = (sorb - 1) / 64 + 1;
   hipStream_t st = (hipStream_t)stream;
@@ -589,10 +664,36 @@
   return check_launch("rbm_children_prepare");
 }
 
-extern "C" int pynqs_rbm_forward_children(const uint64_t *onv, int64_t n, const int32_t *count_dev, const int32_t *parent,
-                                          const uint64_t *walkers, int64_t nwalkers, const void *table, int sorb, const double *weights,
-                                          const double *hidden_bias, const double *visible_bias, int nhidden, int flavour, double *psi,
-                                          void *stream) {
+static bool children_stamp_ok(uint64_t stamp) { return stamp >= 1 && stamp < (1ull << 53); }
+
+extern "C" int pynqs_rbm_children_prepare_stamped(const uint64_t *walkers, int64_t nwalkers, int sorb, const double *weights,
+                                                  const double *hidden_bias, const double *visible_bias, int nhidden, int flavour,
+                                                  uint64_t stamp, void *table, void *stream) {
+  pynqs::DeviceScope device_scope_(table);
+  if (const int rc = children_prepare_check(walkers, nwalkers, sorb, weights, hidden_bias, nhidden, flavour, table)) return rc;
+  if (!children_stamp_ok(stamp)) return set_error(PYNQS_EINVAL, "rbm_children_prepare_stamped: stamp must be in [1, 2^53)");
+  const bool cplx = flavour == PYNQS_RBM_COMPLEX;
+  const int len = (sorb - 1) / 64 + 1;
+  double *parents = (double *)table;
+  double *factors = parents + (size_t)nwalkers * (size_t)(nhidden + 2) * (cplx ? 2 : 1);
+  const uint32_t gf = (uint32_t)(((2 * sorb + 1) * children_hp(nhidden) + kBlock - 1) / kBlock);
+  const uint32_t gw = (uint32_t)((nwalkers + kBlock - 1) / kBlock), nchunks = (uint32_t)((nhidden + kParentChunk - 1) / kParentChunk);
+  const dim3 grid(gw > gf ? gw : gf, nchunks + 2);
+  if (grid.y > 65535u) return set_error(PYNQS_EINVAL, "too many hidden units");
+  DISPATCH_LEN(len, {
+    if (cplx)
+      hipLaunchKernelGGL((rbm_children_prepare_kernel<LEN, true>), grid, dim3(kBlock), 0, (hipStream_t)stream, walkers, nwalkers, sorb, nhidden,
+                         weights, hidden_bias, visible_bias, factors, parents, (int)nchunks, (double)stamp);
+    else
+      hipLaunchKernelGGL((rbm_children_prepare_kernel<LEN, false>), grid, dim3(kBlock), 0, (hipStream_t)stream, walkers, nwalkers, sorb, nhidden,
+                         weights, hidden_bias, visible_bias, factors, parents, (int)nchunks, (double)stamp);
+  });
+  return check_launch("rbm_children_prepare_stamped");
+}
+
+static int forward_children_launch(const uint64_t *onv, int64_t n, const int32_t *count_dev, const int32_t *parent, const uint64_t *walkers,
+                                   int64_t nwalkers, const void *table, int sorb, const double *weights, const double *hidden_bias,
+                                   const double *visible_bias, int nhidden, int flavour, double stamp, double *psi, void *stream) {
   pynqs::DeviceScope device_scope_(onv);
   if (n < 0 || n > 0x7fffffffll * kBlock || nwalkers < 0 || sorb < 1 || sorb > kMaxSorb || nhidden < 1) return set_error(PYNQS_EINVAL, "bad n/sorb/nhidden");
   if (!pynqs_rbm_forward_children_supported(sorb, nhidden, flavour))
@@ -614,10 +715,10 @@
   do {                                                                                                                                       \
     if (in_lds)                                                                                                                              \
       hipLaunchKernelGGL((rbm_forward_children_kernel<LEN, F>), dim3(grid), dim3(kChildBlock), lds, st, onv, n, count_dev, parent, walkers,  \
-                         nwalkers, parents, factors, sorb, nhidden, weights, hidden_bias, visible_bias, psi);                                \
+                         nwalkers, parents, factors, sorb, nhidden, weights, hidden_bias, visible_bias, psi, stamp);                         \
     else                                                                                                                                     \
       hipLaunchKernelGGL((rbm_forward_children_wave_kernel<LEN, F>), dim3((uint32_t)wblocks), dim3(kBlock), 0, st, onv, n, count_dev,        \
-                         parent, walkers, nwalkers, parents, factors, sorb, nhidden, weights, hidden_bias, visible_bias, psi);               \
+                         parent, walkers, nwalkers, parents, factors, sorb, nhidden, weights, hidden_bias, visible_bias, psi, stamp);        \
   } while (0)
   DISPATCH_LEN(len, {
     switch (flavour) {
@@ -630,3 +731,20 @@
 #undef PYNQS_RC
   return check_launch("rbm_forward_children");
 }
+
+extern "C" int pynqs_rbm_forward_children(const uint64_t *onv, int64_t n, const int32_t *count_dev, const int32_t *parent,
+                                          const uint64_t *walkers, int64_t nwalkers, const void *table, int sorb, const double *weights,
+                                          const double *hidden_bias, const double *visible_bias, int nhidden, int flavour, double *psi,
+                                          void *stream) {
+  return forward_children_launch(onv, n, count_dev, parent, walkers, nwalkers, table, sorb, weights, hidden_bias, visible_bias, nhidden, flavour,
+                                 0.0, psi, stream);
+}
+
+extern "C" int pynqs_rbm_forward_children_stamped(const uint64_t *onv, int64_t n, const int32_t *count_dev, const int32_t *parent,
+                                                  const uint64_t *walkers, int64_t nwalkers, const void *table, int sorb, const double *weights,
+                                                  const double *hidden_bias, const double *visible_bias, int nhidden, int flavour,
+                                                  uint64_t stamp, double *psi, void *stream) {
+  if (!children_stamp_ok(stamp)) return set_error(PYNQS_EINVAL, "rbm_forward_children_stamped: stamp must be in [1, 2^53)");
+  return forward_children_launch(onv, n, count_dev, parent, walkers, nwalkers, table, sorb, weights, hidden_bias, visible_bias, nhidden, flavour,
+                                 (double)stamp, psi, stream);
+}
diff --git a/pynqs_amd/csrc/kernels_rbm_grad.hip b/pynqs_amd/csrc/kernels_rbm_grad.hip
--- a/pynqs_amd/csrc/kernels_rbm_grad.hip
+++ b/pynqs_amd/csrc/kernels_rbm_grad.hip
@@ -7,8 +7,8 @@
 constexpr int kGradWalkers = 32;
 constexpr int kGradHidden = 32;
 
-template <int LEN, bool CPLX>
-__global__ __launch_bounds__(kBlock) void rbm_grad_partial_kernel(const uint64_t *__restrict__ onv, int64_t n, int sorb, int H,
+template <int LEN, bool CPLX, int B>
+__global__ __launch_bounds__(B) void rbm_grad_partial_kernel(const uint64_t *__restrict__ onv, int64_t n, int sorb, int H,
                                                                   const double *__restrict__ W, const double *__restrict__ hb,
                                                                   const double *__restrict__ vb, const double *__restrict__ prob,
                                                                   const double *__restrict__ eloc, bool eloc_cplx,
@@ -18,7 +18,7 @@
   __shared__ uint64_t xs[kGradWalkers][LEN];
   __shared__ double tc[kGradWalkers][kGradHidden + 1][C];
   __shared__ double cf[kGradWalkers][C];
-  constexpr int NQ = kBlock / kGradWalkers;
+  constexpr int NQ = B / kGradWalkers;
   const int tid = threadIdx.x, w = tid % kGradWalkers, q = tid / kGradWalkers;
   const int64_t i = (int64_t)blockIdx.x * kGradWalkers + w;
   const bool valid = i < n;
@@ -93,7 +93,7 @@
     }
     __syncthreads();
     const int nout = min(kGradHidden, H - h0) * SP;
-    for (int k = tid; k < nout; k += kBlock) {
+    for (int k = tid; k < nout; k += B) {
       const int hh = k / SP, o = k - hh * SP;
       double ar = 0.0, ai = 0.0;
       if (o < sorb) {
@@ -118,9 +118,10 @@
     }
   }
   const int64_t off_vb = (int64_t)H * SP;
-  for (int o = tid; o < sorb; o += kBlock) {
+  for (int o = tid; o < sorb; o += B) {
     const int word = o >> 6, bit = o & 63;
     double ar = 0.0, ai = 0.0;
+#pragma unroll 4
     for (int v = 0; v < kGradWalkers; ++v) {
       const bool up = (xs[v][word] >> bit) & 1ull;
       ar += up ? cf[v][0] : -cf[v][0];
@@ -137,6 +138,7 @@
     }
   }
   __syncthreads();
+  static_assert(NQ * kGradWalkers * 2 <= kGradWalkers * (kGradHidden + 1) * C && kGradHidden % NQ == 0, "B: 256 or 512");
   double *lr = &tc[0][0][0];
   lr[(q * kGradWalkers + w) * 2] = lre;
   lr[(q * kGradWalkers + w) * 2 + 1] = lim;
@@ -159,7 +161,7 @@
 template <bool CPLX>
 __global__ __launch_bounds__(kBlock) void rbm_grad_reduce_kernel(const double *__restrict__ partial, int64_t stride, int ngroups, int sorb, int H,
                                                                  double *__restrict__ gw, double *__restrict__ ghb, double *__restrict__ gvb,
-                                                                 double *__restrict__ loss) {
+                                                                 double *__restrict__ loss, double *__restrict__ loss_copy) {
   constexpr int C = CPLX ? 2 : 1;
   constexpr int NS = kBlock / 64;
   __shared__ double part[NS][64][2];
@@ -192,6 +194,7 @@
   for (int sl = 0; sl < NS; ++sl) { re += part[sl][lane][0]; im += part[sl][lane][1]; }
   if (k == nout - 1) {
     if (loss) loss[0] = re;
+    if (loss_copy) loss_copy[0] = re;
     return;
   }
   double *dst;
@@ -223,10 +226,15 @@
   return groups * grad_stride(sorb, nhidden, flavour == PYNQS_RBM_COMPLEX) * 8;
 }
 
-extern "C" int pynqs_rbm_grad(const uint64_t *onv, int64_t n, int sorb, const double *weights, const double *hidden_bias,
-                              const double *visible_bias, int nhidden, int flavour, const double *prob, const double *eloc,
-                              int eloc_is_complex, const double *e_total, const double *pow, double *grad_weights, double *grad_hidden_bias,
-                              double *grad_visible_bias, double *loss, void *workspace, void *stream) {
+static int grad_block() {
+  static const int b = getenv("PYNQS_RBM_GRAD_BLOCK") ? atoi(getenv("PYNQS_RBM_GRAD_BLOCK")) : 512;
+  return b == 256 ? 256 : 512;
+}
+
+extern "C" int pynqs_rbm_grad_loss(const uint64_t *onv, int64_t n, int sorb, const double *weights, const double *hidden_bias,
+                                   const double *visible_bias, int nhidden, int flavour, const double *prob, const double *eloc,
+                                   int eloc_is_complex, const double *e_total, const double *pow, double *grad_weights, double *grad_hidden_bias,
+                                   double *grad_visible_bias, double *loss, double *loss_copy, void *workspace, void *stream) {
   pynqs::DeviceScope device_scope_(onv);
   if (n < 0 || n > 0x7fffffffll * kGradWalkers || sorb < 1 || sorb > kMaxSorb || nhidden < 1) return set_error(PYNQS_EINVAL, "bad n/sorb/nhidden");
   if (flavour != PYNQS_RBM_REAL && flavour != PYNQS_RBM_COMPLEX) return set_error(PYNQS_EINVAL, "rbm_grad: flavour must be PYNQS_RBM_REAL or PYNQS_RBM_COMPLEX");
@@ -238,12 +246,13 @@
   hipStream_t st = (hipStream_t)stream;
   double *partial = (double *)workspace;
   if (groups > 0) {
-#define PYNQS_RG(C)                                                                                                                          \
-  hipLaunchKernelGGL((rbm_grad_partial_kernel<LEN, C>), dim3((uint32_t)groups), dim3(kBlock), 0, st, onv, n, sorb, nhidden, weights, hidden_bias, \
+    const bool wide = grad_block() == 512;
+#define PYNQS_RG(C, B)                                                                                                                         \
+  hipLaunchKernelGGL((rbm_grad_partial_kernel<LEN, C, B>), dim3((uint32_t)groups), dim3(B), 0, st, onv, n, sorb, nhidden, weights, hidden_bias, \
                      visible_bias, prob, eloc, eloc_is_complex != 0, e_total, pow, partial, stride)
     DISPATCH_LEN(len, {
-      if (cplx) PYNQS_RG(true);
-      else PYNQS_RG(false);
+      if (cplx) { if (wide) PYNQS_RG(true, 512); else PYNQS_RG(true, 256); }
+      else { if (wide) PYNQS_RG(false, 512); else PYNQS_RG(false, 256); }
     });
 #undef PYNQS_RG
   }
@@ -251,9 +260,17 @@
   const uint32_t g2 = (uint32_t)((nout + 63) / 64);
   if (cplx)
     hipLaunchKernelGGL((rbm_grad_reduce_kernel<true>), dim3(g2), dim3(kBlock), 0, st, partial, stride, (int)groups, sorb, nhidden, grad_weights,
-                       grad_hidden_bias, grad_visible_bias, loss);
+                       grad_hidden_bias, grad_visible_bias, loss, loss_copy);
   else
     hipLaunchKernelGGL((rbm_grad_reduce_kernel<false>), dim3(g2), dim3(kBlock), 0, st, partial, stride, (int)groups, sorb, nhidden, grad_weights,
-                       grad_hidden_bias, grad_visible_bias, loss);
+                       grad_hidden_bias, grad_visible_bias, loss, loss_copy);
   return check_launch("rbm_grad");
 }
+
+extern "C" int pynqs_rbm_grad(const uint64_t *onv, int64_t n, int sorb, const double *weights, const double *hidden_bias,
+                              const double *visible_bias, int nhidden, int flavour, const double *prob, const double *eloc,
+                              int eloc_is_complex, const double *e_total, const double *pow, double *grad_weights, double *grad_hidden_bias,
+                              double *grad_visible_bias, double *loss, void *workspace, void *stream) {
+  return pynqs_rbm_grad_loss(onv, n, sorb, weights, hidden_bias, visible_bias, nhidden, flavour, prob, eloc, eloc_is_complex, e_total, pow,
+                             grad_weights, grad_hidden_bias, grad_visible_bias, loss, nullptr, workspace, stream);
+}
diff --git a/pynqs_amd/csrc/kernels_reduce_onepass.hip b/pynqs_amd/csrc/kernels_reduce_onepass.hip
--- a/pynqs_amd/csrc/kernels_reduce_onepass.hip
+++ b/pynqs_amd/csrc/kernels_reduce_onepass.hip
@@ -549,6 +549,12 @@
   }
 }
 
+__global__ __launch_bounds__(kBlock) void reduce_clear_kernel(uint4 *__restrict__ table, size_t n16, uint32_t *__restrict__ counters) {
+  const uint4 ones = make_uint4(0xffffffffu, 0xffffffffu, 0xffffffffu, 0xffffffffu);
+  for (size_t i = (size_t)blockIdx.x * kBlock + threadIdx.x; i < n16; i += (size_t)gridDim.x * kBlock) table[i] = ones;
+  if (blockIdx.x == 0 && threadIdx.x < 4) counters[threadIdx.x] = 0u;
+}
+
 }
 
 using namespace pynqs;
@@ -734,9 +740,17 @@
   if (io->lut_table && io->lut_nkeys < 0) return set_error(PYNQS_EINVAL, "bad lut_nkeys");
   hipStream_t st = (hipStream_t)stream;
   const int len = (sorb - 1) / 64 + 1;
-  if (hipMemsetAsync(io->counters, 0, 16, st) != hipSuccess) return check_launch("memset");
-  if (io->dedup_table &&
-      hipMemsetAsync(io->dedup_table, 0xFF, (size_t)io->dedup_slots * dedup_slot_words(len) * 8, st) != hipSuccess) return check_launch("memset");
+  static const bool clear_kernel = !(getenv("PYNQS_REDUCE_CLEAR_KERNEL") && atoi(getenv("PYNQS_REDUCE_CLEAR_KERNEL")) == 0);
+  const size_t table_bytes = io->dedup_table ? (size_t)io->dedup_slots * dedup_slot_words(len) * 8 : 0;
+  if (clear_kernel && table_bytes && table_bytes % 16 == 0 && ((uintptr_t)io->dedup_table & 15) == 0 && ((uintptr_t)io->counters & 3) == 0) {
+    const size_t n16 = table_bytes / 16;
+    size_t blocks = (n16 + (size_t)kBlock * 8 - 1) / ((size_t)kBlock * 8);
+    if (blocks > 2048) blocks = 2048;
+    hipLaunchKernelGGL(reduce_clear_kernel, dim3((uint32_t)blocks), dim3(kBlock), 0, st, (uint4 *)io->dedup_table, n16, (uint32_t *)io->counters);
+  } else {
+    if (hipMemsetAsync(io->counters, 0, 16, st) != hipSuccess) return check_launch("memset");
+    if (table_bytes && hipMemsetAsync(io->dedup_table, 0xFF, table_bytes, st) != hipSuccess) return check_launch("memset");
+  }
   if (nbatch == 0) return PYNQS_OK;
   if (!bra || !plan) return set_error(PYNQS_EINVAL, "null pointer");
   uint32_t nchunks, chunk_len, max_tiles, fixed;
diff --git a/pynqs_amd/grad.py b/pynqs_amd/grad.py
--- a/pynqs_amd/grad.py
+++ b/pynqs_amd/grad.py
@@ -191,11 +191,13 @@
         params = self.params
         W, hb, vb = (p.detach().contiguous() for p in params)
         gw, ghb, gvb = self.views
-        N.check(N.lib().pynqs_rbm_grad(onv.contiguous().data_ptr(), n, self.sorb, W.data_ptr(), hb.data_ptr(), vb.data_ptr(), self.H, self.flavour,
-                                       prob.data_ptr(), el.data_ptr(), int(cplx), et.data_ptr(), pw.data_ptr() if pw is not None else None,
-                                       gw.data_ptr(), ghb.data_ptr(), gvb.data_ptr(), self.loss.data_ptr(), self.work.data_ptr(),
-                                       torch.cuda.current_stream(dev).cuda_stream), "pynqs_rbm_grad")
         ws = get_world_size()
+        loss_out = torch.empty(1, dtype=torch.float64, device=dev) if ws == 1 else None
+        N.check(N.lib().pynqs_rbm_grad_loss(onv.contiguous().data_ptr(), n, self.sorb, W.data_ptr(), hb.data_ptr(), vb.data_ptr(), self.H,
+                                            self.flavour, prob.data_ptr(), el.data_ptr(), int(cplx), et.data_ptr(),
+                                            pw.data_ptr() if pw is not None else None, gw.data_ptr(), ghb.data_ptr(), gvb.data_ptr(),
+                                            self.loss.data_ptr(), loss_out.data_ptr() if loss_out is not None else None, self.work.data_ptr(),
+                                            torch.cuda.current_stream(dev).cuda_stream), "pynqs_rbm_grad_loss")
         ev = None
         if self.events is not None:
             ev = [torch.cuda.Event(enable_timing=True) for _ in range(2)]
@@ -210,7 +212,7 @@
             self.events.append(ev)
         for p, v in zip(params, self.views):
             p.grad = v
-        return self.loss * ws if ws > 1 else self.loss.clone()
+        return self.loss * ws if ws > 1 else loss_out
 
 
 class FusedJastrowRbmGrad:
diff --git a/pynqs_amd/stats.py b/pynqs_amd/stats.py
--- a/pynqs_amd/stats.py
+++ b/pynqs_amd/stats.py
@@ -39,14 +39,25 @@
 _WS: dict = {}
 
 
+def _on_kernel(x: Tensor, prob: Tensor) -> bool:
+    return x.is_cuda and prob.is_cuda and prob.dtype == torch.float64 and x.dtype in (torch.float64, torch.complex128) and x.dim() == 1
+
+
+def _workspace(dev) -> Tensor:
+    from . import _native as N
+
+    ws = _WS.get(dev)
+    if ws is None:
+        ws = _WS[dev] = torch.zeros(N.lib().pynqs_moments_workspace() // 8, dtype=torch.float64, device=dev)
+    return ws
+
+
 def _moments(x: Tensor, prob: Tensor) -> Tensor:
-    if x.is_cuda and prob.is_cuda and prob.dtype == torch.float64 and x.dtype in (torch.float64, torch.complex128) and x.dim() == 1:
+    if _on_kernel(x, prob):
         from . import _native as N
 
         dev = x.device
-        ws = _WS.get(dev)
-        if ws is None:
-            ws = _WS[dev] = torch.zeros(N.lib().pynqs_moments_workspace() // 8, dtype=torch.float64, device=dev)
+        ws = _workspace(dev)
         xc, pc = x.contiguous(), prob.contiguous()
         N.check(N.lib().pynqs_weighted_moments(xc.data_ptr(), int(x.is_complex()), pc.data_ptr(), x.numel(), ws.data_ptr(),
                                                torch.cuda.current_stream(dev).cuda_stream), "pynqs_weighted_moments")
@@ -58,6 +69,17 @@
 
 
 def dist_stats_moments(x: Tensor, prob: Tensor, counts: Optional[int] = None, world_size: int = 1):
+    if get_world_size() == 1 and _on_kernel(x, prob):
+        from . import _native as N
+
+        dev = x.device
+        out = torch.empty(6, dtype=torch.float64, device=dev)
+        xc, pc = x.contiguous(), prob.contiguous()
+        N.check(N.lib().pynqs_weighted_moments_finish(xc.data_ptr(), int(x.is_complex()), pc.data_ptr(), x.numel(), _workspace(dev).data_ptr(),
+                                                      1.0 / world_size, float(counts if counts is not None else x.size(0)), out.data_ptr(),
+                                                      torch.cuda.current_stream(dev).cuda_stream), "pynqs_weighted_moments_finish")
+        mean = torch.view_as_complex(out[0:2]).reshape(()) if torch.is_complex(x) else out[0]
+        return mean, out[2], out[3], out[4]
     m = _moments(x, prob)
     if counts is None:
         counts = x.size(0) * get_world_size()
```

After: 9.888 million, median of 6. 3.8% higher.
